# shubhamchandak94/Spring

Hardware: AMD Instinct MI355X
Metric: Mreads/s through reorder stage (higher is better)
Workload: dtype u64; 1 GPU; 100000000 x 150 bp single-end synthetic reads per GPU (uniform genome 600000000 bp, 25x coverage, 1.0% substitutions, 50% reverse-complemented), inputs resident in HBM as .dna records; reads_per_gpu=100000000, read_len=150, chains=65536, num_thr=8, parallelism=single GPU, unmatched=13958636, singletons=12720853, rounds=1984, chain_groups=2

## Files before the change

### include/spring_reorder.h

```cpp
#ifndef SPRING_REORDER_H_
#define SPRING_REORDER_H_

#include <stddef.h>
#include <stdint.h>

#ifdef __cplusplus
extern "C" {
#endif

#define SPRING_REORDER_E_ARG (-1)
#define SPRING_REORDER_E_IO (-2)
#define SPRING_REORDER_E_HIP (-3)
#define SPRING_REORDER_E_STATE (-4)

typedef struct spring_reorder_ctx spring_reorder_ctx;

typedef struct {
  int32_t device;
  uint32_t num_chains;
  int32_t num_thr;
  int32_t collect_stats;
  int32_t time_search;
  int32_t force_literal_update;
  int32_t rounds_per_sync;
  int32_t long_budget;
  int32_t first_shifts;
  int32_t seed_wide;
  int32_t tab_scale;
  int32_t search_wpb;
  int32_t dbg_search_lds;
  int32_t dbg_apply_lds;
  int32_t fused;
  int32_t deep_bins;
  int32_t num_devices;
  int32_t devices[8];
  int32_t mg_host_transport;
  int32_t table_mode;
  int32_t plan0[6];
  int32_t plan1[6];
  int32_t long_min;
  int32_t long_blocks;
  int32_t debug;
  int32_t long_split;
  int32_t entry_flags;
  int32_t out_writers;
  int32_t alternatives;
  int32_t phases;
  int32_t known_absent;
  int32_t sort_prefix_bits;
  int32_t dict_build_mode;
  int32_t strand_filter;
} spring_reorder_opts;

typedef struct {
  uint64_t n_reads, n_matched, n_single, unmatched;
  uint64_t probes, keyok, cands, hits, iterations, rounds, lost;
  uint64_t numkeys[2], dict_numreads[2];
  double ms_unpack, ms_dict, ms_chains, ms_finalize, ms_total;
  double ms_search_kernel;
  uint64_t search_launches;
  uint64_t device_bytes;
  double ms_exchange, ms_resolve_mark;
  uint64_t chains;
  uint64_t deep_pool;
  uint64_t long_searches;
  uint64_t table_minz;
  uint64_t table_marked_lines;
  uint64_t long_splits;
  uint64_t alternatives;
  uint64_t phases;
  double ms_search_busy;
  uint64_t sort_prefix_bits;
  uint64_t sort_repaired_runs;
  uint64_t sort_full_sorts;
  uint64_t sort_long_runs;
  uint64_t sort_list_overflows;
  uint64_t dict_build_path;
  uint64_t strand_filter;
  uint64_t strand_filter_dropped;
  uint64_t strand_filter_build;
} spring_reorder_stats;

void spring_reorder_default_opts(spring_reorder_opts *o);
const char *spring_reorder_last_error(void);
void spring_reorder_trim_pool(void);

int spring_reorder_run(const char *temp_dir, uint32_t max_readlen, int32_t num_thr, int32_t paired_end,
                       uint32_t num_reads_clean_0, uint32_t num_reads_clean_1,
                       const spring_reorder_opts *opts );

int spring_reorder_create(spring_reorder_ctx **ctx, const spring_reorder_opts *opts);
void spring_reorder_destroy(spring_reorder_ctx *ctx);

int spring_reorder_load_dna(spring_reorder_ctx *ctx, const uint8_t *dna, size_t nbytes, uint32_t n,
                            uint32_t max_readlen);

int spring_reorder_load_dna_device(spring_reorder_ctx *ctx, const void *d_dna, size_t nbytes, uint32_t n,
                                   uint32_t max_readlen, int32_t fixed_len);

int spring_reorder_build_dict(spring_reorder_ctx *ctx);

int spring_reorder_run_chains(spring_reorder_ctx *ctx);
int spring_reorder_auto_chains(spring_reorder_ctx *ctx, uint32_t *chains, int32_t *deep);

typedef struct {
  uint32_t num_reads[2], num_reads_clean[2], num_reads_N[2];
  uint32_t max_readlen;
  uint32_t pad;
  double ms_device;
} spring_fastq_info;
int spring_reorder_load_fastq(spring_reorder_ctx *ctx, const uint8_t *fastq_1, size_t nbytes_1, const uint8_t *fastq_2,
                              size_t nbytes_2 , spring_fastq_info *info);
int spring_reorder_fastq_N(spring_reorder_ctx *ctx, int32_t which, uint8_t *n_dna, size_t cap, size_t *nbytes,
                           uint32_t *order_N, uint32_t *count);

int spring_reorder_mg_begin(spring_reorder_ctx *ctx, uint32_t rank, uint32_t world, uint32_t total_chains, void *d_prop);
int spring_reorder_mg_search(spring_reorder_ctx *ctx);
int spring_reorder_mg_slice(spring_reorder_ctx *ctx, void **d_prop, size_t *slice_off, size_t *slice_bytes,
                            size_t *total_bytes);
int spring_reorder_mg_slices(spring_reorder_ctx *ctx, void **d_prop, size_t slice_off[2], size_t slice_bytes[2],
                             size_t *total_bytes, uint32_t *count);
int spring_reorder_mg_apply(spring_reorder_ctx *ctx, int32_t check_alive, uint32_t *alive);
int spring_reorder_mg_end(spring_reorder_ctx *ctx);
int spring_reorder_debug_check_seed_state(spring_reorder_ctx *ctx, int32_t group, uint64_t *violations);
int spring_reorder_mg_exchange_virtual(spring_reorder_ctx **ctxs, uint32_t world);

#define SPRING_RCCL_ID_BYTES 128
typedef struct spring_mg_comm spring_mg_comm;
typedef int (*spring_mg_allgather_fn)(void *host_buf, size_t slice_off, size_t slice_bytes, size_t total_bytes,
                                      void *user);
int spring_mg_rccl_unique_id(void *id128);
int spring_mg_comm_create_rccl(spring_mg_comm **comm, int32_t device, const void *id128, uint32_t rank, uint32_t world);
int spring_mg_comm_create_host(spring_mg_comm **comm, spring_mg_allgather_fn fn, void *user, uint32_t rank,
                               uint32_t world);
void spring_mg_comm_destroy(spring_mg_comm *comm);
int spring_reorder_mg_run(spring_reorder_ctx *ctx, spring_mg_comm *comm, uint32_t total_chains);

int spring_reorder_finalize(spring_reorder_ctx *ctx);

int spring_reorder_get_stats(spring_reorder_ctx *ctx, spring_reorder_stats *st);

int spring_reorder_download(spring_reorder_ctx *ctx, uint32_t *order, char *rc, char *flag, int64_t *pos,
                            uint16_t *rlen, uint32_t *order_s, uint64_t *tid_off, uint64_t *tid_off_s);
int spring_reorder_tid_split(spring_reorder_ctx *ctx, uint64_t *mid, uint64_t *mid_s);

int spring_reorder_emit_dna(spring_reorder_ctx *ctx, int32_t tid, uint8_t *dst, size_t cap, size_t *nbytes);

int spring_reorder_dict_lookup(spring_reorder_ctx *ctx, int32_t which, const uint64_t *keys, uint32_t nkeys,
                               uint32_t *bin_size, uint32_t *bin_ids, size_t ids_cap);

int spring_reorder_presence_table(spring_reorder_ctx *ctx, void *out, size_t cap, int32_t *lgb);

int spring_reorder_download_reads(spring_reorder_ctx *ctx, uint64_t *limbs , uint16_t *len);

int spring_order_invert_se(const uint32_t *order, uint32_t n, uint32_t *order_array, double *kernel_ms);
int spring_order_invert_pe(const uint32_t *order, uint32_t n, uint32_t *order_array, double *kernel_ms);
int spring_order_correct(uint32_t *order, uint64_t m, const uint32_t *order_N, uint32_t nN, uint32_t n_clean,
                         double *kernel_ms);
int spring_order_pe_encode(const uint32_t *order, uint32_t n, uint32_t *new_order, double *kernel_ms);

int spring_fastq_reorder(const uint8_t *fastq, size_t nbytes, const uint32_t *order, uint32_t n, uint8_t *out,
                         size_t out_cap, size_t *out_bytes, double *kernel_ms);

#define SPRING_SYNTH_REPEATS 0x80000000u
#define SPRING_SYNTH_PAIRED 0x40000000u
#define SPRING_SYNTH_GENOMIC 0x20000000u
size_t spring_synth_dna_bytes(uint32_t n, uint32_t L);
int spring_synth_dna_host(uint8_t *dst, uint32_t n, uint32_t L, uint64_t G, uint64_t seed, uint32_t err_ppm);
int spring_synth_genome_host(uint8_t *dst, uint64_t G, uint64_t seed, uint32_t flags);
int spring_synth_dna_device(void *d_dst, uint32_t n, uint32_t L, uint64_t G, uint64_t seed, uint32_t err_ppm);
int spring_reorder_load_synth(spring_reorder_ctx *ctx, uint32_t n, uint32_t L, uint64_t G, uint64_t seed,
                              uint32_t err_ppm);
int spring_reorder_download_dna(spring_reorder_ctx *ctx, uint8_t *dst, size_t cap);

#ifdef __cplusplus
}
#endif
#endif
```

### spring_amd/_lib.py

```python
import ctypes as C
import os

HERE = os.path.dirname(os.path.abspath(__file__))
LIB_PATH = os.environ.get("SPRING_AMD_LIB") or os.path.join(HERE, "lib", "libspring_reorder_hip.so")

EXPORTS = [
    "spring_reorder_default_opts", "spring_reorder_last_error", "spring_reorder_trim_pool", "spring_reorder_run", "spring_reorder_create",
    "spring_reorder_destroy", "spring_reorder_load_dna", "spring_reorder_load_dna_device",
    "spring_reorder_build_dict", "spring_reorder_run_chains", "spring_reorder_auto_chains", "spring_reorder_finalize",
    "spring_reorder_mg_begin", "spring_reorder_mg_search", "spring_reorder_mg_slice", "spring_reorder_mg_slices",
    "spring_reorder_mg_apply",
    "spring_reorder_mg_end", "spring_reorder_mg_exchange_virtual", "spring_reorder_debug_check_seed_state",
    "spring_mg_rccl_unique_id", "spring_mg_comm_create_rccl", "spring_mg_comm_create_host", "spring_mg_comm_destroy",
    "spring_reorder_mg_run",
    "spring_reorder_get_stats", "spring_reorder_download", "spring_reorder_tid_split", "spring_reorder_emit_dna",
    "spring_reorder_dict_lookup", "spring_reorder_presence_table", "spring_reorder_download_reads", "spring_synth_dna_bytes",
    "spring_reorder_load_fastq", "spring_reorder_fastq_N",
    "spring_order_invert_se", "spring_order_invert_pe", "spring_order_correct", "spring_order_pe_encode",
    "spring_fastq_reorder",
    "spring_synth_dna_host", "spring_synth_genome_host", "spring_synth_dna_device", "spring_reorder_load_synth", "spring_reorder_download_dna",
    "spring_encoder_create", "spring_encoder_destroy", "spring_encoder_set_split_tables", "spring_encoder_encode_reorder", "spring_encoder_download",
    "spring_encoder_download_seq_packed", "spring_encoder_get_info", "spring_reorder_encode_run", "spring_encoder_encode_host", "spring_encoder_run",
]

STREAMS_EXPORTS = [
    "spring_streams_create", "spring_streams_destroy", "spring_streams_from_encoder", "spring_streams_from_host",
    "spring_streams_download", "spring_streams_get_info", "spring_streams_run",
]
STREAMS_NUM = 9

DECODE_EXPORTS = [
    "spring_decode_create", "spring_decode_destroy", "spring_decode_seq_from_encoder", "spring_decode_seq_from_host",
    "spring_decode_seq_from_files", "spring_decode_from_streams", "spring_decode_from_host", "spring_decode_from_files",
    "spring_decode_download", "spring_decode_get_info",
]

QUALID_EXPORTS = [
    "spring_qualid_create", "spring_qualid_destroy", "spring_qualid_order_from_host", "spring_qualid_order_from_encoder",
    "spring_qualid_from_fastq", "spring_qualid_from_lines", "spring_qualid_download", "spring_qualid_get_info",
    "spring_quality_table", "spring_id_pattern",
]

FASTQ_OUT_EXPORTS = [
    "spring_fastq_out_create", "spring_fastq_out_destroy", "spring_fastq_out_assemble", "spring_fastq_out_download",
    "spring_fastq_out_write", "spring_fastq_out_get_info",
]

GZIP_EXPORTS = [
    "spring_gzip_create", "spring_gzip_destroy", "spring_gzip_set_chunk_bytes", "spring_gzip_set_token_bytes",
    "spring_gzip_from_fastq_out", "spring_gzip_from_host", "spring_gzip_download", "spring_gzip_write",
    "spring_gzip_get_info",
]

BWT_EXPORTS = [
    "spring_bwt_create", "spring_bwt_destroy", "spring_bwt_set_block_bytes", "spring_bwt_set_workspace_bytes",
    "spring_bwt_workspace_need", "spring_bwt_from_host", "spring_bwt_from_streams", "spring_bwt_download",
    "spring_bwt_segments", "spring_bwt_get_info", "spring_bwt_encode_inplace", "spring_bwt_set_run_keys",
    "spring_bwt_from_qualid", "spring_bwt_round_entries",
]
BWT_MAX_INDEXES = 256
BWT_SRC_QUALITY, BWT_SRC_ID = -2, -3

UNBWT_EXPORTS = [
    "spring_unbwt_create", "spring_unbwt_destroy", "spring_unbwt_set_workspace_bytes", "spring_unbwt_workspace_need",
    "spring_unbwt_set_head_spacing", "spring_unbwt_from_host", "spring_unbwt_from_bwt", "spring_unbwt_download",
    "spring_unbwt_get_info", "spring_unbwt_decode_inplace", "spring_unbwt_from_unqlfc",
]
UNBWT_PASSES = 6

IDCODEC_EXPORTS = [
    "spring_idcodec_create", "spring_idcodec_destroy", "spring_idcodec_set_workspace_bytes",
    "spring_idcodec_workspace_need", "spring_idcodec_from_qualid", "spring_idcodec_from_host", "spring_idcodec_download",
    "spring_idcodec_symbols", "spring_idcodec_get_info",
]
QLFC_EXPORTS = [
    "spring_qlfc_create", "spring_qlfc_destroy", "spring_qlfc_set_state_tables", "spring_qlfc_set_workspace_bytes",
    "spring_qlfc_workspace_need", "spring_qlfc_from_host", "spring_qlfc_from_bwt", "spring_qlfc_download",
    "spring_qlfc_get_info", "spring_qlfc_compress",
]
QLFC_RANK_TABLE, QLFC_RUN_TABLE = 32768, 8192
QLFC_PASSES = 6
QLFC_NOT_COMPRESSIBLE = -16
QLFC_EVENT_BYTES = 160

UNQLFC_EXPORTS = [
    "spring_unqlfc_create", "spring_unqlfc_destroy", "spring_unqlfc_set_state_tables", "spring_unqlfc_set_workspace_bytes",
    "spring_unqlfc_workspace_need", "spring_unqlfc_from_host", "spring_unqlfc_from_qlfc", "spring_unqlfc_download",
    "spring_unqlfc_get_info", "spring_unqlfc_decompress",
]
UNQLFC_PASSES = 3
UNQLFC_MODEL_BYTES = 1619200

BSC_EXPORTS = [
    "spring_bsc_create", "spring_bsc_destroy", "spring_bsc_from_streams", "spring_bsc_from_qualid", "spring_bsc_from_host",
    "spring_bsc_download", "spring_bsc_files", "spring_bsc_get_info", "spring_bsc_adler32", "spring_bsc_compress",
]
BSC_HEADER_BYTES = 28
BSC_PASSES = 3
BSC_BLOCKS, BSC_FILE, BSC_STR_ARRAY = 0, 1, 2
BSC_CODED, BSC_STORED_SMALL, BSC_STORED_CODER, BSC_STORED_NO_GAIN = 0, 1, 2, 3


class Opts(C.Structure):
    _fields_ = [("device", C.c_int32), ("num_chains", C.c_uint32), ("num_thr", C.c_int32),
                ("collect_stats", C.c_int32), ("time_search", C.c_int32), ("force_literal_update", C.c_int32),
                ("rounds_per_sync", C.c_int32), ("long_budget", C.c_int32),
                ("first_shifts", C.c_int32), ("seed_wide", C.c_int32), ("tab_scale", C.c_int32),
                ("search_wpb", C.c_int32), ("dbg_search_lds", C.c_int32), ("dbg_apply_lds", C.c_int32),
                ("fused", C.c_int32), ("deep_bins", C.c_int32),
                ("num_devices", C.c_int32), ("devices", C.c_int32 * 8), ("mg_host_transport", C.c_int32),
                ("table_mode", C.c_int32), ("plan0", C.c_int32 * 6), ("plan1", C.c_int32 * 6), ("long_min", C.c_int32),
                ("long_blocks", C.c_int32), ("debug", C.c_int32), ("long_split", C.c_int32), ("entry_flags", C.c_int32),
                ("out_writers", C.c_int32), ("alternatives", C.c_int32), ("phases", C.c_int32), ("known_absent", C.c_int32),
                ("sort_prefix_bits", C.c_int32), ("dict_build_mode", C.c_int32), ("strand_filter", C.c_int32)]


class Info(C.Structure):

    def asdict(self):
        d = {}
        for k, _ in self._fields_:
            v = getattr(self, k)
            d[k] = list(v) if hasattr(v, "__len__") else v
        return d


class FastqInfo(C.Structure):
    _fields_ = [("num_reads", C.c_uint32 * 2), ("num_reads_clean", C.c_uint32 * 2), ("num_reads_N", C.c_uint32 * 2),
                ("max_readlen", C.c_uint32), ("pad", C.c_uint32), ("ms_device", C.c_double)]


class EncoderInfo(Info):
    _fields_ = ([(k, C.c_uint64) for k in ("n_aligned", "n_total", "seq_len", "noise_bytes", "n_noisepos",
                                           "unaligned_bytes", "len_unaligned", "num_contigs")]
                + [(k, C.c_uint32) for k in ("matched_s", "matched_N", "align_passes", "max_bin")]
                + [("ms_device", C.c_double), ("ms_phase", C.c_double * 8)])


class StreamsInfo(Info):
    _fields_ = ([("num_units", C.c_uint64), ("num_blocks", C.c_uint64), ("bytes", C.c_uint64 * STREAMS_NUM),
                 ("flag_count", C.c_uint64 * 5), ("pos_escapes", C.c_uint64), ("n_aligned", C.c_uint64),
                 ("ms_device", C.c_double), ("ms_file", C.c_double)])


class QualIdInfo(Info):
    _fields_ = [("num_units", C.c_uint64), ("num_blocks", C.c_uint64), ("bytes", C.c_uint64 * 2),
                ("bytes_changed", C.c_uint64), ("max_len", C.c_uint32 * 2), ("ms_device", C.c_double)]


class FastqOutParams(C.Structure):
    _fields_ = ([(k, C.c_uint32) for k in ("first_block", "num_blocks", "num_reads", "num_reads_per_block")]
                + [(k, C.c_int32) for k in ("paired_end", "mate", "preserve_quality", "id_mode", "paired_id_code", "pad")]
                + [("range_start", C.c_uint64), ("range_end", C.c_uint64)])


class FastqOutSources(C.Structure):
    _fields_ = [("decode", C.c_void_p), ("bases", C.c_void_p), ("read_off", C.c_void_p),
                ("quality_ctx", C.c_void_p), ("quality", C.c_void_p), ("quality_bytes", C.c_uint64),
                ("quality_block_off", C.c_void_p),
                ("id_ctx", C.c_void_p), ("ids", C.c_void_p), ("id_bytes", C.c_uint64), ("id_block_off", C.c_void_p)]


class FastqOutInfo(Info):
    _fields_ = [("num_units", C.c_uint64), ("first_slot", C.c_uint64), ("bytes", C.c_uint64),
                ("ms_device", C.c_double), ("ms_file", C.c_double)]


class GzipInfo(Info):
    _fields_ = ([(k, C.c_uint64) for k in ("num_members", "bytes_in", "bytes_out", "chunk_bytes", "num_chunks",
                                           "chunks_stored")]
                + [("ms_device", C.c_double), ("ms_file", C.c_double), ("ms_pass", C.c_double * 6),
                   ("num_batches", C.c_uint64)])


class BwtInfo(Info):
    _fields_ = ([(k, C.c_uint64) for k in ("num_segments", "bytes", "max_segment", "sub_batches", "rounds",
                                           "rounds_total", "workspace_bytes")]
                + [("ms_device", C.c_double), ("ms_pass", C.c_double * 5), ("run_positions", C.c_uint64)])


class UnbwtInfo(Info):
    _fields_ = ([(k, C.c_uint64) for k in ("num_segments", "bytes", "max_segment", "sub_batches", "heads", "head_spacing",
                                           "max_walk", "rank_rounds", "workspace_bytes")]
                + [("ms_device", C.c_double), ("ms_pass", C.c_double * UNBWT_PASSES)])


class IdCodecInfo(Info):
    _fields_ = ([(k, C.c_uint64) for k in ("num_lines", "num_blocks", "num_symbols", "bytes", "max_tokens", "sub_batches")]
                + [("ms_tokens", C.c_double), ("ms_coder", C.c_double)])


class DecodeInfo(Info):
    _fields_ = ([(k, C.c_uint64) for k in ("seq_len", "first_block", "num_blocks", "num_units")]
                + [("bases", C.c_uint64 * 2)]
                + [(k, C.c_uint64) for k in ("n_aligned", "n_unaligned", "pos_escapes")]
                + [("ms_device", C.c_double), ("ms_file", C.c_double)])


class Stats(Info):
    _fields_ = ([(k, C.c_uint64) for k in ("n_reads", "n_matched", "n_single", "unmatched", "probes", "keyok",
                                          "cands", "hits", "iterations", "rounds", "lost")]
                + [("numkeys", C.c_uint64 * 2), ("dict_numreads", C.c_uint64 * 2)]
                + [(k, C.c_double) for k in ("ms_unpack", "ms_dict", "ms_chains", "ms_finalize", "ms_total",
                                             "ms_search_kernel")]
                + [("search_launches", C.c_uint64), ("device_bytes", C.c_uint64),
                   ("ms_exchange", C.c_double), ("ms_resolve_mark", C.c_double), ("chains", C.c_uint64),
                   ("deep_pool", C.c_uint64), ("long_searches", C.c_uint64),
                   ("table_minz", C.c_uint64), ("table_marked_lines", C.c_uint64), ("long_splits", C.c_uint64), ("alternatives", C.c_uint64), ("phases", C.c_uint64),
                   ("ms_search_busy", C.c_double),
                   ("sort_prefix_bits", C.c_uint64), ("sort_repaired_runs", C.c_uint64), ("sort_full_sorts", C.c_uint64),
                   ("sort_long_runs", C.c_uint64), ("sort_list_overflows", C.c_uint64), ("dict_build_path", C.c_uint64),
                   ("strand_filter", C.c_uint64), ("strand_filter_dropped", C.c_uint64),
                   ("strand_filter_build", C.c_uint64)])


NOT_INT = {"spring_reorder_last_error": C.c_char_p, "spring_synth_dna_bytes": C.c_size_t,
           "spring_reorder_default_opts": None, "spring_reorder_trim_pool": None, "spring_mg_comm_destroy": None}
NOT_INT.update({p + "_destroy": None for p in ("spring_reorder", "spring_encoder", "spring_streams", "spring_decode",
                                               "spring_qualid", "spring_fastq_out", "spring_gzip", "spring_bwt",
                                               "spring_unbwt", "spring_idcodec", "spring_qlfc", "spring_bsc",
                                               "spring_unqlfc")})
NOT_INT.update({p + "_workspace_need": C.c_uint64 for p in ("spring_bwt", "spring_unbwt", "spring_idcodec", "spring_qlfc",
                                                             "spring_unqlfc")})

MG_ALLGATHER_FN = C.CFUNCTYPE(C.c_int, C.c_void_p, C.c_size_t, C.c_size_t, C.c_size_t, C.c_void_p)

_lib = None


def lib():
    global _lib
    if _lib is not None:
        return _lib
    if not os.path.exists(LIB_PATH):
        raise RuntimeError(
            "spring_amd: %s is missing. Build it with `python -m spring_amd.build` "
            "(or __graft_entry__.build()); there is no CPU fallback." % LIB_PATH)
    L = C.CDLL(LIB_PATH)
    vp, u8p = C.c_void_p, C.c_void_p
    L.spring_reorder_default_opts.argtypes = [C.POINTER(Opts)]
    L.spring_reorder_run.argtypes = [C.c_char_p, C.c_uint32, C.c_int32, C.c_int32, C.c_uint32, C.c_uint32,
                                     C.POINTER(Opts)]
    L.spring_reorder_create.argtypes = [C.POINTER(vp), C.POINTER(Opts)]
    L.spring_reorder_destroy.argtypes = [vp]
    L.spring_reorder_load_dna.argtypes = [vp, u8p, C.c_size_t, C.c_uint32, C.c_uint32]
    L.spring_reorder_load_dna_device.argtypes = [vp, vp, C.c_size_t, C.c_uint32, C.c_uint32, C.c_int32]
    L.spring_reorder_build_dict.argtypes = [vp]
    L.spring_reorder_run_chains.argtypes = [vp]
    L.spring_reorder_auto_chains.argtypes = [vp, C.POINTER(C.c_uint32), C.POINTER(C.c_int32)]
    L.spring_reorder_finalize.argtypes = [vp]
    L.spring_reorder_mg_begin.argtypes = [vp, C.c_uint32, C.c_uint32, C.c_uint32, vp]
    L.spring_reorder_mg_search.argtypes = [vp]
    L.spring_reorder_mg_slice.argtypes = [vp, C.POINTER(vp), C.POINTER(C.c_size_t), C.POINTER(C.c_size_t), C.POINTER(C.c_size_t)]
    L.spring_reorder_mg_slices.argtypes = [vp, C.POINTER(vp), C.POINTER(C.c_size_t), C.POINTER(C.c_size_t), C.POINTER(C.c_size_t),
                                           C.POINTER(C.c_uint32)]
    L.spring_reorder_debug_check_seed_state.argtypes = [vp, C.c_int32, C.POINTER(C.c_uint64)]
    L.spring_reorder_mg_apply.argtypes = [vp, C.c_int32, C.POINTER(C.c_uint32)]
    L.spring_reorder_mg_end.argtypes = [vp]
    L.spring_reorder_mg_exchange_virtual.argtypes = [C.POINTER(vp), C.c_uint32]
    L.spring_mg_rccl_unique_id.argtypes = [vp]
    L.spring_mg_comm_create_rccl.argtypes = [C.POINTER(vp), C.c_int32, vp, C.c_uint32, C.c_uint32]
    L.spring_mg_comm_create_host.argtypes = [C.POINTER(vp), MG_ALLGATHER_FN, vp, C.c_uint32, C.c_uint32]
    L.spring_mg_comm_destroy.argtypes = [vp]
    L.spring_reorder_mg_run.argtypes = [vp, vp, C.c_uint32]
    L.spring_reorder_get_stats.argtypes = [vp, C.POINTER(Stats)]
    L.spring_reorder_download.argtypes = [vp] + [vp] * 8
    L.spring_reorder_tid_split.argtypes = [vp, vp, vp]
    L.spring_reorder_emit_dna.argtypes = [vp, C.c_int32, u8p, C.c_size_t, C.POINTER(C.c_size_t)]
    L.spring_reorder_dict_lookup.argtypes = [vp, C.c_int32, vp, C.c_uint32, vp, vp, C.c_size_t]
    L.spring_reorder_presence_table.argtypes = [vp, vp, C.c_size_t, C.POINTER(C.c_int32)]
    L.spring_reorder_download_reads.argtypes = [vp, vp, vp]
    L.spring_reorder_load_fastq.argtypes = [vp, vp, C.c_size_t, vp, C.c_size_t, C.POINTER(FastqInfo)]
    L.spring_reorder_fastq_N.argtypes = [vp, C.c_int32, vp, C.c_size_t, C.POINTER(C.c_size_t), vp, C.POINTER(C.c_uint32)]
    L.spring_order_invert_se.argtypes = [vp, C.c_uint32, vp, C.POINTER(C.c_double)]
    L.spring_order_invert_pe.argtypes = [vp, C.c_uint32, vp, C.POINTER(C.c_double)]
    L.spring_fastq_reorder.argtypes = [u8p, C.c_size_t, vp, C.c_uint32, u8p, C.c_size_t, C.POINTER(C.c_size_t),
                                       C.POINTER(C.c_double)]
    L.spring_order_pe_encode.argtypes = [vp, C.c_uint32, vp, C.POINTER(C.c_double)]
    L.spring_order_correct.argtypes = [vp, C.c_uint64, vp, C.c_uint32, C.c_uint32, C.POINTER(C.c_double)]
    L.spring_synth_dna_bytes.argtypes = [C.c_uint32, C.c_uint32]
    L.spring_synth_dna_host.argtypes = [u8p, C.c_uint32, C.c_uint32, C.c_uint64, C.c_uint64, C.c_uint32]
    L.spring_synth_genome_host.argtypes = [u8p, C.c_uint64, C.c_uint64, C.c_uint32]
    L.spring_synth_dna_device.argtypes = [vp, C.c_uint32, C.c_uint32, C.c_uint64, C.c_uint64, C.c_uint32]
    L.spring_reorder_load_synth.argtypes = [vp, C.c_uint32, C.c_uint32, C.c_uint64, C.c_uint64, C.c_uint32]
    L.spring_reorder_download_dna.argtypes = [vp, u8p, C.c_size_t]
    L.spring_encoder_create.argtypes = [C.c_int32, C.POINTER(vp)]
    L.spring_encoder_destroy.argtypes = [vp]
    L.spring_encoder_encode_reorder.argtypes = [vp, vp, u8p, C.c_uint64, vp, C.c_uint32, C.POINTER(EncoderInfo)]
    L.spring_encoder_download.argtypes = [vp] + [vp] * 9
    L.spring_encoder_download_seq_packed.argtypes = [vp, vp, vp]
    L.spring_encoder_encode_host.argtypes = [vp, C.c_uint32, C.c_int32, vp, u8p, C.c_uint64, vp, vp, vp, vp, vp, u8p,
                                             C.c_uint64, vp, C.c_uint32, u8p, C.c_uint64, vp, C.c_uint32,
                                             C.POINTER(EncoderInfo)]
    L.spring_encoder_run.argtypes = [C.c_char_p, C.c_uint32, C.c_int32, C.c_uint32, C.c_uint32, C.c_int32,
                                     C.POINTER(EncoderInfo)]
    L.spring_encoder_get_info.argtypes = [vp, C.POINTER(EncoderInfo)]
    L.spring_reorder_encode_run.argtypes = [C.c_char_p, C.c_uint32, C.c_int32, C.c_int32, C.c_uint32, C.c_uint32,
                                            C.c_uint32, C.POINTER(Opts), C.POINTER(EncoderInfo)]
    L.spring_streams_create.argtypes = [C.c_int32, C.POINTER(vp)]
    L.spring_streams_destroy.argtypes = [vp]
    L.spring_streams_from_encoder.argtypes = [vp, vp, C.c_uint32, C.c_int32, C.c_int32, C.c_uint32, C.c_int32,
                                              C.POINTER(StreamsInfo)]
    L.spring_streams_from_host.argtypes = [vp, vp, vp, C.c_uint64, vp, C.c_uint64, vp, C.c_uint64, vp, vp, C.c_uint64, vp,
                                           C.c_uint64, C.c_uint32, C.c_int32, C.c_int32, C.c_uint32, C.POINTER(StreamsInfo)]
    L.spring_streams_download.argtypes = [vp, C.c_int32, vp, vp]
    L.spring_streams_get_info.argtypes = [vp, C.POINTER(StreamsInfo)]
    L.spring_streams_run.argtypes = [C.c_char_p, C.c_uint32, C.c_int32, C.c_int32, C.c_uint32, C.c_int32,
                                     C.POINTER(StreamsInfo)]
    L.spring_decode_create.argtypes = [C.c_int32, C.POINTER(vp)]
    L.spring_decode_destroy.argtypes = [vp]
    L.spring_decode_seq_from_encoder.argtypes = [vp, vp]
    L.spring_decode_seq_from_host.argtypes = [vp, C.c_int32, vp, vp, vp]
    L.spring_decode_seq_from_files.argtypes = [vp, C.c_char_p, C.c_int32]
    L.spring_decode_from_streams.argtypes = [vp, vp, C.POINTER(DecodeInfo)]
    L.spring_decode_from_host.argtypes = [vp, vp, vp, C.c_uint32, C.c_uint32, C.c_uint32, C.c_int32, C.c_int32,
                                          C.c_uint32, C.POINTER(DecodeInfo)]
    L.spring_decode_from_files.argtypes = [vp, C.c_char_p, C.c_uint32, C.c_uint32, C.c_uint32, C.c_int32, C.c_int32,
                                           C.c_uint32, C.POINTER(DecodeInfo)]
    L.spring_decode_download.argtypes = [vp, C.c_int32, vp, vp]
    L.spring_decode_get_info.argtypes = [vp, C.POINTER(DecodeInfo)]
    L.spring_qualid_create.argtypes = [C.c_int32, C.POINTER(vp)]
    L.spring_qualid_destroy.argtypes = [vp]
    L.spring_qualid_order_from_host.argtypes = [vp, vp, C.c_uint32, C.c_int32]
    L.spring_qualid_order_from_encoder.argtypes = [vp, vp, C.c_uint32, C.c_int32]
    L.spring_qualid_from_fastq.argtypes = [vp, u8p, C.c_size_t, C.c_int32, u8p, C.c_uint32, C.POINTER(QualIdInfo)]
    L.spring_qualid_from_lines.argtypes = [vp, C.c_int32, u8p, C.c_size_t, u8p, C.c_uint32, C.POINTER(QualIdInfo)]
    L.spring_qualid_download.argtypes = [vp, C.c_int32, u8p, vp, vp]
    L.spring_qualid_get_info.argtypes = [vp, C.POINTER(QualIdInfo)]
    L.spring_quality_table.argtypes = [C.c_int32, C.c_uint32, C.c_uint32, C.c_uint32, u8p]
    L.spring_id_pattern.argtypes = [u8p, C.c_size_t, u8p, C.c_size_t, C.c_int32, C.POINTER(C.c_uint8),
                                    C.POINTER(C.c_double)]
    L.spring_fastq_out_create.argtypes = [C.c_int32, C.POINTER(vp)]
    L.spring_fastq_out_destroy.argtypes = [vp]
    L.spring_fastq_out_assemble.argtypes = [vp, C.POINTER(FastqOutParams), C.POINTER(FastqOutSources),
                                            C.POINTER(FastqOutInfo)]
    L.spring_fastq_out_download.argtypes = [vp, u8p, vp]
    L.spring_fastq_out_write.argtypes = [vp, C.c_char_p, C.c_int32, C.POINTER(FastqOutInfo)]
    L.spring_fastq_out_get_info.argtypes = [vp, C.POINTER(FastqOutInfo)]
    L.spring_gzip_create.argtypes = [C.c_int32, C.POINTER(vp)]
    L.spring_gzip_destroy.argtypes = [vp]
    L.spring_gzip_set_chunk_bytes.argtypes = [vp, C.c_uint32]
    L.spring_gzip_set_token_bytes.argtypes = [vp, C.c_uint64]
    L.spring_gzip_from_fastq_out.argtypes = [vp, vp, C.c_uint64, C.c_int32, C.POINTER(GzipInfo)]
    L.spring_gzip_from_host.argtypes = [vp, u8p, C.c_uint64, vp, C.c_uint64, C.c_int32, C.POINTER(GzipInfo)]
    L.spring_gzip_download.argtypes = [vp, u8p, vp]
    L.spring_gzip_write.argtypes = [vp, C.c_char_p, C.c_int32, C.POINTER(GzipInfo)]
    L.spring_gzip_get_info.argtypes = [vp, C.POINTER(GzipInfo)]
    L.spring_bwt_create.argtypes = [C.c_int32, C.POINTER(vp)]
    L.spring_bwt_destroy.argtypes = [vp]
    L.spring_bwt_set_block_bytes.argtypes = [vp, C.c_uint64]
    L.spring_bwt_set_workspace_bytes.argtypes = [vp, C.c_uint64]
    L.spring_bwt_workspace_need.argtypes = [C.c_uint64, C.c_uint64]
    L.spring_bwt_from_host.argtypes = [vp, u8p, C.c_uint64, vp, C.c_uint64, C.POINTER(BwtInfo)]
    L.spring_bwt_from_streams.argtypes = [vp, vp, C.c_uint32, C.POINTER(BwtInfo)]
    L.spring_bwt_download.argtypes = [vp, u8p, vp, vp, vp, vp]
    L.spring_bwt_segments.argtypes = [vp, vp, vp, vp]
    L.spring_bwt_get_info.argtypes = [vp, C.POINTER(BwtInfo)]
    L.spring_bwt_encode_inplace.argtypes = [vp, u8p, C.c_int32, vp, vp]
    L.spring_bwt_set_run_keys.argtypes = [vp, C.c_int32, C.c_uint32]
    L.spring_bwt_round_entries.argtypes = [vp, vp, C.c_uint64]
    L.spring_bwt_from_qualid.argtypes = [vp, vp, C.c_int32, C.c_uint64, C.POINTER(BwtInfo)]
    L.spring_unbwt_create.argtypes = [C.c_int32, C.POINTER(vp)]
    L.spring_unbwt_destroy.argtypes = [vp]
    L.spring_unbwt_set_workspace_bytes.argtypes = [vp, C.c_uint64]
    L.spring_unbwt_workspace_need.argtypes = [C.c_uint64, C.c_uint64]
    L.spring_unbwt_set_head_spacing.argtypes = [vp, C.c_uint32]
# ... 51 lines not shown
```

### spring_amd/csrc/dict_build.h

```cpp
#ifndef SPRING_DICT_BUILD_H_
#define SPRING_DICT_BUILD_H_

#include "reorder_device.h"

namespace sr {

bool launch_unpack_keys(hipStream_t st, const uint8_t *dna, uint32_t n, int L, int W, int S, uint32_t rec_fixed,
                        uint64_t *reads, uint16_t *lens, uint32_t *bad_len, int dstart0, int dend0, int dstart1, int dend1,
                        uint64_t *keys0, uint32_t *vals0, uint64_t *keys1, uint32_t *vals1);

constexpr int TAB_WRITE_LG = 10;
inline int tab_write_lg(int bshift) { return 64 - bshift < TAB_WRITE_LG ? 64 - bshift : TAB_WRITE_LG; }
inline uint32_t tab_write_blocks(int bshift) { return (uint32_t)(1ull << (64 - bshift - tab_write_lg(bshift))); }
void launch_tab_partition(hipStream_t st, const uint64_t *h0, uint32_t nk0, const uint64_t *h1, uint32_t nk1, int bshift,
                          uint32_t *part);
constexpr uint32_t TAB_OVF_SLOTS = 8;
void launch_tab_write(hipStream_t st, const uint64_t *h0, uint32_t nk0, const uint64_t *h1, uint32_t nk1,
                      const uint32_t *part, DictBuild d0, DictBuild d1, uint4 *fpt, int bshift, uint32_t *ovf,
                      uint32_t *ovf_blk, uint32_t *ovf_cnt);
void launch_tab_overflow_blocks(hipStream_t st, const uint64_t *h0, uint32_t nk0, const uint64_t *h1, DictBuild d0,
                                DictBuild d1, uint32_t *fpt, int bshift, const uint32_t *ovf_blk, const uint32_t *ovf_cnt);
void launch_tab_overflow_pairs(hipStream_t st, const uint64_t *h0, uint32_t nk0, const uint64_t *h1, DictBuild d0,
                               DictBuild d1, uint32_t *fpt, int bshift, const uint32_t *ovf, uint32_t novf);

constexpr uint32_t PRES_DROP_CTRS = 1024;
constexpr int PRES_WRITE_LG = 10;
inline int pres_write_lg(int lgb) { return lgb < PRES_WRITE_LG ? lgb : PRES_WRITE_LG; }
inline uint32_t pres_write_blocks(int lgb) { return 1u << (lgb - pres_write_lg(lgb)); }
void launch_pres_insert(hipStream_t st, const uint64_t *h0, uint32_t nk0, const uint64_t *h1, uint32_t nk1, int wl, uint32_t *pres,
                        int lgb, uint32_t *drops, bool skip_self_canonical);
void launch_pres_write(hipStream_t st, const uint64_t *h0, uint32_t nk0, const uint64_t *h1, uint32_t nk1, int wl, uint4 *pres,
                       int lgb, uint32_t *part, uint32_t *drops);

}

#endif
```

### spring_amd/csrc/dict_build.hip

```cpp
#include <hip/hip_runtime.h>

#include "dict_build.h"
#include "strand_filter.h"

namespace sr {

__device__ __forceinline__ uint64_t db_mix64(uint64_t x) {
  x ^= x >> 33; x *= 0xff51afd7ed558ccdull; x ^= x >> 33; x *= 0xc4ceb9fe1a85ec53ull; x ^= x >> 33;
  return x;
}
__device__ __forceinline__ uint64_t db_unmix64(uint64_t x) {
  x ^= x >> 33; x *= 0x9cb4b2f8129337dbull; x ^= x >> 33; x *= 0x4f74430c22a54005ull; x ^= x >> 33;
  return x;
}
__device__ __forceinline__ uint32_t db_fp30_of(uint64_t h) {
  const uint32_t f = (uint32_t)h & 0x3fffffffu;
  return f == 0u ? 1u : f == 0x3fffffffu ? 0x3ffffffeu : f;
}

__global__ __launch_bounds__(256) void k_unpack_fixed_keys(const uint8_t *__restrict__ dna, uint32_t n, int L, int W, int lgS,
                                                           uint32_t rec, uint64_t *__restrict__ reads,
                                                           uint16_t *__restrict__ lens, uint32_t *__restrict__ bad_len,
                                                           int dstart0, int klen0, int dstart1, int klen1,
                                                           uint64_t *__restrict__ keys0, uint32_t *__restrict__ vals0,
                                                           uint64_t *__restrict__ keys1, uint32_t *__restrict__ vals1) {
  extern __shared__ uint4 s_unpack[];
  const uint32_t r0 = blockIdx.x * (uint32_t)UNPACK_READS;
  const uint32_t nr = min((uint32_t)UNPACK_READS, n - r0);
  const uint8_t *g = dna + (uint64_t)r0 * rec;
  const uint32_t sh = (uint32_t)((uintptr_t)g & 15u);
  const uint4 *ga = reinterpret_cast<const uint4 *>(g - sh);
  const uint32_t nchunk = (sh + nr * rec + 15u) >> 4;
  for (uint32_t k = threadIdx.x; k < nchunk; k += 256) s_unpack[k] = ga[k];
  __syncthreads();
  const uint8_t *sb = reinterpret_cast<const uint8_t *>(s_unpack);
  const uint32_t *sw = reinterpret_cast<const uint32_t *>(s_unpack);
  const bool chk = bad_len != nullptr;
  const uint32_t S = 1u << lgS;
  auto len_of = [&](uint32_t r) -> uint32_t {
    const uint32_t p = sh + r * rec;
    return (uint32_t)sb[p] | ((uint32_t)sb[p + 1] << 8);
  };
  auto limb = [&](uint32_t m) -> uint64_t {
    const uint32_t r = m >> lgS, j = m & (S - 1u);
    if ((int)j >= W) return 0;
    uint32_t len = len_of(r);
    if (chk && len != (uint32_t)L) len = (uint32_t)L;
    const uint32_t nb = min((len + 3u) / 4u, rec - 2u), pos = 8u * j;
    if (pos >= nb) return 0;
    const uint32_t p = sh + r * rec + 2u + pos, k = p >> 2, s8 = (p & 3u) * 8u;
    uint64_t v = (uint64_t)sw[k] | ((uint64_t)sw[k + 1] << 32);
    if (s8) v = (v >> s8) | ((uint64_t)sw[k + 2] << (64u - s8));
    if (nb - pos < 8u) v &= (1ull << (8u * (nb - pos))) - 1ull;
    return v;
  };
  for (uint32_t t = threadIdx.x; 2u * t < nr; t += 256) {
    const uint32_t r = 2u * t;
    uint32_t l0 = len_of(r), l1 = r + 1 < nr ? len_of(r + 1) : (uint32_t)L;
    if (chk && (l0 != (uint32_t)L || l1 != (uint32_t)L)) {
      *bad_len = 1u;
      l0 = l1 = (uint32_t)L;
    }
    if (r + 1 < nr) *reinterpret_cast<uint32_t *>(lens + r0 + r) = l0 | (l1 << 16);
    else lens[r0 + r] = (uint16_t)l0;
  }
  const uint32_t nl = nr << lgS;
  uint64_t *out = reads + ((uint64_t)r0 << lgS);
  for (uint32_t q = threadIdx.x; 2u * q < nl; q += 256) {
    const uint32_t m = 2u * q;
    const uint64_t v0 = limb(m);
    if (m + 1 < nl) *reinterpret_cast<ulonglong2 *>(out + m) = make_ulonglong2(v0, limb(m + 1));
    else out[m] = v0;
  }
  auto window = [&](uint32_t r, int dstart, int klen2) -> uint64_t {
    const uint32_t bitpos = 2u * (uint32_t)dstart, li = bitpos >> 6, off = bitpos & 63u;
    uint64_t v = limb((r << lgS) + li) >> off;
    if (off && li + 1u < S) v |= limb((r << lgS) + li + 1u) << (64u - off);
    if (klen2 < 64) v &= (1ull << klen2) - 1ull;
    return v;
  };
  for (uint32_t r = threadIdx.x; r < nr; r += 256) {
    const uint32_t i = r0 + r;
    keys0[i] = db_mix64(window(r, dstart0, 2 * klen0));
    vals0[i] = i;
    keys1[i] = db_mix64(window(r, dstart1, 2 * klen1));
    vals1[i] = i;
  }
}

bool launch_unpack_keys(hipStream_t st, const uint8_t *dna, uint32_t n, int L, int W, int S, uint32_t rec_fixed,
                        uint64_t *reads, uint16_t *lens, uint32_t *bad_len, int dstart0, int dend0, int dstart1, int dend1,
                        uint64_t *keys0, uint32_t *vals0, uint64_t *keys1, uint32_t *vals1) {
  if (!n || ((uintptr_t)reads & 15u) || ((uintptr_t)lens & 3u)) return false;
  if (dstart0 < 0 || dstart1 < 0 || dend0 >= L || dend1 >= L || 2 * dend0 / 64 >= S || 2 * dend1 / 64 >= S) return false;
  int lgS = 0;
  while ((1 << lgS) < S) lgS++;
  const size_t lds = ((size_t)UNPACK_READS * rec_fixed + 15 + 12 + 15) / 16 * 16;
  hipLaunchKernelGGL(k_unpack_fixed_keys, dim3((n + UNPACK_READS - 1) / UNPACK_READS), dim3(256), lds, st, dna, n, L, W, lgS,
                     rec_fixed, reads, lens, bad_len, dstart0, dend0 - dstart0 + 1, dstart1, dend1 - dstart1 + 1, keys0, vals0,
                     keys1, vals1);
  return true;
}

__global__ void k_tab_partition(const uint64_t *__restrict__ h0, uint32_t nk0, const uint64_t *__restrict__ h1, uint32_t nk1,
                                int bshift, int lg, uint32_t nblk, uint32_t *__restrict__ part) {
  const uint64_t t = (uint64_t)blockIdx.x * blockDim.x + threadIdx.x;
  if (t >= 2ull * ((uint64_t)nblk + 1)) return;
  const uint32_t l = t > nblk ? 1u : 0u, j = (uint32_t)(t - (l ? (uint64_t)nblk + 1 : 0));
  const uint64_t *__restrict__ h = l ? h1 : h0;
  const uint32_t nk = l ? nk1 : nk0;
  uint32_t lo = 0, hi = nk;
  if (j == nblk) {
    lo = nk;
  } else if (j != 0u) {
    const uint64_t bound = ((uint64_t)j << lg) << bshift;
    while (lo < hi) {
      const uint32_t mid = lo + (hi - lo) / 2;
      if (h[mid] < bound) lo = mid + 1; else hi = mid;
    }
  }
  part[t] = lo;
}

constexpr uint32_t TAB_WRITE_TILE = 512, TAB_WRITE_THREADS = 512;
__global__ __launch_bounds__(TAB_WRITE_THREADS) void k_tab_write(const uint64_t *__restrict__ h0, uint32_t nk0,
                                                                 const uint64_t *__restrict__ h1, uint32_t nk1,
                                                                 const uint32_t *__restrict__ part, uint32_t nblk,
                                                                 DictBuild d0, DictBuild d1, uint4 *__restrict__ fpt,
                                                                 int bshift, int lg, uint32_t *__restrict__ ovf,
                                                                 uint32_t *__restrict__ ovf_blk, uint32_t *__restrict__ ovf_cnt) {
  __shared__ uint4 img[2u << TAB_WRITE_LG];
  __shared__ uint64_t tile[2][TAB_WRITE_TILE];
  __shared__ uint16_t first[2][1u << TAB_WRITE_LG];
  __shared__ uint32_t s_novf;
  const uint32_t nbk = 1u << lg, bmask = nbk - 1u, blk = blockIdx.x;
  for (uint32_t k = threadIdx.x; k < 2u * nbk; k += TAB_WRITE_THREADS) img[k] = make_uint4(0u, 0u, 0u, 0u);
  for (uint32_t k = threadIdx.x; k < nbk / 2u + 1u; k += TAB_WRITE_THREADS) {
    if (2u * k < nbk) { reinterpret_cast<uint32_t *>(first[0])[k] = 0u; reinterpret_cast<uint32_t *>(first[1])[k] = 0u; }
  }
  if (threadIdx.x == 0) s_novf = 0u;
  const uint32_t a0 = part[blk], a1 = part[(uint64_t)nblk + 1 + blk];
  const uint32_t c0 = part[blk + 1] - a0, c1 = part[(uint64_t)nblk + 2 + blk] - a1;
  const uint32_t ntot = c0 + c1;
  auto bin_of = [&](uint32_t t, uint32_t &st, uint32_t &cn, uint32_t &pay) {
    const bool l = t >= c0;
    const uint32_t i = l ? a1 + (t - c0) : a0 + t;
    st = (l ? d1.ustart : d0.ustart)[i]; cn = (l ? d1.ucount : d0.ucount)[i];
    pay = cn == 1u ? (l ? d1.ids : d0.ids)[st] : i;
  };
  uint32_t st0 = 0, cn0 = 0, pay0 = 0, st1 = 0, cn1 = 0, pay1 = 0;
  if (threadIdx.x < ntot) bin_of(threadIdx.x, st0, cn0, pay0);
  if (threadIdx.x + TAB_WRITE_THREADS < ntot) bin_of(threadIdx.x + TAB_WRITE_THREADS, st1, cn1, pay1);
  __syncthreads();
  for (uint32_t k = threadIdx.x; k < min(c0, TAB_WRITE_TILE); k += TAB_WRITE_THREADS) {
    const uint64_t x = h0[a0 + k];
    tile[0][k] = x;
    if (k == 0u || (h0[a0 + k - 1u] >> bshift) != (x >> bshift)) first[0][(uint32_t)(x >> bshift) & bmask] = (uint16_t)(k + 1u);
  }
  for (uint32_t k = threadIdx.x; k < min(c1, TAB_WRITE_TILE); k += TAB_WRITE_THREADS) {
    const uint64_t x = h1[a1 + k];
    tile[1][k] = x;
    if (k == 0u || (h1[a1 + k - 1u] >> bshift) != (x >> bshift)) first[1][(uint32_t)(x >> bshift) & bmask] = (uint16_t)(k + 1u);
  }
  const bool staged = c0 <= TAB_WRITE_TILE && c1 <= TAB_WRITE_TILE;
  __syncthreads();
  if (ntot) {
    uint32_t *imgw = reinterpret_cast<uint32_t *>(img);
    auto H = [&](bool l, uint32_t k) -> uint64_t {
      if (k < TAB_WRITE_TILE) return l ? tile[1][k] : tile[0][k];
      return l ? h1[a1 + k] : h0[a0 + k];
    };
    auto place = [&](uint32_t t, uint32_t st, uint32_t cn, uint32_t pay) {
      const bool l = t >= c0;
      const uint32_t k = l ? t - c0 : t, i = (l ? a1 : a0) + k;
      const uint64_t hh = H(l, k), b = hh >> bshift;
      uint32_t rank = 0;
      while (rank < 4u && k > rank && (H(l, k - 1u - rank) >> bshift) == b) rank++;
      if (rank < 4u && staged) {
        const uint32_t f = l ? first[0][(uint32_t)b & bmask] : first[1][(uint32_t)b & bmask], co = l ? c0 : c1;
        if (f) {
          for (uint32_t o = f - 1u; rank < 4u && o < co; o++) {
            const uint64_t x = l ? tile[0][o] : tile[1][o];
            if ((x >> bshift) != b || (l ? x > hh : x >= hh)) break;
            rank++;
          }
        }
      } else if (rank < 4u) {
        uint32_t lo = 0, hi = l ? c0 : c1;
        while (lo < hi) {
          const uint32_t mid = (lo + hi) >> 1;
          const uint64_t x = H(!l, mid);
          if (l ? x <= hh : x < hh) lo = mid + 1u; else hi = mid;
        }
        while (rank < 4u && lo > 0u && (H(!l, lo - 1u) >> bshift) == b) { rank++; lo--; }
      }
      uint32_t *nd = l ? d1.ndeep : d0.ndeep;
      if (cn >= DEEP_BIN) (l ? d1.deep : d0.deep)[atomicAdd(nd, 1u)] = i;
      if (cn >= BIG_BIN) atomicAdd(nd + 1, cn);
      if (cn >= MID_BIN) atomicAdd(nd + 2, cn);
      (l ? d1.urec : d0.urec)[i] = make_ulonglong2(db_unmix64(hh), (uint64_t)st | ((uint64_t)cn << 32));
      if (rank >= 4u) {
        const uint32_t g = l ? nk0 + i : i, slot = atomicAdd(&s_novf, 1u);
        if (slot < TAB_OVF_SLOTS) ovf_blk[(uint64_t)blk * TAB_OVF_SLOTS + slot] = g;
        else ovf[1u + atomicAdd(ovf, 1u)] = g;
      } else {
        const uint32_t bl = (uint32_t)b & bmask;
        imgw[bl * 8u + rank] = (db_fp30_of(hh) << 2) | ((uint32_t)l << 1) | (cn == 1u ? 1u : 0u);
        imgw[bl * 8u + 4u + rank] = pay;
      }
    };
    if (threadIdx.x < ntot) place(threadIdx.x, st0, cn0, pay0);
    if (threadIdx.x + TAB_WRITE_THREADS < ntot) place(threadIdx.x + TAB_WRITE_THREADS, st1, cn1, pay1);
    for (uint32_t t = threadIdx.x + 2u * TAB_WRITE_THREADS; t < ntot; t += TAB_WRITE_THREADS) {
      bin_of(t, st0, cn0, pay0);
      place(t, st0, cn0, pay0);
    }
    __syncthreads();
  }
  if (threadIdx.x == 0) ovf_cnt[blk] = min(s_novf, TAB_OVF_SLOTS);
  uint4 *__restrict__ out = fpt + (((uint64_t)blk << lg) << 1);
  for (uint32_t k = threadIdx.x; k < 2u * nbk; k += TAB_WRITE_THREADS) out[k] = img[k];
}

__device__ __forceinline__ void tab_overflow_insert(uint32_t g, const uint64_t *__restrict__ h0, uint32_t nk0,
                                                    const uint64_t *__restrict__ h1, const DictBuild &d0, const DictBuild &d1,
                                                    uint32_t *fpt, int bshift) {
  const uint32_t l = g >= nk0 ? 1u : 0u, u = l ? g - nk0 : g;
  const uint64_t h = (l ? h1 : h0)[u];
  const DictBuild &d = l ? d1 : d0;
  const uint32_t st = d.ustart[u], cn = d.ucount[u];
  const bool single = cn == 1u;
  const uint32_t tag = (db_fp30_of(h) << 2) | (l << 1) | (single ? 1u : 0u);
  const uint32_t pay = single ? d.ids[st] : u;
  const uint64_t bmask = (1ull << (64 - bshift)) - 1;
  uint64_t b = ((h >> bshift) + 1) & bmask;
  for (;;) {
    uint32_t *bk = fpt + b * 8;
    for (int sl = 0; sl < 4; sl++) {
      if (atomicCAS(bk + sl, 0u, tag) == 0u) {
        bk[4 + sl] = pay;
        return;
      }
    }
    b = (b + 1) & bmask;
  }
}
__global__ void k_tab_overflow_blocks(const uint64_t *__restrict__ h0, uint32_t nk0, const uint64_t *__restrict__ h1,
                                      DictBuild d0, DictBuild d1, uint32_t *fpt, int bshift, uint32_t nblk,
                                      const uint32_t *__restrict__ ovf_blk, const uint32_t *__restrict__ ovf_cnt) {
  const uint64_t t = (uint64_t)blockIdx.x * blockDim.x + threadIdx.x;
  const uint64_t blk = t / TAB_OVF_SLOTS;
  if (blk >= nblk || (uint32_t)(t % TAB_OVF_SLOTS) >= ovf_cnt[blk]) return;
  tab_overflow_insert(ovf_blk[t], h0, nk0, h1, d0, d1, fpt, bshift);
}
// ... 124 lines not shown
```

### spring_amd/csrc/reorder_pipeline.cpp

```cpp
#include <hip/hip_runtime.h>
#include <dlfcn.h>

#include <algorithm>
#include <system_error>
#include <thread>
#include <memory>
#include <atomic>
#include <chrono>
#include <cstdarg>
#include <cstdio>
#include <cstdlib>
#include <cstring>
#include <map>
#include <mutex>
#include <new>
#include <stdexcept>
#include <string>
#include <unordered_map>
#include <vector>
#include <zlib.h>

#include "reorder_device.h"
#include "dict_build.h"
#include "reorder_internal.h"
#include "spring_reorder.h"
#include "stage_host.h"
#include "synth_common.h"

namespace sr {
thread_local std::string g_err;
int fail(int code, const char *fmt, ...) {
  char buf[512];
  va_list ap;
  va_start(ap, fmt);
  vsnprintf(buf, sizeof(buf), fmt, ap);
  va_end(ap);
  g_err = buf;
  return code;
}
}

using namespace sr;

namespace {
struct DevPool {
  std::mutex mu;
  std::multimap<size_t, void *> free_blocks;
  std::unordered_map<void *, size_t> sizes;
  size_t cached = 0;
};
DevPool g_pool[16];
constexpr size_t POOL_GRAN = 2u << 20;

hipError_t pool_alloc(int dev, size_t bytes, void **out, size_t *actual) {
  const size_t want = (bytes + POOL_GRAN - 1) / POOL_GRAN * POOL_GRAN;
  DevPool &p = g_pool[dev & 15];
  {
    std::lock_guard<std::mutex> lk(p.mu);
    auto it = p.free_blocks.lower_bound(want);
    if (it != p.free_blocks.end() && it->first <= want + want / 4 + POOL_GRAN) {
      *out = it->second; *actual = it->first;
      p.cached -= it->first;
      p.free_blocks.erase(it);
      return hipSuccess;
    }
  }
  hipError_t e = hipMalloc(out, want);
  if (e != hipSuccess) {
    std::lock_guard<std::mutex> lk(p.mu);
    for (auto &kv : p.free_blocks) { (void)hipFree(kv.second); p.sizes.erase(kv.second); }
    p.free_blocks.clear(); p.cached = 0;
    (void)hipGetLastError();
    e = hipMalloc(out, want);
  }
  if (e == hipSuccess) {
    std::lock_guard<std::mutex> lk(p.mu);
    p.sizes[*out] = want;
    *actual = want;
  }
  return e;
}
void pool_free(int dev, void *ptr) {
  DevPool &p = g_pool[dev & 15];
  std::lock_guard<std::mutex> lk(p.mu);
  auto it = p.sizes.find(ptr);
  if (it == p.sizes.end()) { (void)hipFree(ptr); return; }
  p.free_blocks.emplace(it->second, ptr);
  p.cached += it->second;
}
}

enum { ST_CREATED = 0, ST_LOADED = 1, ST_DICT = 2, ST_CHAINS = 3, ST_FINAL = 4 };

struct DictDev {
  int start = 0, end = 0;
  uint32_t numkeys = 0, numreads = 0;
  ulonglong2 *urec = nullptr;
  uint32_t *ids = nullptr;
  uint32_t *deep = nullptr, *d_ndeep = nullptr;
  uint32_t ndeep = 0;
  uint32_t big_reads = 0;
  uint32_t mid_reads = 0;
};

struct spring_reorder_ctx {
  spring_reorder_opts o;
  int dev = 0;
  hipStream_t st = nullptr;
  int stage = ST_CREATED;
  std::vector<void *> allocs;
  uint64_t dev_bytes = 0, peak_bytes = 0;
  uint8_t *d_dna = nullptr;
  bool dna_borrowed = false;
  size_t dna_bytes = 0;
  uint64_t *d_off = nullptr;
  uint32_t n = 0;
  int L = 0, W = 0, S = 0, Lpad = 0;
  bool uniform = true;
  uint64_t *d_reads = nullptr;
  uint16_t *d_lens = nullptr;
  uint64_t *pre_keys[2] = {nullptr, nullptr};
  uint32_t *pre_vals[2] = {nullptr, nullptr};
  DictDev dict[2];
  uint4 *fpt = nullptr;
  int bshift = 63;
  int minz = 0, lshift = 31;
  uint32_t marked_lines = 0;
  uint4 *pres = nullptr;
  int pres_lgb = 0;
  bool user_plan0 = false;
  DevParams P;
  uint32_t K = 0;
  uint64_t nrec = 0, nsing = 0, cap = 0;
  bool mg = false;
  uint32_t *cnt_buf[2] = {nullptr, nullptr};
  uint64_t round_no = 0;
  hipStream_t st2 = nullptr, st3 = nullptr;
  uint64_t *taken2 = nullptr;
  uint32_t *resv2 = nullptr, *won = nullptr;
  uint32_t Kh = 0, nmid = 0;
  struct GroupGeom { uint32_t g0 = 0, Kg = 0, c0 = 0, gg0 = 0, gKg = 0; } grp[2];
  struct LongBufs { uint32_t *longq = nullptr, *lctl = nullptr, *lparts = nullptr; LongHead *lhead = nullptr; uint2 *lbin = nullptr; uint16_t *lbcode = nullptr; } lb2;
  bool in_source_fallback = false;
  uint8_t *d_N[2] = {nullptr, nullptr};
  uint32_t *d_orderN[2] = {nullptr, nullptr};
  uint64_t *d_offN[2] = {nullptr, nullptr};
  uint64_t N_bytes[2] = {0, 0};
  spring_fastq_info fq;
  double fq_ms = 0;
  std::vector<uint64_t> tid_off, tid_off_s;
  std::vector<uint64_t> tid_mid, tid_mid_s;
  spring_reorder_stats stats;
  hipEvent_t ev[8];
  bool ev_ok = false;

  int dmalloc(void **p, size_t bytes) {
    if (bytes == 0) bytes = 16;
    size_t actual = 0;
    hipError_t e = pool_alloc(dev, bytes, p, &actual);
    if (e != hipSuccess) return fail(SPRING_REORDER_E_HIP, "hipMalloc(%zu) failed: %s", bytes, hipGetErrorString(e));
    allocs.push_back(*p);
    dev_bytes += actual;
    peak_bytes = std::max(peak_bytes, dev_bytes);
    return 0;
  }
  void dfree(void *p) {
    if (!p) return;
    auto it = std::find(allocs.begin(), allocs.end(), p);
    if (it != allocs.end()) allocs.erase(it);
    {
      std::lock_guard<std::mutex> lk(g_pool[dev & 15].mu);
      auto sz = g_pool[dev & 15].sizes.find(p);
      if (sz != g_pool[dev & 15].sizes.end()) dev_bytes -= std::min<uint64_t>(dev_bytes, sz->second);
    }
    (void)hipStreamSynchronize(st);
    pool_free(dev, p);
  }
};

namespace sr {
int reorder_view(spring_reorder_ctx *ctx, ReorderView *v) {
  if (ctx && ctx->mg) return fail(SPRING_REORDER_E_STATE, "single-pool multi-GPU contexts hold partial streams");
  return reorder_view_any(ctx, v);
}
int reorder_view_any(spring_reorder_ctx *ctx, ReorderView *v) {
  if (!ctx || !v) return fail(SPRING_REORDER_E_ARG, "NULL argument");
  if (ctx->stage != ST_FINAL) return fail(SPRING_REORDER_E_STATE, "reorder context is not finalized");
  v->dev = ctx->dev; v->st = ctx->st; v->n = ctx->n; v->L = ctx->L; v->W = ctx->W; v->S = ctx->S;
  v->reads = ctx->d_reads; v->lens = ctx->d_lens; v->nrec = ctx->nrec; v->nsing = ctx->nsing;
  v->f_order = ctx->P.f_order; v->f_order_s = ctx->P.f_order_s; v->f_rc = ctx->P.f_rc; v->f_flag = ctx->P.f_flag;
  v->f_pos = ctx->P.f_pos; v->f_len = ctx->P.f_len; v->tid_off = ctx->tid_off.data(); v->num_thr = ctx->o.num_thr;
  v->tid_off_s = ctx->tid_off_s.data();
  v->tid_mid = ctx->tid_mid.data(); v->tid_mid_s = ctx->tid_mid_s.data();
  for (int j = 0; j < 2; j++) {
    v->N_dna[j] = ctx->d_N[j]; v->N_off[j] = ctx->d_offN[j]; v->N_order[j] = ctx->d_orderN[j];
    v->N_count[j] = ctx->fq.num_reads_N[j]; v->N_bytes[j] = ctx->N_bytes[j];
  }
  v->fq_num_reads_0 = ctx->fq.num_reads[0];
  return 0;
}
hipError_t dev_alloc(int dev, size_t bytes, void **out) {
  size_t actual = 0;
  return pool_alloc(dev, bytes ? bytes : 16, out, &actual);
}
void dev_free(int dev, void *p) { if (p) pool_free(dev, p); }
}

namespace {
struct RcclId128 { char b[128]; };
struct Rccl {
  void *h = nullptr;
  int (*GetUniqueId)(void *) = nullptr;
  int (*CommInitRank)(void **, int, RcclId128, int) = nullptr;
  int (*CommDestroy)(void *) = nullptr;
  int (*CommAbort)(void *) = nullptr;
  int (*AllGather)(const void *, void *, size_t, int, void *, hipStream_t) = nullptr;
  const char *(*GetErrorString)(int) = nullptr;
};
Rccl g_rccl;
std::mutex g_rccl_mu;
int rccl_load() {
  std::lock_guard<std::mutex> lk(g_rccl_mu);
  if (g_rccl.h) return 0;
  void *h = dlopen("librccl.so.1", RTLD_NOW | RTLD_GLOBAL);
  if (!h) h = dlopen("librccl.so", RTLD_NOW | RTLD_GLOBAL);
  if (!h) return fail(SPRING_REORDER_E_HIP, "cannot load librccl.so.1: %s", dlerror());
  g_rccl.GetUniqueId = (decltype(g_rccl.GetUniqueId))dlsym(h, "ncclGetUniqueId");
  g_rccl.CommInitRank = (decltype(g_rccl.CommInitRank))dlsym(h, "ncclCommInitRank");
  g_rccl.CommDestroy = (decltype(g_rccl.CommDestroy))dlsym(h, "ncclCommDestroy");
  g_rccl.CommAbort = (decltype(g_rccl.CommAbort))dlsym(h, "ncclCommAbort");
  g_rccl.AllGather = (decltype(g_rccl.AllGather))dlsym(h, "ncclAllGather");
  g_rccl.GetErrorString = (decltype(g_rccl.GetErrorString))dlsym(h, "ncclGetErrorString");
  if (!g_rccl.GetUniqueId || !g_rccl.CommInitRank || !g_rccl.CommDestroy || !g_rccl.AllGather)
    return fail(SPRING_REORDER_E_HIP, "librccl lacks an expected entry point");
  g_rccl.h = h;
  return 0;
}
const char *rccl_err(int e) { return g_rccl.GetErrorString ? g_rccl.GetErrorString(e) : "rccl error"; }
constexpr int RCCL_UINT64 = 5;
}
#if defined(__has_include)
#if __has_include(<rccl/rccl.h>)
#include <rccl/rccl.h>
#include <type_traits>
static_assert(sizeof(ncclUniqueId) == sizeof(RcclId128) && NCCL_UNIQUE_ID_BYTES == 128, "ncclUniqueId is not 128 bytes");
static_assert((int)ncclUint64 == RCCL_UINT64, "ncclUint64 has another code");
static_assert(sizeof(ncclResult_t) == sizeof(int) && sizeof(ncclDataType_t) == sizeof(int) && sizeof(ncclComm_t) == sizeof(void *),
              "enum / handle sizes differ from the hand-written prototypes");
static_assert(std::is_same<decltype(&ncclGetUniqueId), ncclResult_t (*)(ncclUniqueId *)>::value, "ncclGetUniqueId");
static_assert(std::is_same<decltype(&ncclCommInitRank), ncclResult_t (*)(ncclComm_t *, int, ncclUniqueId, int)>::value, "ncclCommInitRank");
static_assert(std::is_same<decltype(&ncclCommDestroy), ncclResult_t (*)(ncclComm_t)>::value, "ncclCommDestroy");
static_assert(std::is_same<decltype(&ncclCommAbort), ncclResult_t (*)(ncclComm_t)>::value, "ncclCommAbort");
static_assert(std::is_same<decltype(&ncclAllGather),
                           ncclResult_t (*)(const void *, void *, size_t, ncclDataType_t, ncclComm_t, hipStream_t)>::value, "ncclAllGather");
static_assert(std::is_same<decltype(&ncclGetErrorString), const char *(*)(ncclResult_t)>::value, "ncclGetErrorString");
#endif
#endif
namespace {
}

struct spring_mg_comm {
  uint32_t rank = 0, world = 1;
  int dev = 0;
  void *rccl = nullptr;
  std::mutex mu;
  bool aborted = false;
  spring_mg_allgather_fn host_fn = nullptr;
  void *host_user = nullptr;
};

#define DMALLOC(ptr, bytes)                                   \
  do {                                                        \
    int r_ = ctx->dmalloc((void **)&(ptr), (bytes));          \
    if (r_) return r_;                                        \
  } while (0)

extern "C" {

void spring_reorder_default_opts(spring_reorder_opts *o) {
  memset(o, 0, sizeof(*o));
  o->device = -1;
  o->num_chains = 0;
  o->num_thr = 1;
}

const char *spring_reorder_last_error(void) { return g_err.c_str(); }

extern "C++" {
namespace {
struct PinCache {
  std::mutex mu;
  std::vector<void *> free_chunks;
};
PinCache g_pin;
}
namespace sr {
void *pinned_get() {
  {
    std::lock_guard<std::mutex> lk(g_pin.mu);
    if (!g_pin.free_chunks.empty()) {
      void *p = g_pin.free_chunks.back();
      g_pin.free_chunks.pop_back();
      return p;
    }
  }
  void *p = nullptr;
  if (hipHostMalloc(&p, PIN_CHUNK, hipHostMallocDefault) != hipSuccess) { (void)hipGetLastError(); return nullptr; }
  return p;
}
void pinned_put(void *p) {
  if (!p) return;
  std::lock_guard<std::mutex> lk(g_pin.mu);
  g_pin.free_chunks.push_back(p);
}
}
}

void spring_reorder_trim_pool(void) {
  {
    std::lock_guard<std::mutex> lk(g_pin.mu);
    for (void *p : g_pin.free_chunks) (void)hipHostFree(p);
    g_pin.free_chunks.clear();
  }
  for (int d = 0; d < 16; d++) {
    DevPool &p = g_pool[d];
    std::lock_guard<std::mutex> lk(p.mu);
    if (p.free_blocks.empty()) continue;
    (void)hipSetDevice(d);
    for (auto &kv : p.free_blocks) { (void)hipFree(kv.second); p.sizes.erase(kv.second); }
    p.free_blocks.clear();
    p.cached = 0;
  }
}

int spring_reorder_create(spring_reorder_ctx **out, const spring_reorder_opts *opts) {
  if (!out) return fail(SPRING_REORDER_E_ARG, "ctx is NULL");
  spring_reorder_opts o;
  if (opts) o = *opts; else spring_reorder_default_opts(&o);
  if (o.num_thr <= 0) return fail(SPRING_REORDER_E_ARG, "num_thr must be >= 1");
  if (o.sort_prefix_bits < 0 || o.sort_prefix_bits > 64)
    return fail(SPRING_REORDER_E_ARG, "sort_prefix_bits: 0 (library's choice) or 1 .. 64 bits of the key hash (64 = the full sort)");
  if (o.dict_build_mode < 0 || o.dict_build_mode > 1)
    return fail(SPRING_REORDER_E_ARG, "dict_build_mode: 0 (library's choice) or 1 (key pass, memset, merge and insert passes)");
  if (o.strand_filter < -1 || o.strand_filter > 32)
    return fail(SPRING_REORDER_E_ARG, "strand_filter: 0 (library's choice), -1 (off) or 1 .. 32 (on, at most 2^n buckets)");
  int ndev = 0;
  HIPCHK(hipGetDeviceCount(&ndev));
  if (ndev <= 0) return fail(SPRING_REORDER_E_HIP, "no HIP device");
  int dev = o.device;
  if (dev < 0) HIPCHK(hipGetDevice(&dev));
  if (dev >= ndev) return fail(SPRING_REORDER_E_ARG, "device %d out of range (%d devices)", dev, ndev);
  HIPCHK(hipSetDevice(dev));
  spring_reorder_ctx *ctx = new spring_reorder_ctx();
  ctx->o = o;
  ctx->dev = dev;
  memset(&ctx->P, 0, sizeof(ctx->P));
  memset(&ctx->stats, 0, sizeof(ctx->stats));
  HIPCHK(hipStreamCreateWithFlags(&ctx->st, hipStreamNonBlocking));
  for (auto &e : ctx->ev) HIPCHK(hipEventCreate(&e));
  ctx->ev_ok = true;
  *out = ctx;
  return 0;
}

void spring_reorder_destroy(spring_reorder_ctx *ctx) {
  if (!ctx) return;
  (void)hipSetDevice(ctx->dev);
  if (ctx->st) (void)hipStreamSynchronize(ctx->st);
  if (ctx->st2) (void)hipStreamSynchronize(ctx->st2);
  if (ctx->st3) (void)hipStreamSynchronize(ctx->st3);
  for (void *p : ctx->allocs) pool_free(ctx->dev, p);
  if (ctx->ev_ok) for (auto &e : ctx->ev) (void)hipEventDestroy(e);
  if (ctx->st) (void)hipStreamDestroy(ctx->st);
  if (ctx->st2) (void)hipStreamDestroy(ctx->st2);
  if (ctx->st3) (void)hipStreamDestroy(ctx->st3);
  delete ctx;
}

static int setup_geometry(spring_reorder_ctx *ctx, uint32_t n, uint32_t max_readlen) {
  if (max_readlen == 0 || max_readlen > (uint32_t)MAX_READ_LEN)
    return fail(SPRING_REORDER_E_ARG, "Wrong bitset size. (max_readlen=%u, supported 1..511)", max_readlen);
  ctx->n = n;
  ctx->L = (int)max_readlen;
  ctx->W = (2 * ctx->L - 1) / 64 + 1;
  int S = 1;
  while (S < ctx->W) S <<= 1;
  ctx->S = S;
  ctx->Lpad = (ctx->L + 63) / 64 * 64;
  const int L = ctx->L;
  ctx->dict[0].start = L > 100 ? L / 2 - 32 : L / 2 - L * 32 / 100;
  ctx->dict[0].end = L / 2 - 1;
  ctx->dict[1].start = L / 2;
  ctx->dict[1].end = L > 100 ? L / 2 - 1 + 32 : L / 2 - 1 + L * 32 / 100;
  return 0;
}

static void drop_pre_keys(spring_reorder_ctx *ctx) {
  for (int l = 0; l < 2; l++) {
    ctx->dfree(ctx->pre_keys[l]); ctx->pre_keys[l] = nullptr;
    ctx->dfree(ctx->pre_vals[l]); ctx->pre_vals[l] = nullptr;
  }
}

static int unpack_on_device(spring_reorder_ctx *ctx, uint32_t *d_bad_len = nullptr, bool with_keys = false) {
  if (!ctx->d_reads) DMALLOC(ctx->d_reads, (size_t)std::max<uint32_t>(ctx->n, 1) * ctx->S * sizeof(uint64_t));
  if (!ctx->d_lens) DMALLOC(ctx->d_lens, (size_t)std::max<uint32_t>(ctx->n, 1) * sizeof(uint16_t));
  drop_pre_keys(ctx);
  const uint32_t rec = 2u + ((uint32_t)ctx->L + 3u) / 4u;
  with_keys = with_keys && ctx->n && !ctx->d_off && ctx->uniform && ctx->o.dict_build_mode != 1 &&
              ctx->L > ctx->dict[0].end && ctx->L > ctx->dict[1].end && ctx->dict[0].start >= 0;
  if (with_keys) {
    for (int l = 0; l < 2; l++) {
      DMALLOC(ctx->pre_keys[l], (size_t)ctx->n * 8);
      DMALLOC(ctx->pre_vals[l], (size_t)ctx->n * 4);
    }
  }
  HIPCHK(hipEventRecord(ctx->ev[0], ctx->st));
  if (with_keys && !launch_unpack_keys(ctx->st, ctx->d_dna, ctx->n, ctx->L, ctx->W, ctx->S, rec, ctx->d_reads, ctx->d_lens, d_bad_len,
                                       ctx->dict[0].start, ctx->dict[0].end, ctx->dict[1].start, ctx->dict[1].end,
                                       ctx->pre_keys[0], ctx->pre_vals[0], ctx->pre_keys[1], ctx->pre_vals[1])) {
    with_keys = false;
    drop_pre_keys(ctx);
  }
  if (!with_keys)
    launch_unpack(ctx->st, ctx->d_dna, ctx->d_off, ctx->n, ctx->L, ctx->W, ctx->S, rec, ctx->d_reads, ctx->d_lens, d_bad_len);
  HIPCHK(hipGetLastError());
  HIPCHK(hipEventRecord(ctx->ev[1], ctx->st));
  ctx->stage = ST_LOADED;
  return 0;
}

static int upload_chunked(spring_reorder_ctx *ctx, uint8_t *d_dst, size_t nbytes,
                          int (*fill)(void *, size_t, void *, size_t), void *self) {
  if (!nbytes) return 0;
  const size_t nchunks = (nbytes + PIN_CHUNK - 1) / PIN_CHUNK;
  const unsigned hw = std::max(1u, std::thread::hardware_concurrency());
  const int nthr = (int)std::min<size_t>(std::min<size_t>(8, hw), nchunks);
  std::atomic<size_t> next{0};
  std::atomic<int> rc{0};
  std::vector<std::string> errs((size_t)nthr);
  auto worker = [&](int ti) {
    void *pin[2] = {nullptr, nullptr};
    hipEvent_t ev[2] = {nullptr, nullptr};
    hipStream_t st = nullptr;
    bool used[2] = {false, false};
    auto bail = [&](int code, const char *what) {
      int zero = 0;
      if (rc.compare_exchange_strong(zero, code)) errs[(size_t)ti] = what;
    };
    if (hipSetDevice(ctx->dev) != hipSuccess || hipStreamCreateWithFlags(&st, hipStreamNonBlocking) != hipSuccess) {
      bail(SPRING_REORDER_E_HIP, "upload: cannot create a copy stream");
    } else {
      for (int k = 0; k < 2 && !rc.load(); k++) {
        pin[k] = pinned_get();
        if (!pin[k] || hipEventCreateWithFlags(&ev[k], hipEventDisableTiming) != hipSuccess) bail(SPRING_REORDER_E_HIP, "upload: cannot pin a staging chunk");
      }
      for (int k = 0; !rc.load(); k ^= 1) {
        const size_t i = next.fetch_add(1);
        if (i >= nchunks) break;
        const size_t off = i * PIN_CHUNK, len = std::min(PIN_CHUNK, nbytes - off);
        if (used[k] && hipEventSynchronize(ev[k]) != hipSuccess) { bail(SPRING_REORDER_E_HIP, "upload: event wait failed"); break; }
        if (fill(self, off, pin[k], len)) { bail(SPRING_REORDER_E_IO, g_err.c_str()); break; }
        if (hipMemcpyAsync(d_dst + off, pin[k], len, hipMemcpyHostToDevice, st) != hipSuccess ||
            hipEventRecord(ev[k], st) != hipSuccess) { bail(SPRING_REORDER_E_HIP, "upload: hipMemcpyAsync failed"); break; }
        used[k] = true;
      }
      (void)hipStreamSynchronize(st);
    }
    for (int k = 0; k < 2; k++) { if (ev[k]) (void)hipEventDestroy(ev[k]); pinned_put(pin[k]); }
    if (st) (void)hipStreamDestroy(st);
  };
  std::vector<std::thread> th;
  try {
    for (int t = 1; t < nthr; t++) th.emplace_back(worker, t);
  } catch (const std::system_error &) {
  }
  worker(0);
  for (auto &x : th) x.join();
  (void)hipGetLastError();
  if (rc.load()) {
    for (auto &e : errs) if (!e.empty()) return fail(rc.load(), "%s", e.c_str());
    return fail(rc.load(), "upload failed");
  }
  return 0;
}

struct D2HJob { void *dst; const void *src; size_t nbytes; };
static int download_chunked(spring_reorder_ctx *ctx, const std::vector<D2HJob> &jobs) {
  struct Piece { uint8_t *dst; const uint8_t *src; size_t len; };
  std::vector<Piece> pieces;
  for (const D2HJob &j : jobs)
    for (size_t off = 0; off < j.nbytes; off += PIN_CHUNK)
      pieces.push_back({(uint8_t *)j.dst + off, (const uint8_t *)j.src + off, std::min(PIN_CHUNK, j.nbytes - off)});
  if (pieces.empty()) return 0;
  HIPCHK(hipStreamSynchronize(ctx->st));
  const unsigned hw = std::max(1u, std::thread::hardware_concurrency());
  const int nthr = (int)std::min<size_t>(std::min<size_t>(8, hw), pieces.size());
  std::atomic<size_t> next{0};
  std::atomic<int> rc{0};
  auto worker = [&]() {
    void *pin[2] = {nullptr, nullptr};
    hipStream_t st = nullptr;
    const Piece *pending[2] = {nullptr, nullptr};
    if (hipSetDevice(ctx->dev) != hipSuccess || hipStreamCreateWithFlags(&st, hipStreamNonBlocking) != hipSuccess) rc = SPRING_REORDER_E_HIP;
    for (int k = 0; k < 2 && !rc.load(); k++) if (!(pin[k] = pinned_get())) rc = SPRING_REORDER_E_HIP;
    hipEvent_t ev[2] = {nullptr, nullptr};
    for (int k = 0; k < 2 && !rc.load(); k++) if (hipEventCreateWithFlags(&ev[k], hipEventDisableTiming) != hipSuccess) rc = SPRING_REORDER_E_HIP;
    auto drain = [&](int k) {
      if (!pending[k]) return;
      if (hipEventSynchronize(ev[k]) != hipSuccess) rc = SPRING_REORDER_E_HIP;
      else memcpy(pending[k]->dst, pin[k], pending[k]->len);
      pending[k] = nullptr;
    };
    for (int k = 0; !rc.load(); k ^= 1) {
      const size_t i = next.fetch_add(1);
      if (i >= pieces.size()) break;
      drain(k);
      if (hipMemcpyAsync(pin[k], pieces[i].src, pieces[i].len, hipMemcpyDeviceToHost, st) != hipSuccess ||
          hipEventRecord(ev[k], st) != hipSuccess) { rc = SPRING_REORDER_E_HIP; break; }
      pending[k] = &pieces[i];
// ... 341 lines not shown
  HIPCHK(hipEventRecord(ctx->ev[6], st));
  for (int j = 0; j < 2; j++) {
    if (!f[j].nreads) continue;
    DMALLOC(ctx->d_N[j], f[j].N_bytes + 16);
    DMALLOC(ctx->d_orderN[j], (size_t)std::max<uint32_t>(f[j].n_N, 1) * 4);
    DMALLOC(ctx->d_offN[j], (size_t)std::max<uint32_t>(f[j].n_N, 1) * 8);
    ctx->N_bytes[j] = f[j].N_bytes;
    launch_pack_reads(st, f[j].d_txt, f[j].line_end, f[j].nreads, f[j].len, f[j].fclean, f[j].cidx, f[j].coff, f[j].nidx,
                      f[j].noff, cbase, obase, 0u, ctx->d_dna, ctx->d_off, ctx->d_N[j], ctx->d_orderN[j], ctx->d_offN[j]);
    HIPCHK(hipGetLastError());
    cbase += f[j].n_clean; obase += f[j].clean_bytes; rbase += (uint32_t)f[j].nreads;
  }
  (void)rbase;
  ctx->uniform = n_clean > 0 && std::min(f[0].min_clean, f[1].min_clean) == maxlen;
  if (ctx->uniform) { ctx->dfree(ctx->d_off); ctx->d_off = nullptr; }
  r = unpack_on_device(ctx);
  if (r) return r;
  HIPCHK(hipEventRecord(ctx->ev[7], st));
  HIPCHK(hipStreamSynchronize(st));
  { float ms = 0; if (hipEventElapsedTime(&ms, ctx->ev[6], ctx->ev[7]) == hipSuccess) ctx->fq_ms += ms; }
  ms_dev = ctx->fq_ms;
  ctx->fq.ms_device = ms_dev;
  if (info) info->ms_device = ms_dev;
  for (int j = 0; j < 2; j++) {
    ctx->dfree(f[j].d_txt); ctx->dfree(f[j].line_end); ctx->dfree(f[j].len); ctx->dfree(f[j].fclean); ctx->dfree(f[j].szc);
    ctx->dfree(f[j].fN); ctx->dfree(f[j].szN); ctx->dfree(f[j].cidx); ctx->dfree(f[j].nidx); ctx->dfree(f[j].coff);
    ctx->dfree(f[j].noff);
  }
  ctx->dfree(d_err);
  return 0;
}

int spring_reorder_fastq_N(spring_reorder_ctx *ctx, int32_t which, uint8_t *n_dna, size_t cap, size_t *nbytes,
                           uint32_t *order_N, uint32_t *count) {
  if (!ctx || ctx->stage < ST_LOADED) return fail(SPRING_REORDER_E_STATE, "fastq_N: load_fastq first");
  if (which < 0 || which > 1) return fail(SPRING_REORDER_E_ARG, "which must be 0 or 1");
  HIPCHK(hipSetDevice(ctx->dev));
  const uint32_t nN = ctx->fq.num_reads_N[which];
  if (nbytes) *nbytes = ctx->N_bytes[which];
  if (count) *count = nN;
  if (n_dna && ctx->N_bytes[which]) {
    if (cap < ctx->N_bytes[which]) return fail(SPRING_REORDER_E_ARG, "fastq_N: buffer too small");
    HIPCHK(hipMemcpy(n_dna, ctx->d_N[which], ctx->N_bytes[which], hipMemcpyDeviceToHost));
  }
  if (order_N && nN) HIPCHK(hipMemcpy(order_N, ctx->d_orderN[which], (size_t)nN * 4, hipMemcpyDeviceToHost));
  return 0;
}

size_t spring_synth_dna_bytes(uint32_t n, uint32_t L) { return (size_t)n * (2u + (L + 3u) / 4u); }

int spring_synth_dna_host(uint8_t *dst, uint32_t n, uint32_t L, uint64_t G, uint64_t seed, uint32_t err_ppm) {
  if (L == 0 || L > (uint32_t)MAX_READ_LEN || G < L) return fail(SPRING_REORDER_E_ARG, "bad synth geometry");
  if ((err_ppm & SYN_PAIRED_FLAG) && (n & 1)) return fail(SPRING_REORDER_E_ARG, "a paired pool holds an even number of reads");
  const uint32_t rec = 2u + (L + 3u) / 4u, thr = syn_err_thr24(err_ppm);
  for (uint64_t i = 0; i < n; i++) {
    uint8_t *o = dst + i * rec;
    uint64_t pos; uint32_t rc;
    syn_read_params(seed, G, L, i, (err_ppm & SYN_PAIRED_FLAG) ? n / 2 : 0, &pos, &rc);
    o[0] = (uint8_t)(L & 0xff); o[1] = (uint8_t)(L >> 8);
    for (uint32_t b = 0; b < (L + 3) / 4; b++) {
      uint32_t v = 0;
      for (uint32_t q = 0; q < 4; q++) {
        uint32_t j = 4 * b + q;
        if (j < L) v |= syn_nat_to_spring(syn_read_base(seed, G, L, thr, i, j, pos, rc)) << (2 * q);
      }
      o[2 + b] = (uint8_t)v;
    }
  }
  return 0;
}

int spring_synth_genome_host(uint8_t *dst, uint64_t G, uint64_t seed, uint32_t flags) {
  if (!dst) return fail(SPRING_REORDER_E_ARG, "dst is NULL");
  for (uint64_t p = 0; p < G; p++) {
    uint64_t gp = p;
    if (flags & SYN_REPEAT_FLAG) {
      const uint64_t seg = G / 8, k = seg ? gp / seg : 0;
      if (seg && k < 8 && (k & 1) == 0) gp %= seg;
    }
    dst[p] = (uint8_t)"ACGT"[(flags & SYN_GENOMIC_FLAG) ? syn_genomic_base(seed, gp) : syn_genome_base(seed, gp)];
  }
  return 0;
}

int spring_synth_dna_device(void *d_dst, uint32_t n, uint32_t L, uint64_t G, uint64_t seed, uint32_t err_ppm) {
  if (!d_dst || L == 0 || L > (uint32_t)MAX_READ_LEN || G < L) return fail(SPRING_REORDER_E_ARG, "bad synth arguments");
  if ((err_ppm & SYN_PAIRED_FLAG) && (n & 1)) return fail(SPRING_REORDER_E_ARG, "a paired pool holds an even number of reads");
  launch_synth(nullptr, (uint8_t *)d_dst, n, L, G, seed, syn_err_thr24(err_ppm));
  HIPCHK(hipGetLastError());
  HIPCHK(hipStreamSynchronize(nullptr));
  return 0;
}

int spring_reorder_load_synth(spring_reorder_ctx *ctx, uint32_t n, uint32_t L, uint64_t G, uint64_t seed,
                              uint32_t err_ppm) {
  if (!ctx) return fail(SPRING_REORDER_E_ARG, "ctx is NULL");
  if (ctx->stage != ST_CREATED) return fail(SPRING_REORDER_E_STATE, "load_synth: context already loaded");
  if (L == 0 || L > (uint32_t)MAX_READ_LEN || G < L) return fail(SPRING_REORDER_E_ARG, "bad synth geometry");
  if ((err_ppm & SYN_PAIRED_FLAG) && (n & 1)) return fail(SPRING_REORDER_E_ARG, "a paired pool holds an even number of reads");
  HIPCHK(hipSetDevice(ctx->dev));
  int r = setup_geometry(ctx, n, L);
  if (r) return r;
  ctx->uniform = true;
  ctx->dna_bytes = spring_synth_dna_bytes(n, L);
  DMALLOC(ctx->d_dna, ctx->dna_bytes + 16);
  launch_synth(ctx->st, ctx->d_dna, n, L, G, seed, syn_err_thr24(err_ppm));
  HIPCHK(hipGetLastError());
  return unpack_on_device(ctx, nullptr, true);
}

int spring_reorder_download_dna(spring_reorder_ctx *ctx, uint8_t *dst, size_t cap) {
  if (!ctx || ctx->stage < ST_LOADED) return fail(SPRING_REORDER_E_STATE, "download_dna: nothing loaded");
  if (cap < ctx->dna_bytes) return fail(SPRING_REORDER_E_ARG, "buffer too small");
  HIPCHK(hipSetDevice(ctx->dev));
  HIPCHK(hipStreamSynchronize(ctx->st));
  if (ctx->dna_bytes) HIPCHK(hipMemcpy(dst, ctx->d_dna, ctx->dna_bytes, hipMemcpyDeviceToHost));
  return 0;
}

int spring_reorder_download_reads(spring_reorder_ctx *ctx, uint64_t *limbs, uint16_t *len) {
  if (!ctx || ctx->stage < ST_LOADED) return fail(SPRING_REORDER_E_STATE, "download_reads: nothing loaded");
  HIPCHK(hipSetDevice(ctx->dev));
  HIPCHK(hipStreamSynchronize(ctx->st));
  if (!ctx->n) return 0;
  if (limbs)
    HIPCHK(hipMemcpy2D(limbs, (size_t)ctx->W * 8, ctx->d_reads, (size_t)ctx->S * 8, (size_t)ctx->W * 8, ctx->n,
                       hipMemcpyDeviceToHost));
  if (len) HIPCHK(hipMemcpy(len, ctx->d_lens, (size_t)ctx->n * 2, hipMemcpyDeviceToHost));
  return 0;
}

static uint64_t pow2ceil(uint64_t x) {
  uint64_t p = 1;
  while (p < x) p <<= 1;
  return p;
}

static double now_ms() {
  return std::chrono::duration<double, std::milli>(std::chrono::steady_clock::now().time_since_epoch()).count();
}
#define DBG_T(label)                                                                         \
  do {                                                                                       \
    if (dbg) { (void)hipStreamSynchronize(st); double t_ = now_ms(); fprintf(stderr, "[dict] %-14s %8.2f ms\n", label, t_ - t_last); t_last = t_; } \
  } while (0)

static TabView tab_view(const spring_reorder_ctx *ctx) {
  TabView t;
  t.buck = ctx->fpt;
  t.bshift = ctx->bshift; t.minz = ctx->minz; t.lshift = ctx->lshift;
  return t;
}

static unsigned sort_prefix_auto(uint64_t m) { return m <= (1ull << 29) ? 40u : 48u; }

static bool strand_filter_wanted(const spring_reorder_ctx *ctx);

static bool presence_wanted(const spring_reorder_ctx *ctx, uint64_t nm) { return nm && nm < 0xffffffffull && strand_filter_wanted(ctx); }
static int presence_alloc(spring_reorder_ctx *ctx, uint64_t nm, bool dbg) {
  int lgb = 0;
  while (lgb < 32 && (1ull << lgb) < nm) lgb++;
  if (ctx->o.strand_filter > 0) lgb = std::min(lgb, ctx->o.strand_filter);
  if (ctx->dmalloc((void **)&ctx->pres, (size_t)16 << lgb)) {
    (void)hipGetLastError();
    ctx->pres = nullptr;
    if (dbg) fprintf(stderr, "[dict] presence table: no room for 2^%d buckets, running without\n", lgb);
  }
  return lgb;
}
int spring_reorder_build_dict(spring_reorder_ctx *ctx) {
  double t_last = now_ms();
  if (!ctx) return fail(SPRING_REORDER_E_ARG, "ctx is NULL");
  const bool dbg = ctx->o.debug != 0;
  if (ctx->stage != ST_LOADED) return fail(SPRING_REORDER_E_STATE, "build_dict: load reads first");
  HIPCHK(hipSetDevice(ctx->dev));
  hipStream_t st = ctx->st;
  const uint32_t n = ctx->n;
  HIPCHK(hipEventRecord(ctx->ev[2], st));
  ctx->pres = nullptr; ctx->pres_lgb = 0;
  ctx->stats.strand_filter = 0; ctx->stats.strand_filter_dropped = 0; ctx->stats.strand_filter_build = 0;
  uint64_t *uhash[2] = {nullptr, nullptr};
  uint32_t *ustart[2] = {nullptr, nullptr}, *ucount[2] = {nullptr, nullptr};
  const bool both_dense = n && ctx->uniform && ctx->L > ctx->dict[0].end && ctx->L > ctx->dict[1].end;
  uint64_t *keys_both[2] = {nullptr, nullptr};
  uint32_t *vals_both[2] = {nullptr, nullptr};
  ctx->stats.dict_build_path = 0;
  if (both_dense && ctx->pre_keys[0] && ctx->o.dict_build_mode != 1) {
    for (int l = 0; l < 2; l++) {
      keys_both[l] = ctx->pre_keys[l]; vals_both[l] = ctx->pre_vals[l];
      ctx->pre_keys[l] = nullptr; ctx->pre_vals[l] = nullptr;
    }
    ctx->stats.dict_build_path |= 1;
  } else {
    drop_pre_keys(ctx);
  }
  ctx->stats.sort_repaired_runs = 0; ctx->stats.sort_full_sorts = 0; ctx->stats.sort_prefix_bits = 0;
  ctx->stats.sort_long_runs = 0; ctx->stats.sort_list_overflows = 0;
  for (int l = 0; l < 2; l++) {
    DictDev &d = ctx->dict[l];
    uint32_t m = 0;
    uint32_t *d_slot = nullptr, *d_flag = nullptr;
    void *d_tmp = nullptr;
    size_t tmp_bytes = 0;
    if (n) {
      if (ctx->uniform) {
        m = ctx->L > d.end ? n : 0;
      } else {
        DMALLOC(d_flag, (size_t)n * 4);
        DMALLOC(d_slot, (size_t)n * 4);
        launch_flag_in_dict(st, ctx->d_lens, n, d.end, d_flag);
        HIPCHK(excl_scan_u32(st, nullptr, tmp_bytes, d_flag, d_slot, n));
        DMALLOC(d_tmp, tmp_bytes);
        HIPCHK(excl_scan_u32(st, d_tmp, tmp_bytes, d_flag, d_slot, n));
        uint32_t last_slot = 0, last_flag = 0;
        HIPCHK(hipMemcpyAsync(&last_slot, d_slot + (n - 1), 4, hipMemcpyDeviceToHost, st));
        HIPCHK(hipMemcpyAsync(&last_flag, d_flag + (n - 1), 4, hipMemcpyDeviceToHost, st));
        HIPCHK(hipStreamSynchronize(st));
        m = last_slot + last_flag;
        ctx->dfree(d_tmp); d_tmp = nullptr;
      }
    }
    d.numreads = m;
    d.numkeys = 0;
    d.ndeep = 0; d.big_reads = 0; d.mid_reads = 0;
    if (m == 0) {
      DMALLOC(d.urec, 16);
      DMALLOC(d.ids, 16);
      DMALLOC(d.deep, 16);
      DMALLOC(d.d_ndeep, 16);
      HIPCHK(hipMemsetAsync(d.d_ndeep, 0, 12, st));
      if (d_flag) { ctx->dfree(d_flag); ctx->dfree(d_slot); }
      continue;
    }
    uint64_t *k_in = keys_both[l], *k_out = nullptr;
    uint32_t *v_in = vals_both[l], *cnt = nullptr, *d_nruns = nullptr;
    if (!k_in) {
      DMALLOC(k_in, (size_t)m * 8);
      DMALLOC(v_in, (size_t)m * 4);
    }
    DMALLOC(k_out, (size_t)m * 8);
    DMALLOC(d.ids, (size_t)m * 4);
    DBG_T("alloc keys");
    if (l == 0 && both_dense && !keys_both[0]) {
      DMALLOC(keys_both[1], (size_t)n * 8);
      DMALLOC(vals_both[1], (size_t)n * 4);
      launch_keys2(st, ctx->d_reads, n, ctx->S, d.start, d.end, ctx->dict[1].start, ctx->dict[1].end, k_in, v_in,
                   keys_both[1], vals_both[1]);
    } else if (!keys_both[l]) {
      launch_keys(st, ctx->d_reads, ctx->d_lens, ctx->uniform ? nullptr : d_slot, n, ctx->S, d.start, d.end, k_in, v_in);
    }
    HIPCHK(hipGetLastError());
    DBG_T("k_keys");
    const unsigned T = ctx->o.sort_prefix_bits > 0 ? (unsigned)ctx->o.sort_prefix_bits : sort_prefix_auto(m);
    ctx->stats.sort_prefix_bits = T;
    bool full = T >= 64;
    if (!full) {
      uint32_t *d_ctr = nullptr, *d_list = nullptr;
      uint2 *d_runs = nullptr;
      const uint32_t cap = m / 4 + 1024;
      DMALLOC(d_ctr, 16);
      DMALLOC(d_list, (size_t)cap * 4);
      DMALLOC(d_runs, (size_t)cap * 8);
      HIPCHK(hipMemsetAsync(d_ctr, 0, 16, st));
      tmp_bytes = 0;
      HIPCHK(sort_pairs(st, nullptr, tmp_bytes, k_in, k_out, v_in, d.ids, m, 64, 64 - T));
      DMALLOC(d_tmp, tmp_bytes);
      HIPCHK(sort_pairs(st, d_tmp, tmp_bytes, k_in, k_out, v_in, d.ids, m, 64, 64 - T));
      DBG_T("prefix sort");
      launch_sort_repair(st, k_out, d.ids, m, T, d_list, cap, d_ctr, d_runs);
      HIPCHK(hipGetLastError());
      uint32_t ctr[4] = {0, 0, 0, 0};
      HIPCHK(hipMemcpyAsync(ctr, d_ctr, 16, hipMemcpyDeviceToHost, st));
      HIPCHK(hipStreamSynchronize(st));
      full = ctr[0] > cap || ctr[2] != 0;
      if (ctr[0] > cap) ctx->stats.sort_list_overflows++;
      else if (ctr[2]) ctx->stats.sort_long_runs++;
      if (!full) ctx->stats.sort_repaired_runs += ctr[1];
      if (dbg) fprintf(stderr, "[dict] prefix bits %u: %u hash changes inside runs, %u runs re-ordered%s\n", T, ctr[0], ctr[1],
                       full ? " -- not repairable in place: full sort" : "");
      ctx->dfree(d_tmp); d_tmp = nullptr;
      ctx->dfree(d_ctr); ctx->dfree(d_list); ctx->dfree(d_runs);
      DBG_T("sort repair");
    }
    if (full) {
      if (T < 64) ctx->stats.sort_full_sorts++;
      tmp_bytes = 0;
      HIPCHK(sort_pairs(st, nullptr, tmp_bytes, k_in, k_out, v_in, d.ids, m, 64));
      DMALLOC(d_tmp, tmp_bytes);
      HIPCHK(sort_pairs(st, d_tmp, tmp_bytes, k_in, k_out, v_in, d.ids, m, 64));
      DBG_T("sort");
    }
    ctx->dfree(d_tmp); d_tmp = nullptr;
    ctx->dfree(v_in);
    DMALLOC(cnt, (size_t)m * 4);
    DMALLOC(d_nruns, 16);
    tmp_bytes = 0;
    HIPCHK(rle(st, nullptr, tmp_bytes, k_out, m, k_in, cnt, d_nruns));
    DMALLOC(d_tmp, tmp_bytes);
    HIPCHK(rle(st, d_tmp, tmp_bytes, k_out, m, k_in, cnt, d_nruns));
    uint32_t numkeys = 0;
    HIPCHK(hipMemcpyAsync(&numkeys, d_nruns, 4, hipMemcpyDeviceToHost, st));
    HIPCHK(hipStreamSynchronize(st));
    ctx->dfree(d_tmp); d_tmp = nullptr;
    ctx->dfree(k_out); ctx->dfree(d_nruns);
    d.numkeys = numkeys;
    DBG_T("rle");
    DMALLOC(ustart[l], (size_t)numkeys * 4);
    tmp_bytes = 0;
    HIPCHK(excl_scan_u32(st, nullptr, tmp_bytes, cnt, ustart[l], numkeys));
    DMALLOC(d_tmp, tmp_bytes);
    HIPCHK(excl_scan_u32(st, d_tmp, tmp_bytes, cnt, ustart[l], numkeys));
    DBG_T("scan");
    uhash[l] = k_in;
    ucount[l] = cnt;
    DMALLOC(d.urec, (size_t)numkeys * 16);
    DMALLOC(d.deep, ((size_t)m / DEEP_BIN + 1) * 4);
    DMALLOC(d.d_ndeep, 16);
    HIPCHK(hipMemsetAsync(d.d_ndeep, 0, 12, st));
    HIPCHK(hipStreamSynchronize(st));
    ctx->dfree(d_tmp);
    if (d_flag) { ctx->dfree(d_flag); ctx->dfree(d_slot); }
  }
  const uint64_t nk0 = ctx->dict[0].numkeys, nk1 = ctx->dict[1].numkeys, nm = nk0 + nk1;
  const int tab_scale = ctx->o.tab_scale > 0 ? ctx->o.tab_scale : 2;
  const uint64_t nb = std::max<uint64_t>(8, pow2ceil(std::max<uint64_t>(2, (nm * 10 + 15) / 16)) * (uint64_t)pow2ceil(tab_scale));
  ctx->bshift = 64;
  for (uint64_t v = nb; v > 1; v >>= 1) ctx->bshift--;
  ctx->minz = (ctx->dict[0].end - ctx->dict[0].start + 1 == MINZ_WL && ctx->L <= 192 && ctx->o.table_mode == 2) ? 1 : 0;
  ctx->lshift = 32 - (64 - ctx->bshift - 2);
  if (ctx->lshift < 1) return fail(SPRING_REORDER_E_ARG, "build_dict: table too large for minimizer addressing");
  ctx->stats.table_minz = ctx->minz; ctx->stats.table_marked_lines = 0;
  DMALLOC(ctx->fpt, nb * 32);
  const bool one_pass = nm && !ctx->minz && ctx->o.dict_build_mode != 1;
  if (!one_pass) HIPCHK(hipMemsetAsync(ctx->fpt, 0, nb * 32, st));
  uint32_t *const tab_words = reinterpret_cast<uint32_t *>(ctx->fpt);
  DBG_T("alloc+memset tab");
  if (one_pass) {
    if (nm >= 0xffffffffull) return fail(SPRING_REORDER_E_ARG, "build_dict: %llu keys exceed the 32-bit index space of the table build", (unsigned long long)nm);
    ctx->stats.dict_build_path |= 2;
    ctx->marked_lines = 0;
    DictBuild db[2];
    for (int l = 0; l < 2; l++) {
      DictDev &d = ctx->dict[l];
      db[l].ustart = ustart[l]; db[l].ucount = ucount[l]; db[l].ids = d.ids; db[l].urec = d.urec;
      db[l].deep = d.deep; db[l].ndeep = d.d_ndeep;
    }
    uint32_t *d_part = nullptr, *d_ovf = nullptr, *d_ovf_blk = nullptr, *d_ovf_cnt = nullptr, novf = 0;
    const size_t nblk = tab_write_blocks(ctx->bshift);
    DMALLOC(d_part, 2 * (nblk + 1) * 4);
    DMALLOC(d_ovf_blk, nblk * TAB_OVF_SLOTS * 4);
    DMALLOC(d_ovf_cnt, nblk * 4);
    DMALLOC(d_ovf, ((size_t)nm + 1) * 4);
    HIPCHK(hipMemsetAsync(d_ovf, 0, 4, st));
    launch_tab_partition(st, uhash[0], (uint32_t)nk0, uhash[1], (uint32_t)nk1, ctx->bshift, d_part);
    launch_tab_write(st, uhash[0], (uint32_t)nk0, uhash[1], (uint32_t)nk1, d_part, db[0], db[1], ctx->fpt, ctx->bshift, d_ovf,
                     d_ovf_blk, d_ovf_cnt);
    launch_tab_overflow_blocks(st, uhash[0], (uint32_t)nk0, uhash[1], db[0], db[1], tab_words, ctx->bshift, d_ovf_blk, d_ovf_cnt);
    HIPCHK(hipGetLastError());
    HIPCHK(hipMemcpyAsync(&novf, d_ovf, 4, hipMemcpyDeviceToHost, st));
    uint32_t nd[2][3] = {{0, 0, 0}, {0, 0, 0}};
    for (int l = 0; l < 2; l++)
      HIPCHK(hipMemcpyAsync(nd[l], ctx->dict[l].d_ndeep, 12, hipMemcpyDeviceToHost, st));
    HIPCHK(hipStreamSynchronize(st));
    DBG_T("table write");
    launch_tab_overflow_pairs(st, uhash[0], (uint32_t)nk0, uhash[1], db[0], db[1], tab_words, ctx->bshift, d_ovf, novf);
    HIPCHK(hipGetLastError());
    for (int l = 0; l < 2; l++) { ctx->dict[l].ndeep = nd[l][0]; ctx->dict[l].big_reads = nd[l][1]; ctx->dict[l].mid_reads = nd[l][2]; }
    if (dbg) {
      fprintf(stderr, "[dict] %u of %llu pairs past the %u overflow slots of their workgroup\n", novf, (unsigned long long)nm, TAB_OVF_SLOTS);
      fprintf(stderr, "[dict] reads %u + %u, keys %u + %u, bins >= %u: %u + %u, reads in bins >= %u: %u + %u, >= %u: %u + %u\n",
              ctx->dict[0].numreads, ctx->dict[1].numreads, ctx->dict[0].numkeys, ctx->dict[1].numkeys, DEEP_BIN, nd[0][0], nd[1][0],
              MID_BIN, nd[0][2], nd[1][2], BIG_BIN, nd[0][1], nd[1][1]);
    }
    ctx->stats.table_marked_lines = 0;
    ctx->dfree(d_part); ctx->dfree(d_ovf); ctx->dfree(d_ovf_blk); ctx->dfree(d_ovf_cnt);
    DBG_T("overflow");
  } else if (nm) {
    uint64_t *mv0 = nullptr, *mh = nullptr, *mv = nullptr;
    void *d_tmp = nullptr;
    const uint64_t *h_in = nullptr, *v_in = nullptr;
    if (nk0 && nk1) {
      DMALLOC(mh, nm * 8);
      DMALLOC(mv, nm * 8);
      size_t tb = 0;
      HIPCHK(merge_by_hash(st, nullptr, tb, uhash[0], uhash[1], 1ull << 63, mh, mv, nk0, nk1));
      DMALLOC(d_tmp, tb);
      HIPCHK(merge_by_hash(st, d_tmp, tb, uhash[0], uhash[1], 1ull << 63, mh, mv, nk0, nk1));
      h_in = mh; v_in = mv;
    } else {
      DMALLOC(mv0, nm * 8);
      launch_iota_tag(st, mv0, nm, nk0 ? 0ull : 1ull << 63);
      h_in = nk0 ? uhash[0] : uhash[1];
      v_in = mv0;
    }
    DBG_T("merge");
    DictBuild db[2];
    for (int l = 0; l < 2; l++) {
      DictDev &d = ctx->dict[l];
      db[l].ustart = ustart[l]; db[l].ucount = ucount[l]; db[l].ids = d.ids; db[l].urec = d.urec;
      db[l].deep = d.deep; db[l].ndeep = d.d_ndeep;
    }
    uint32_t *bk_in = nullptr, *bk_out = nullptr, *d_marked = nullptr, *d_ovf = nullptr;
    uint64_t *tp_in = nullptr, *tp_out = nullptr;
    ctx->marked_lines = 0;
    void *d_tmp2 = nullptr;
    if (!ctx->minz) {
      ctx->dfree(d_tmp); d_tmp = nullptr;
      if (nm >= 0xffffffffull) return fail(SPRING_REORDER_E_ARG, "build_dict: %llu keys exceed the 32-bit index space of the table build", (unsigned long long)nm);
      uint32_t novf = 0;
      DMALLOC(d_ovf, ((size_t)nm + 1) * 4);
      HIPCHK(hipMemsetAsync(d_ovf, 0, 4, st));
      launch_tab_insert(st, h_in, v_in, nm, db[0], db[1], tab_words, ctx->bshift, d_ovf);
      HIPCHK(hipMemcpyAsync(&novf, d_ovf, 4, hipMemcpyDeviceToHost, st));
      HIPCHK(hipStreamSynchronize(st));
      DBG_T("insert pass 0");
      launch_tab_overflow(st, h_in, v_in, nm, db[0], db[1], tab_words, ctx->bshift, d_ovf, novf);
      if (dbg) fprintf(stderr, "[dict] %u of %llu pairs overflow their bucket\n", novf, (unsigned long long)nm);
    } else {
      DMALLOC(bk_in, nm * 4); DMALLOC(bk_out, nm * 4);
      DMALLOC(tp_in, nm * 8); DMALLOC(tp_out, nm * 8);
      launch_minz_prepare(st, h_in, v_in, nm, db[0], db[1], ctx->lshift, bk_in, tp_in);
      DBG_T("minz prepare");
      const unsigned end_bit = (unsigned)(64 - ctx->bshift);
      size_t tb = 0;
      HIPCHK(sort_pairs_u32_u64(st, nullptr, tb, bk_in, bk_out, tp_in, tp_out, nm, end_bit));
      DMALLOC(d_tmp2, tb);
      HIPCHK(sort_pairs_u32_u64(st, d_tmp2, tb, bk_in, bk_out, tp_in, tp_out, nm, end_bit));
      DBG_T("minz sort");
      DMALLOC(d_marked, 16);
      HIPCHK(hipMemsetAsync(d_marked, 0, 4, st));
      launch_tab_insert_minz(st, bk_out, tp_out, nm, tab_words, ctx->bshift, d_marked);
      HIPCHK(hipMemcpyAsync(&ctx->marked_lines, d_marked, 4, hipMemcpyDeviceToHost, st));
    }
    HIPCHK(hipGetLastError());
    uint32_t nd[2][3] = {{0, 0, 0}, {0, 0, 0}};
    for (int l = 0; l < 2; l++)
      HIPCHK(hipMemcpyAsync(nd[l], ctx->dict[l].d_ndeep, 12, hipMemcpyDeviceToHost, st));
    HIPCHK(hipStreamSynchronize(st));
    for (int l = 0; l < 2; l++) { ctx->dict[l].ndeep = nd[l][0]; ctx->dict[l].big_reads = nd[l][1]; ctx->dict[l].mid_reads = nd[l][2]; }
    if (dbg) fprintf(stderr, "[dict] reads %u + %u, keys %u + %u, bins >= %u: %u + %u, reads in bins >= %u: %u + %u, >= %u: %u + %u\n",
                     ctx->dict[0].numreads, ctx->dict[1].numreads, ctx->dict[0].numkeys, ctx->dict[1].numkeys, DEEP_BIN, nd[0][0], nd[1][0],
                     MID_BIN, nd[0][2], nd[1][2], BIG_BIN, nd[0][1], nd[1][1]);
    ctx->stats.table_marked_lines = ctx->marked_lines;
    DBG_T("insert");
    ctx->dfree(mv0); ctx->dfree(mh); ctx->dfree(mv); ctx->dfree(d_tmp);
    ctx->dfree(bk_in); ctx->dfree(bk_out); ctx->dfree(tp_in); ctx->dfree(tp_out); ctx->dfree(d_tmp2); ctx->dfree(d_marked); ctx->dfree(d_ovf);
  }
  int lgb = 0;
  if (presence_wanted(ctx, nm)) lgb = presence_alloc(ctx, nm, dbg);
  if (ctx->pres) {
    const int wl = ctx->dict[0].end - ctx->dict[0].start + 1;
    uint32_t *d_drops = nullptr, *d_part = nullptr;
    std::vector<uint32_t> h_drops(PRES_DROP_CTRS);
    DMALLOC(d_drops, PRES_DROP_CTRS * 4);
    HIPCHK(hipMemsetAsync(d_drops, 0, PRES_DROP_CTRS * 4, st));
    if (one_pass) {
      DMALLOC(d_part, 2 * ((size_t)pres_write_blocks(lgb) + 1) * 4);
      launch_pres_write(st, uhash[0], (uint32_t)nk0, uhash[1], (uint32_t)nk1, wl, ctx->pres, lgb, d_part, d_drops);
    } else {
      HIPCHK(hipMemsetAsync(ctx->pres, 0, (size_t)16 << lgb, st));
    }
    launch_pres_insert(st, uhash[0], (uint32_t)nk0, uhash[1], (uint32_t)nk1, wl, reinterpret_cast<uint32_t *>(ctx->pres), lgb, d_drops,
                       one_pass);
    HIPCHK(hipGetLastError());
    HIPCHK(hipMemcpyAsync(h_drops.data(), d_drops, PRES_DROP_CTRS * 4, hipMemcpyDeviceToHost, st));
    HIPCHK(hipStreamSynchronize(st));
    for (uint32_t v : h_drops) ctx->stats.strand_filter_dropped += v;
    ctx->pres_lgb = lgb;
    ctx->stats.strand_filter_build = one_pass ? 2 : 1;
    ctx->dfree(d_drops); ctx->dfree(d_part);
    if (dbg) fprintf(stderr, "[dict] presence table: 2^%d buckets%s, %llu of %llu keys dropped\n", lgb, one_pass ? " written once" : "",
                     (unsigned long long)ctx->stats.strand_filter_dropped, (unsigned long long)nm);
    DBG_T("presence table");
  }
  for (int l = 0; l < 2; l++) { ctx->dfree(uhash[l]); ctx->dfree(ustart[l]); ctx->dfree(ucount[l]); }
  DBG_T("free temps");
  HIPCHK(hipEventRecord(ctx->ev[3], st));
  ctx->stage = ST_DICT;
  return 0;
}

int spring_reorder_dict_lookup(spring_reorder_ctx *ctx, int32_t which, const uint64_t *keys, uint32_t nkeys,
                               uint32_t *bin_size, uint32_t *bin_ids, size_t ids_cap) {
  if (!ctx || ctx->stage < ST_DICT) return fail(SPRING_REORDER_E_STATE, "dict_lookup: build_dict first");
  if (which < 0 || which > 1) return fail(SPRING_REORDER_E_ARG, "which must be 0 or 1");
  HIPCHK(hipSetDevice(ctx->dev));
  DictDev &d = ctx->dict[which];
  uint64_t *dk = nullptr;
  uint32_t *ds = nullptr, *dc = nullptr;
  DMALLOC(dk, (size_t)nkeys * 8);
  DMALLOC(ds, (size_t)nkeys * 4);
  DMALLOC(dc, (size_t)nkeys * 4);
  std::vector<uint32_t> hs(nkeys), hc(nkeys), hids(d.numreads);
  if (nkeys) {
    HIPCHK(hipMemcpyAsync(dk, keys, (size_t)nkeys * 8, hipMemcpyHostToDevice, ctx->st));
    launch_dict_lookup(ctx->st, tab_view(ctx), d.urec, which, ctx->d_reads, ctx->S, d.start, d.end, dk, nkeys, ds, dc);
    HIPCHK(hipMemcpyAsync(hs.data(), ds, (size_t)nkeys * 4, hipMemcpyDeviceToHost, ctx->st));
    HIPCHK(hipMemcpyAsync(hc.data(), dc, (size_t)nkeys * 4, hipMemcpyDeviceToHost, ctx->st));
  }
  if (d.numreads) HIPCHK(hipMemcpyAsync(hids.data(), d.ids, (size_t)d.numreads * 4, hipMemcpyDeviceToHost, ctx->st));
  HIPCHK(hipStreamSynchronize(ctx->st));
  ctx->dfree(dk); ctx->dfree(ds); ctx->dfree(dc);
  size_t o = 0;
  for (uint32_t i = 0; i < nkeys; i++) {
    if (hc[i] != 0xffffffffu && (hc[i] & 0x80000000u)) {
      bin_size[i] = 1;
      if (o + 1 > ids_cap) return fail(SPRING_REORDER_E_ARG, "bin_ids too small");
      bin_ids[o++] = hs[i];
      continue;
    }
    bin_size[i] = hc[i];
    if (hc[i] == 0xffffffffu) continue;
    if (o + hc[i] > ids_cap) return fail(SPRING_REORDER_E_ARG, "bin_ids too small");
    memcpy(bin_ids + o, hids.data() + hs[i], (size_t)hc[i] * 4);
    o += hc[i];
  }
  return 0;
}

int spring_reorder_presence_table(spring_reorder_ctx *ctx, void *out, size_t cap, int32_t *lgb) {
  if (!ctx || ctx->stage < ST_DICT) return fail(SPRING_REORDER_E_STATE, "presence_table: build_dict first");
  if (!ctx->pres) return fail(SPRING_REORDER_E_STATE, "presence_table: this build made no presence table");
  const size_t nb = (size_t)16 << ctx->pres_lgb;
  if (lgb) *lgb = ctx->pres_lgb;
  if (!out) return 0;
  if (cap < nb) return fail(SPRING_REORDER_E_ARG, "presence_table: the table has %zu bytes, the buffer %zu", nb, cap);
  HIPCHK(hipSetDevice(ctx->dev));
  HIPCHK(hipMemcpyAsync(out, ctx->pres, nb, hipMemcpyDeviceToHost, ctx->st));
  HIPCHK(hipStreamSynchronize(ctx->st));
  return 0;
}

static bool dict_is_deep(const spring_reorder_ctx *ctx) {
  const uint64_t nd = (uint64_t)ctx->dict[0].numreads + ctx->dict[1].numreads, nk = (uint64_t)ctx->dict[0].numkeys + ctx->dict[1].numkeys;
  return nd * 10 >= nk * 13;
}
static bool dict_has_heavy_tail(const spring_reorder_ctx *ctx) {
  const uint64_t mid = (uint64_t)ctx->dict[0].mid_reads + ctx->dict[1].mid_reads, nd = (uint64_t)ctx->dict[0].numreads + ctx->dict[1].numreads;
  return nd > 0 && mid * 1000 >= nd;
}
static bool dict_is_contended(const spring_reorder_ctx *ctx) {
  const uint64_t mid = (uint64_t)ctx->dict[0].mid_reads + ctx->dict[1].mid_reads, nd = (uint64_t)ctx->dict[0].numreads + ctx->dict[1].numreads;
  return nd > 0 && mid * 4 >= nd;
}
static bool dict_wants_deep_kernel(const spring_reorder_ctx *ctx) {
  const uint64_t nd = (uint64_t)ctx->dict[0].numreads + ctx->dict[1].numreads, nk = (uint64_t)ctx->dict[0].numkeys + ctx->dict[1].numkeys;
  return nd * 100 >= nk * 115 || dict_has_heavy_tail(ctx);
}
static bool dict_is_very_deep(const spring_reorder_ctx *ctx) {
  const uint64_t big = (uint64_t)ctx->dict[0].big_reads + ctx->dict[1].big_reads, nd = (uint64_t)ctx->dict[0].numreads + ctx->dict[1].numreads;
  return dict_is_deep(ctx) && nd > 0 && big * 4 >= nd;
}
static bool ka_layout_ok(const spring_reorder_ctx *ctx, int *ka_lo) {
  if (ctx->Lpad > 192 || ctx->o.known_absent < 0 || ctx->minz) return false;
  const int wlen = ctx->dict[0].end - ctx->dict[0].start + 1, lo = ctx->dict[0].start >> 5;
  if (wlen <= 32 && ctx->dict[1].start == ctx->dict[0].end + 1 && ctx->dict[1].end - ctx->dict[1].start + 1 == wlen &&
      2 * (ctx->L - wlen) + 2 <= 64 * (lo + 4) && 2 * ctx->dict[1].start + 2 <= 256 && lo + 4 <= 6) {
    if (ka_lo) *ka_lo = lo;
    return true;
  }
  return false;
}
static uint32_t auto_chains(uint32_t n, bool deep, bool very_deep, bool heavy_tail);
static bool deep_kernel_chosen(const spring_reorder_ctx *ctx) {
  const spring_reorder_opts &o = ctx->o;
  return (o.deep_bins ? o.deep_bins > 0 : dict_wants_deep_kernel(ctx)) || o.alternatives == 2;
}
static uint32_t group_half(uint32_t Ktot) {
  return (uint32_t)std::max<uint64_t>((((uint64_t)Ktot / 2 + 1024) / 2048) * 2048, 2048);
}
static uint32_t group_nmid(uint32_t n) { return (uint32_t)(((uint64_t)n / 2) >> UBLK_SHIFT << UBLK_SHIFT); }
static bool two_groups_fit(uint32_t n, uint32_t Ktot) {
  const uint32_t half = group_half(Ktot), nmid = group_nmid(n);
  return Ktot >= 4096 && half < Ktot && n < 0x80000000u && nmid > 0 && n >= Ktot;
}
static bool two_groups_pay_shallow(uint32_t Ktot) { return Ktot >= 16384; }
static int groups_wanted(const spring_reorder_opts &o, uint32_t Ktot, bool pays) {
  return o.phases > 0 ? o.phases : (pays && Ktot % 2048 == 0 ? 2 : 1);
}
static bool mc_kernel_chosen(const spring_reorder_ctx *ctx, uint32_t K, int phases, bool ka_ok) {
  if (ctx->o.fused == 2 || 64 - ctx->bshift > 32) return false;
  const uint64_t nd = (uint64_t)ctx->dict[0].numreads + ctx->dict[1].numreads, nk = (uint64_t)ctx->dict[0].numkeys + ctx->dict[1].numkeys;
  const uint32_t mc_min = phases == 2 ? ((ka_ok && nd * 100 < nk * 105) ? 20480u : 32768u) : 49152u;
  return K >= mc_min || ctx->o.fused == 3;
}
static bool strand_filter_wanted(const spring_reorder_ctx *ctx) {
  const spring_reorder_opts &o = ctx->o;
  if (o.strand_filter < 0 || !ka_layout_ok(ctx, nullptr)) return false;
  const bool fused = !o.force_literal_update && o.fused >= 0;
  if (!fused || o.collect_stats || deep_kernel_chosen(ctx)) return false;
  const uint32_t K = o.num_chains ? o.num_chains : auto_chains(ctx->n, dict_is_deep(ctx), dict_is_very_deep(ctx), dict_has_heavy_tail(ctx));
  const int phases = (groups_wanted(o, K, two_groups_pay_shallow(K)) == 2 && two_groups_fit(ctx->n, K)) ? 2 : 1;
  return mc_kernel_chosen(ctx, K, phases, true);
}
static void fill_params(spring_reorder_ctx *ctx, DevParams &P) {
  const spring_reorder_opts &o = ctx->o;
  P.reads = ctx->d_reads; P.lens = ctx->d_lens; P.n = ctx->n;
  P.L = ctx->L; P.W = ctx->W; P.S = ctx->S; P.Lpad = ctx->Lpad;
  P.maxshift = ctx->L / 2;
  memset(P.plan, 0, sizeof(P.plan));
  if (o.first_shifts < 0) { P.plan[0][0] = 4; P.plan[0][1] = 4; P.plan[0][2] = 8; P.plan[0][3] = 8; }
  else if (o.first_shifts > 0) { P.plan[0][0] = std::min(16, o.first_shifts); P.plan[0][1] = 16; }
  else if (o.fused >= 0 && o.fused != 2 && !o.collect_stats && !o.force_literal_update) {
    P.plan[0][0] = 4; P.plan[0][1] = 8; P.plan[0][2] = 16;
  } else { P.plan[0][0] = 8; P.plan[0][1] = 16; }
  P.plan[1][0] = 16; P.plan[1][1] = 16;
  bool user_plan[2] = {false, false};
  for (int w = 0; w < 2; w++) {
    const int32_t *up = w ? o.plan1 : o.plan0;
    if (up[0] <= 0) continue;
    int k = 0, sum = 0;
    int tmp[6] = {0, 0, 0, 0, 0, 0};
    for (; k < 6 && up[k] > 0; k++) {
      if (up[k] > 16 || sum + up[k] > 32) break;
      tmp[k] = up[k]; sum += up[k];
    }
    if (k == 0) continue;
    memcpy(P.plan[w], tmp, sizeof(tmp));
    user_plan[w] = true;
  }
  ctx->user_plan0 = user_plan[0];
  P.seed_wide = o.seed_wide < 0 ? 0 : 1;
  P.search_wpb = (o.search_wpb == 1 || o.search_wpb == 2 || o.search_wpb == 4) ? o.search_wpb : 1;
  P.dbg_search_lds = std::max(0, o.dbg_search_lds);
  P.dbg_apply_lds = std::max(0, o.dbg_apply_lds);
  P.uniform_len = ctx->uniform ? 1 : 0;
  P.wl = ctx->dict[0].end - ctx->dict[0].start + 1;
  for (int l = 0; l < 2; l++) {
    P.dstart[l] = ctx->dict[l].start; P.dend[l] = ctx->dict[l].end; P.numkeys[l] = ctx->dict[l].numkeys;
    P.urec[l] = ctx->dict[l].urec; P.ids[l] = ctx->dict[l].ids;
    P.epos[l] = nullptr;
  }
  P.idmask = 0xffffffffu;
  P.tab = tab_view(ctx);
  P.deep_bins = deep_kernel_chosen(ctx) ? 1 : 0;
  if (P.deep_bins && !dict_is_deep(ctx) && o.first_shifts == 0 && !user_plan[0]) {
    memset(P.plan[0], 0, sizeof(P.plan[0]));
    P.plan[0][0] = 8; P.plan[0][1] = 16;
  }
  if (P.deep_bins && dict_is_deep(ctx) && o.first_shifts == 0 && o.fused >= 0 && !o.collect_stats && !o.force_literal_update &&
      !user_plan[0]) {
    memset(P.plan[0], 0, sizeof(P.plan[0]));
    P.plan[0][0] = 2; P.plan[0][1] = 6; P.plan[0][2] = 8; P.plan[0][3] = 16;
    if (!user_plan[1]) {
      memset(P.plan[1], 0, sizeof(P.plan[1]));
      P.plan[1][0] = 4; P.plan[1][1] = 12; P.plan[1][2] = 16;
    }
  }
  const bool very_deep = P.deep_bins && (dict_is_very_deep(ctx) || (dict_has_heavy_tail(ctx) && !dict_is_deep(ctx)));
  P.long_budget = o.long_budget < 0 ? 0 : (o.long_budget ? o.long_budget : (very_deep ? 8 : 0));
  P.long_blocks = 256;
  P.long_min = P.long_budget < 8 ? 0 : 512;
  if (o.long_min > 0) P.long_min = o.long_min;
  if (o.long_blocks > 0) P.long_blocks = o.long_blocks;
  P.long_part = o.long_split > 0 ? o.long_split : (o.long_split < 0 ? 0 : 192);
  P.longq = nullptr;
  P.lctl = nullptr; P.lparts = nullptr; P.lhead = nullptr; P.lbin = nullptr; P.lbcode = nullptr; P.lbin_stride = 0;
  P.sig[0] = P.sig[1] = nullptr;
}
static uint32_t auto_chains(uint32_t n, bool deep, bool very_deep, bool heavy_tail) {
  uint64_t k = (deep || heavy_tail) ? n >> 7 : n >> 10;
  const uint64_t cap = ((deep && !very_deep) || (heavy_tail && !deep)) ? 131072 : 65536;
  if (k < 1) k = 1;
  if (k > cap) k = cap;
  if (k >= 16384) k &= ~2047ull;
  return (uint32_t)k;
}

static int setup_chains(spring_reorder_ctx *ctx, uint32_t K, uint32_t c0, uint32_t Ktot, bool fused, void *d_prop,
                        bool allow_phases = false) {
  hipStream_t st = ctx->st;
  const uint32_t n = ctx->n;
  ctx->K = K;
  DevParams &P = ctx->P;
  fill_params(ctx, P);
  const uint64_t nublk = std::max<uint64_t>(((uint64_t)n + (1u << UBLK_SHIFT) - 1) >> UBLK_SHIFT, 1);
  const uint64_t nwords = nublk << (UBLK_SHIFT - 6);
  const size_t nn = std::max<uint32_t>(n, 1);
  if (ctx->o.alternatives > 2) return fail(SPRING_REORDER_E_ARG, "alternatives: <= 0 (library's choice), 1 or 2");
  if (ctx->o.phases > 2) return fail(SPRING_REORDER_E_ARG, "phases: <= 0 (library's choice), 1 or 2");
  P.K = K; P.c0 = c0; P.Ktot = Ktot;
  P.fused = fused ? 1 : 0;
  {
    const bool can = fused && P.deep_bins && n < ALT_MAX_READS && Ktot < ALT_KEY;
    const int want = ctx->o.alternatives > 0 ? ctx->o.alternatives : (dict_is_contended(ctx) ? 2 : 1);
    if (ctx->o.alternatives == 2 && !can)
      return fail(SPRING_REORDER_E_ARG, "alternatives = 2 needs the fused round (no literal consensus path, fused >= 0) and a pool of fewer than %u reads", ALT_MAX_READS);
    P.alts = (want == 2 && can) ? 2 : 1;
    ctx->stats.alternatives = (uint64_t)P.alts;
  }
  {
    const uint32_t world = K ? Ktot / K : 1, rank = K ? c0 / K : 0;
    const uint32_t half = group_half(Ktot);
    const uint32_t nmid = group_nmid(n);
    const bool pool_ok = world == 1 ? c0 == 0
                                    : ((uint64_t)K * world == Ktot && half % (MARK_BLOCK * world) == 0 && (Ktot - half) % (MARK_BLOCK * world) == 0);
    const bool can = allow_phases && fused && K > 0 && pool_ok && two_groups_fit(n, Ktot);
    const bool long_kernels = P.deep_bins && P.long_budget > 0;
    const bool pays = P.deep_bins ? (Ktot >= 131072 && P.alts == 1 && !long_kernels) : two_groups_pay_shallow(Ktot);
    const int want = groups_wanted(ctx->o, Ktot, pays);
    if (ctx->o.phases > 2) return fail(SPRING_REORDER_E_ARG, "phases: 0 (library's choice), 1 or 2");
    if (ctx->o.phases == 2 && !can)
      return fail(SPRING_REORDER_E_ARG, "phases = 2 needs the fused round (fused >= 0, no literal consensus path), at least 4096 "
                  "chains and 8192 .. 2^31 - 1 reads, at least as many reads as chains; in a pool over G GPUs both groups' chain "
                  "counts must be multiples of %u x G", MARK_BLOCK);
    P.phases = (want == 2 && can) ? 2 : 1;
    ctx->nmid = nmid;
    if (P.phases == 2) {
      const uint32_t sA = half / world, sB = (Ktot - half) / world;
      ctx->grp[0].g0 = 0; ctx->grp[0].Kg = sA; ctx->grp[0].c0 = rank * sA; ctx->grp[0].gg0 = 0; ctx->grp[0].gKg = half;
      ctx->grp[1].g0 = sA; ctx->grp[1].Kg = sB; ctx->grp[1].c0 = half + rank * sB - sA; ctx->grp[1].gg0 = half; ctx->grp[1].gKg = Ktot - half;
      ctx->Kh = sA;
    } else {
      ctx->grp[0].g0 = 0; ctx->grp[0].Kg = K; ctx->grp[0].c0 = c0; ctx->grp[0].gg0 = 0; ctx->grp[0].gKg = Ktot;
      ctx->grp[1] = spring_reorder_ctx::GroupGeom();
      ctx->grp[1].g0 = K; ctx->grp[1].gg0 = Ktot;
      ctx->Kh = K;
    }
    ctx->stats.phases = (uint64_t)P.phases;
  }
  DMALLOC(P.taken, nwords * 8);
  DMALLOC(P.ublk, nublk * 4);
  DMALLOC(P.resv, nn * 4);
  const size_t needy_bytes = (((size_t)Ktot + 31) / 32 + 255) / 256 * 256 * 4;
  DMALLOC(P.needy, needy_bytes);
  DMALLOC(P.glob, sizeof(Globals));
  P.cursor = &P.glob->cursor;
  DMALLOC(P.chains, (size_t)K * sizeof(Chain));
  DMALLOC(P.cnt, (size_t)K * 2 * ctx->Lpad * sizeof(int4));
  DMALLOC(P.cnt8, (size_t)K * 2 * ctx->Lpad * sizeof(uint32_t) + 64);
  const size_t cap = (size_t)n + (size_t)K * CHUNK;
  if (cap > 0xfffffff0ull) return fail(SPRING_REORDER_E_ARG, "n + K*%u exceeds the 32-bit slot space", CHUNK);
  ctx->cap = cap;
  const size_t nchunk = cap / CHUNK + 2;
  DMALLOC(P.e_rec, cap * sizeof(uint4)); DMALLOC(P.e_chunk, nchunk * sizeof(uint2));
  DMALLOC(P.s_rec, cap * 4); DMALLOC(P.s_chunk, nchunk * sizeof(uint2));
  int ka_lo = 0;
  const bool ka_ok = ka_layout_ok(ctx, &ka_lo);
  P.mc = mc_kernel_chosen(ctx, K, P.phases, ka_ok) ? 1 : 0;
  P.ka = (P.mc && ka_ok) ? 1 : 0;
  P.ka_lo = P.ka ? ka_lo : 0;
  P.sf = (P.ka && ctx->pres && fused && !ctx->o.collect_stats && !P.deep_bins) ? 1 : 0;
  P.pres = P.sf ? ctx->pres : nullptr;
  P.pres_lgb = P.sf ? ctx->pres_lgb : 0;
  ctx->stats.strand_filter = (uint64_t)P.sf;
  if (ctx->minz && !(fused && P.mc && !ctx->o.collect_stats && !P.deep_bins))
// ... 59 lines not shown
        DMALLOC(ctx->lb2.lbin, K1 * P.lbin_stride * sizeof(uint2));
        DMALLOC(ctx->lb2.lbcode, K1 * P.lbin_stride * sizeof(uint16_t));
      }
      for (int l = 0; l < 2; l++) {
        ulonglong2 *sg = nullptr;
        const uint64_t m = ctx->dict[l].numreads;
        DMALLOC(sg, std::max<uint64_t>(m, 1) * sizeof(ulonglong2));
        launch_build_sig(st, ctx->dict[l].ids, m, ctx->d_reads, ctx->S, ctx->W, sg);
        P.sig[l] = sg;
      }
    }
  } else {
    P.ord = nullptr; P.ord_cnt = nullptr;
  }
#ifdef SR_PHASE_TIMING
  DMALLOC(P.dbg, 65 * sizeof(unsigned long long));
  HIPCHK(hipMemsetAsync(P.dbg, 0, 65 * sizeof(unsigned long long), ctx->st));
#endif
  HIPCHK(hipEventRecord(ctx->ev[4], st));
  launch_init_taken(st, P.taken, nwords, n, P.ublk);
  launch_fill_u32(st, P.resv, n, 0xffffffffu);
  HIPCHK(hipMemsetAsync(P.needy, 0, needy_bytes, st));
  HIPCHK(hipMemsetAsync(P.chains, 0, (size_t)K * sizeof(Chain), st));
  Globals g;
  memset(&g, 0, sizeof(g));
  g.cursor = (long long)n - 1;
  g.cursor_b = (long long)ctx->nmid - 1;
  g.e_alloc = g.s_alloc = K * CHUNK;
  g.alive = n == 0 ? 0 : (n / Ktot > 0 ? K : (c0 == 0 ? 1 : 0));
  HIPCHK(hipMemsetAsync(P.e_chunk, 0xff, nchunk * sizeof(uint2), st));
  HIPCHK(hipMemsetAsync(P.s_chunk, 0xff, nchunk * sizeof(uint2), st));
  HIPCHK(hipMemcpyAsync(P.glob, &g, sizeof(g), hipMemcpyHostToDevice, st));
  if (P.phases == 2) {
    for (int g = 0; g < 2; g++) {
      DevParams Q = P;
      const auto &a = ctx->grp[g];
      Q.g0 = a.g0; Q.Kg = a.Kg; Q.c0 = a.c0; Q.gg0 = a.gg0; Q.gKg = a.gKg;
      launch_init_chains(st, Q, g == 0);
    }
    HIPCHK(hipMemcpyAsync(ctx->taken2, P.taken, nwords * 8, hipMemcpyDeviceToDevice, st));
    launch_fill_u32(st, ctx->resv2, n, 0xffffffffu);
    HIPCHK(hipMemsetAsync(ctx->won, 0xff, (size_t)Ktot * 4, st));
  } else launch_init_chains(st, P);
  HIPCHK(hipGetLastError());
  ctx->round_no = 0;
  return 0;
}

static void set_round_buffers(const spring_reorder_ctx *ctx, uint64_t round_no, DevParams &Q) {
  const int w = (int)(round_no & 1);
  Q.needy_cnt = ctx->cnt_buf[w ^ 1];
  Q.needy_cnt_next = ctx->cnt_buf[w];
}

static void trim_deep_bins(const spring_reorder_ctx *ctx, hipStream_t st, const uint64_t *taken) {
  const DevParams &P = ctx->P;
  for (int l = 0; l < 2; l++)
    launch_trim_bins(st, ctx->dict[l].deep, ctx->dict[l].d_ndeep, ctx->dict[l].ndeep, ctx->dict[l].urec, ctx->dict[l].ids, taken, const_cast<ulonglong2 *>(P.sig[l]), P.epos[l]);
}

static int running_chains(spring_reorder_ctx *ctx, std::vector<uint32_t> &buf, uint32_t *alive) {
  const size_t nw = ((size_t)ctx->P.Ktot + 63) / 64;
  buf.resize(nw);
  HIPCHK(hipMemcpyAsync(buf.data(), ctx->P.alive_wave, nw * 4, hipMemcpyDeviceToHost, ctx->st));
  HIPCHK(hipStreamSynchronize(ctx->st));
  uint64_t a = 0;
  for (uint32_t v : buf) a += v;
  *alive = (uint32_t)std::min<uint64_t>(a, 0xffffffffull);
  return 0;
}

static DevParams group_params(spring_reorder_ctx *ctx, int g, uint64_t round_no) {
  DevParams Q = ctx->P;
  const auto &a = ctx->grp[g], &b = ctx->grp[g ^ 1];
  Q.g0 = a.g0; Q.Kg = a.Kg; Q.c0 = a.c0; Q.gg0 = a.gg0; Q.gKg = a.gKg;
  Q.g0_other = b.g0; Q.Kg_other = b.Kg; Q.gKg_other = b.gKg;
  Q.seed_lo = g ? 0u : ctx->nmid; Q.seed_hi = g ? ctx->nmid : ctx->n;
  Q.nb_lo = a.gg0 / 2048; Q.nb_hi = (a.gg0 + a.gKg + 2047) / 2048;
  Q.taken = g ? ctx->taken2 : ctx->P.taken; Q.taken_other = g ? ctx->P.taken : ctx->taken2;
  Q.resv = g ? ctx->resv2 : ctx->P.resv;
  Q.cursor = g ? &ctx->P.glob->cursor_b : &ctx->P.glob->cursor;
  Q.won = ctx->won + a.gg0; Q.won_other = ctx->won + b.gg0;
  if (g == 1 && ctx->P.longq) {
    Q.longq = ctx->lb2.longq; Q.lctl = ctx->lb2.lctl; Q.lparts = ctx->lb2.lparts; Q.lhead = ctx->lb2.lhead;
    Q.lbin = ctx->lb2.lbin; Q.lbcode = ctx->lb2.lbcode;
  }
  set_round_buffers(ctx, round_no, Q);
  return Q;
}

struct AliveLook {
  uint32_t *h_aw = nullptr;
  size_t nw = 0;
  hipEvent_t bev[2] = {nullptr, nullptr};
  int init(RunOwned &own, const DevParams &P) {
    nw = ((size_t)P.Ktot + 63) / 64;
    HIPCHK(own.pin(&h_aw, 2 * nw * sizeof(uint32_t)));
    for (auto &e : bev) HIPCHK(own.event(&e, hipEventDisableTiming));
    return 0;
  }
  int queue(hipStream_t st, const DevParams &P, int slot) const {
    HIPCHK(hipMemcpyAsync(h_aw + (size_t)slot * nw, P.alive_wave, nw * 4, hipMemcpyDeviceToHost, st));
    HIPCHK(hipEventRecord(bev[slot], st));
    return 0;
  }
};

static uint64_t alive_in(const uint32_t *h_aw, size_t nw, int slot) {
  uint64_t a = 0;
  for (size_t i = 0; i < nw; i++) a += h_aw[(size_t)slot * nw + i];
  return a;
}

static double union_ms(std::vector<std::pair<float, float>> &iv) {
  if (iv.empty()) return 0;
  std::sort(iv.begin(), iv.end());
  double busy = 0;
  float cs = iv[0].first, ce = iv[0].second;
  for (size_t i = 1; i < iv.size(); i++) {
    if (iv[i].first > ce) { busy += ce - cs; cs = iv[i].first; ce = iv[i].second; }
    else ce = std::max(ce, iv[i].second);
  }
  return busy + (ce - cs);
}

extern "C++" {
template <class Enqueue, class Count, class After>
static int run_round_loop(const spring_reorder_ctx *ctx, const AliveLook &look, const uint64_t &rounds, bool late, const char *suffix,
                          Enqueue enqueue_batch, Count count_batch, After after_batch) {
  uint64_t a = 0;
  auto running = [&](int slot, uint64_t at) -> int {
    HIPCHK(hipEventSynchronize(look.bev[slot]));
    a = alive_in(look.h_aw, look.nw, slot);
    HIPCHK(hipGetLastError());
    if (ctx->o.debug) fprintf(stderr, "[chains] rounds %llu running %llu%s\n", (unsigned long long)at, (unsigned long long)a, suffix);
    return 0;
  };
  int rr;
  if (!late) {
    do {
      if ((rr = enqueue_batch()) || (rr = count_batch(0)) || (rr = running(0, rounds)) || (rr = after_batch())) return rr;
    } while (a);
    return 0;
  }
  if ((rr = enqueue_batch()) || (rr = count_batch(0))) return rr;
  for (int b = 0;; b ^= 1) {
    const uint64_t at = rounds;
    if ((rr = enqueue_batch()) || (rr = count_batch(b ^ 1)) || (rr = running(b, at))) return rr;
    if (!a) return 0;
  }
}
}

static int run_chains_phased(spring_reorder_ctx *ctx, int R, bool timed) {
  DevParams &P = ctx->P;
  const bool stats = ctx->o.collect_stats != 0;
  if (!ctx->st2) HIPCHK(hipStreamCreateWithFlags(&ctx->st2, hipStreamNonBlocking));
  if (!ctx->st3) HIPCHK(hipStreamCreateWithFlags(&ctx->st3, hipStreamNonBlocking));
  hipStream_t sg[2] = {ctx->st, ctx->st2}, sc = ctx->st3;
  uint64_t round_no[2] = {0, 0};
  RunOwned own;
  SyncOnError sync_guard{{ctx->st2, ctx->st3, ctx->st}};
  constexpr unsigned ORDER_ONLY = hipEventDisableTiming | hipEventDisableSystemFence;
  hipEvent_t ev[2], cev[2], ev0, evt;
  for (int i = 0; i < 2; i++) {
    HIPCHK(own.event(&ev[i], ORDER_ONLY));
    HIPCHK(own.event(&cev[i], hipEventDisableTiming));
  }
  HIPCHK(own.event(&ev0, ORDER_ONLY));
  HIPCHK(own.event(&evt, ORDER_ONLY));
  std::vector<hipEvent_t> tev(timed ? 4 * (size_t)R : 0);
  for (auto &e : tev) HIPCHK(own.event(&e));
  AliveLook look;
  int rr = look.init(own, P);
  if (rr) return rr;
  HIPCHK(hipEventRecord(ev0, sg[0]));
  HIPCHK(hipStreamWaitEvent(sg[1], ev0, 0));
  launch_delay(sg[1], 80);
  bool have_b = false;
  uint64_t rounds = 0, launches = 0;
  double ms_search = 0;
  auto enqueue_batch = [&]() -> int {
    for (int r = 0; r < R; r++) {
      for (int g = 0; g < 2; g++) {
        const DevParams Q = group_params(ctx, g, round_no[g]);
        if (timed) HIPCHK(hipEventRecord(tev[4 * r + 2 * g], sg[g]));
        launch_round(sg[g], Q, stats, false);
        if (timed) HIPCHK(hipEventRecord(tev[4 * r + 2 * g + 1], sg[g]));
        if (g == 1 || have_b) HIPCHK(hipStreamWaitEvent(sg[g], ev[g ^ 1], 0));
        launch_ph_mark(sg[g], Q);
        HIPCHK(hipEventRecord(ev[g], sg[g]));
        round_no[g]++;
      }
      have_b = true;
    }
    for (int g = 0; g < 2; g++) HIPCHK(hipEventRecord(cev[g], sg[g]));
    rounds += R;
    if (P.deep_bins && (ctx->dict[0].ndeep || ctx->dict[1].ndeep)) {
      HIPCHK(hipStreamWaitEvent(sg[0], ev[1], 0));
      trim_deep_bins(ctx, sg[0], P.taken);
      HIPCHK(hipEventRecord(evt, sg[0]));
      HIPCHK(hipStreamWaitEvent(sg[1], evt, 0));
    }
    return 0;
  };
  auto count_batch = [&](int slot) -> int {
    HIPCHK(hipStreamWaitEvent(sc, cev[0], 0));
    HIPCHK(hipStreamWaitEvent(sc, cev[1], 0));
    return look.queue(sc, P, slot);
  };
  double ms_busy = 0;
  auto collect_times = [&]() -> int {
    HIPCHK(hipStreamSynchronize(sg[0]));
    HIPCHK(hipStreamSynchronize(sg[1]));
    std::vector<std::pair<float, float>> iv(2 * (size_t)R);
    for (int i = 0; i < 2 * R; i++) {
      float ms = 0, s0 = 0;
      HIPCHK(hipEventElapsedTime(&ms, tev[2 * i], tev[2 * i + 1]));
      HIPCHK(hipEventElapsedTime(&s0, tev[0], tev[2 * i]));
      ms_search += ms;
      iv[i] = {s0, s0 + ms};
    }
    ms_busy += union_ms(iv);
    launches += 2 * (uint64_t)R;
    return 0;
  };
  if ((rr = run_round_loop(ctx, look, rounds, !timed, " (two groups)", enqueue_batch, count_batch, collect_times))) return rr;
  HIPCHK(hipStreamWaitEvent(sg[0], ev[1], 0));
  HIPCHK(hipEventRecord(ctx->ev[5], sg[0]));
  HIPCHK(hipStreamSynchronize(sg[1]));
  HIPCHK(hipStreamSynchronize(sc));
  HIPCHK(hipStreamSynchronize(sg[0]));
  ctx->round_no = round_no[0];
  ctx->stats.rounds = rounds;
  ctx->stats.ms_search_kernel = ms_search;
  ctx->stats.ms_search_busy = ms_busy;
  ctx->stats.search_launches = launches;
  sync_guard.ok = true;
  return 0;
}

int spring_reorder_auto_chains(spring_reorder_ctx *ctx, uint32_t *chains, int32_t *deep) {
  if (!ctx) return fail(SPRING_REORDER_E_ARG, "ctx is NULL");
  if (ctx->stage < ST_DICT) return fail(SPRING_REORDER_E_STATE, "auto_chains: build_dict first");
  const bool d = dict_is_deep(ctx);
  if (chains) *chains = auto_chains(ctx->n, d, dict_is_very_deep(ctx), dict_has_heavy_tail(ctx));
  if (deep) *deep = d ? 1 : 0;
  return 0;
}

int spring_reorder_run_chains(spring_reorder_ctx *ctx) {
  if (!ctx) return fail(SPRING_REORDER_E_ARG, "ctx is NULL");
  if (ctx->stage != ST_DICT) return fail(SPRING_REORDER_E_STATE, "run_chains: build_dict first");
  HIPCHK(hipSetDevice(ctx->dev));
  hipStream_t st = ctx->st;
  const uint32_t n = ctx->n;
  const uint32_t K = ctx->o.num_chains ? ctx->o.num_chains : auto_chains(n, dict_is_deep(ctx), dict_is_very_deep(ctx), dict_has_heavy_tail(ctx));
  const bool stats = ctx->o.collect_stats != 0;
  const bool timed = ctx->o.time_search != 0;
  const bool literal = ctx->o.force_literal_update != 0;
  const bool fused = !literal && ctx->o.fused >= 0;
  ctx->stats.chains = K;
  ctx->stats.deep_pool = (dict_is_deep(ctx) ? 1 : 0) | (dict_has_heavy_tail(ctx) ? 2 : 0);
  int r0 = setup_chains(ctx, K, 0, K, fused, nullptr, true);
  if (r0) return r0;
  DevParams &P = ctx->P;
  int R = ctx->o.rounds_per_sync > 0 ? ctx->o.rounds_per_sync : (K >= 256 ? 16 : 256);
  if (P.phases == 2) {
    int rp = run_chains_phased(ctx, R, timed);
    if (rp) return rp;
    ctx->stage = ST_CHAINS;
    return 0;
  }
  RunOwned own;
  SyncOnError sync_guard{{st}};
  std::vector<hipEvent_t> tev(timed ? 2 * (size_t)R : 0);
  for (auto &e : tev) HIPCHK(own.event(&e));
  uint32_t *h_alive = nullptr;
  std::vector<uint32_t> alive_tmp;
  HIPCHK(own.pin(&h_alive, sizeof(uint32_t)));
  uint64_t rounds = 0;
  double ms_search = 0;
  uint64_t launches = 0;
  HIPCHK(hipMemcpyAsync(h_alive, &P.glob->alive, 4, hipMemcpyDeviceToHost, st));
  HIPCHK(hipStreamSynchronize(st));
  auto enqueue_batch = [&]() -> int {
    for (int r = 0; r < R; r++) {
      if (timed) HIPCHK(hipEventRecord(tev[2 * r], st));
      if (fused) {
        set_round_buffers(ctx, ctx->round_no, P);
        launch_round(st, P, stats, false);
        if (timed) HIPCHK(hipEventRecord(tev[2 * r + 1], st));
        launch_mg_mark(st, P);
        ctx->round_no++;
      } else {
        launch_search(st, P, stats);
        if (timed) HIPCHK(hipEventRecord(tev[2 * r + 1], st));
        launch_apply(st, P, literal);
      }
    }
    rounds += R;
    trim_deep_bins(ctx, st, P.taken);
    return 0;
  };
  if (fused && !timed && *h_alive) {
    AliveLook look;
    int rr = look.init(own, P);
    if (rr) return rr;
    rr = run_round_loop(ctx, look, rounds, true, "", enqueue_batch, [&](int slot) { return look.queue(st, P, slot); }, [] { return 0; });
    if (rr) return rr;
    *h_alive = 0;
  }
  while (*h_alive) {
    int rr = enqueue_batch();
    if (rr) return rr;
    if (fused) {
      int ra = running_chains(ctx, alive_tmp, h_alive);
      if (ra) return ra;
    } else {
      HIPCHK(hipMemcpyAsync(h_alive, &P.glob->alive, 4, hipMemcpyDeviceToHost, st));
      HIPCHK(hipStreamSynchronize(st));
    }
    HIPCHK(hipGetLastError());
    if (ctx->o.debug) fprintf(stderr, "[chains] rounds %llu running %u\n", (unsigned long long)rounds, *h_alive);
    if (timed) {
      for (int r = 0; r < R; r++) {
        float ms = 0;
        HIPCHK(hipEventElapsedTime(&ms, tev[2 * r], tev[2 * r + 1]));
        ms_search += ms;
      }
      launches += R;
    }
  }
  HIPCHK(hipEventRecord(ctx->ev[5], st));
  HIPCHK(hipStreamSynchronize(st));
  sync_guard.ok = true;
  ctx->stats.rounds = rounds;
  ctx->stats.ms_search_kernel = ms_search;
  ctx->stats.ms_search_busy = ms_search;
  ctx->stats.search_launches = launches;
  ctx->stage = ST_CHAINS;
  return 0;
}

int spring_reorder_mg_begin(spring_reorder_ctx *ctx, uint32_t rank, uint32_t world, uint32_t total_chains,
                            void *d_prop) {
  if (!ctx) return fail(SPRING_REORDER_E_ARG, "ctx is NULL");
  if (ctx->stage != ST_DICT) return fail(SPRING_REORDER_E_STATE, "mg_begin: build_dict first");
  if (world == 0 || rank >= world || total_chains == 0 || total_chains % world)
    return fail(SPRING_REORDER_E_ARG, "mg_begin: total_chains (%u) must be a positive multiple of world (%u)", total_chains, world);
  if (ctx->o.force_literal_update) return fail(SPRING_REORDER_E_ARG, "mg_begin: the literal consensus path only exists in the two-kernel round");
  HIPCHK(hipSetDevice(ctx->dev));
  const uint32_t K = total_chains / world;
  ctx->stats.chains = total_chains;
  ctx->stats.deep_pool = (dict_is_deep(ctx) ? 1 : 0) | (dict_has_heavy_tail(ctx) ? 2 : 0);
  int r = setup_chains(ctx, K, rank * K, total_chains, true, d_prop, true);
  if (r) return r;
  HIPCHK(hipStreamSynchronize(ctx->st));
  ctx->mg = true;
  ctx->stats.rounds = 0;
  return 0;
}

int spring_reorder_mg_search(spring_reorder_ctx *ctx) {
  if (!ctx || !ctx->mg || ctx->stage != ST_DICT) return fail(SPRING_REORDER_E_STATE, "mg_search: mg_begin first");
  HIPCHK(hipSetDevice(ctx->dev));
  if (ctx->P.phases == 2) {
    for (int g = 0; g < 2; g++) launch_round(ctx->st, group_params(ctx, g, ctx->round_no), ctx->o.collect_stats != 0, true);
  } else {
    set_round_buffers(ctx, ctx->round_no, ctx->P);
    launch_round(ctx->st, ctx->P, ctx->o.collect_stats != 0, true);
  }
  HIPCHK(hipGetLastError());
  HIPCHK(hipStreamSynchronize(ctx->st));
  return 0;
}

int spring_reorder_mg_slice(spring_reorder_ctx *ctx, void **d_prop, size_t *slice_off, size_t *slice_bytes,
                            size_t *total_bytes) {
  if (!ctx || !ctx->mg) return fail(SPRING_REORDER_E_STATE, "mg_slice: mg_begin first");
  if (ctx->P.phases == 2) return fail(SPRING_REORDER_E_STATE, "mg_slice: with two chain groups a rank owns two slices of the proposal words: ask mg_slices");
  if (d_prop) *d_prop = ctx->P.prop;
  if (slice_off) *slice_off = (size_t)ctx->P.c0 * 8;
  if (slice_bytes) *slice_bytes = (size_t)ctx->P.K * 8;
  if (total_bytes) *total_bytes = (size_t)ctx->P.Ktot * 8;
  return 0;
}

int spring_reorder_mg_slices(spring_reorder_ctx *ctx, void **d_prop, size_t *slice_off, size_t *slice_bytes,
                             size_t *total_bytes, uint32_t *count) {
  if (!ctx || !ctx->mg) return fail(SPRING_REORDER_E_STATE, "mg_slices: mg_begin first");
  const uint32_t ns = ctx->P.phases == 2 ? 2u : 1u;
  if (d_prop) *d_prop = ctx->P.prop;
  for (uint32_t g = 0; g < 2; g++) {
    const auto &a = ctx->grp[g];
    if (slice_off) slice_off[g] = g < ns ? ((size_t)a.c0 + a.g0) * 8 : 0;
    if (slice_bytes) slice_bytes[g] = g < ns ? (size_t)a.Kg * 8 : 0;
  }
  if (total_bytes) *total_bytes = (size_t)ctx->P.Ktot * 8;
  if (count) *count = ns;
  return 0;
}

int spring_reorder_mg_apply(spring_reorder_ctx *ctx, int32_t check_alive, uint32_t *alive) {
  if (!ctx || !ctx->mg || ctx->stage != ST_DICT) return fail(SPRING_REORDER_E_STATE, "mg_apply: mg_begin first");
  HIPCHK(hipSetDevice(ctx->dev));
  hipStream_t st = ctx->st;
  if (ctx->P.phases == 2) {
    for (int g = 0; g < 2; g++) {
      const DevParams Q = group_params(ctx, g, ctx->round_no);
      launch_mg_resolve(st, Q);
      launch_ph_mark(st, Q);
    }
  } else {
    launch_mg_resolve(st, ctx->P);
    launch_mg_mark(st, ctx->P);
  }
  HIPCHK(hipGetLastError());
  ctx->round_no++;
  ctx->stats.rounds++;
  if (ctx->stats.rounds % 16 == 0) trim_deep_bins(ctx, st, ctx->P.taken);
  if (check_alive) {
    uint32_t a = 0;
    std::vector<uint32_t> tmp;
    int ra = running_chains(ctx, tmp, &a);
    if (ra) return ra;
    if (alive) *alive = a;
  }
  return 0;
}

int spring_reorder_mg_end(spring_reorder_ctx *ctx) {
  if (!ctx || !ctx->mg || ctx->stage != ST_DICT) return fail(SPRING_REORDER_E_STATE, "mg_end: mg_begin first");
  HIPCHK(hipSetDevice(ctx->dev));
  HIPCHK(hipEventRecord(ctx->ev[5], ctx->st));
  HIPCHK(hipStreamSynchronize(ctx->st));
  ctx->stage = ST_CHAINS;
  return 0;
}

int spring_reorder_debug_check_seed_state(spring_reorder_ctx *ctx, int32_t group, uint64_t *violations ) {
  if (!ctx || !ctx->mg || ctx->stage != ST_DICT || !violations) return fail(SPRING_REORDER_E_STATE, "debug_check_seed_state: between mg_begin and mg_end");
  const int ng = ctx->P.phases == 2 ? 2 : 1;
  if (group < 0 || group >= ng) return fail(SPRING_REORDER_E_ARG, "debug_check_seed_state: group %d, the chains run as %d group(s)", group, ng);
  HIPCHK(hipSetDevice(ctx->dev));
  const DevParams Q = ng == 2 ? group_params(ctx, group, ctx->round_no) : ctx->P;
  unsigned long long *d_bad = nullptr;
  DMALLOC(d_bad, 16);
  HIPCHK(hipMemsetAsync(d_bad, 0, 16, ctx->st));
  const uint64_t nwords = (((uint64_t)ctx->n + (1ull << UBLK_SHIFT) - 1) >> UBLK_SHIFT) << (UBLK_SHIFT - 6);
  const uint64_t hi = Q.seed_hi >= ctx->n ? nwords * 64 : Q.seed_hi;
  launch_check_seed_state(ctx->st, Q, nwords, hi, d_bad);
  unsigned long long h[2] = {0, 0};
  HIPCHK(hipMemcpyAsync(h, d_bad, 16, hipMemcpyDeviceToHost, ctx->st));
  HIPCHK(hipStreamSynchronize(ctx->st));
  ctx->dfree(d_bad);
  violations[0] = h[0]; violations[1] = h[1];
  return 0;
}

int spring_reorder_mg_exchange_virtual(spring_reorder_ctx **ctxs, uint32_t world) {
  if (!ctxs || !world) return fail(SPRING_REORDER_E_ARG, "bad arguments");
  for (uint32_t d = 0; d < world; d++) {
    spring_reorder_ctx *dc = ctxs[d];
    if (!dc || !dc->mg) return fail(SPRING_REORDER_E_STATE, "exchange_virtual: mg_begin first");
    HIPCHK(hipSetDevice(dc->dev));
    for (uint32_t s2 = 0; s2 < world; s2++) {
      if (s2 == d) continue;
      spring_reorder_ctx *sc = ctxs[s2];
      if (sc->P.prop == dc->P.prop) continue;
      for (int g = 0; g < 2; g++) {
        const auto &a = sc->grp[g];
        if (!a.Kg) continue;
        const size_t o = (size_t)a.c0 + a.g0;
        HIPCHK(hipMemcpyAsync(dc->P.prop + o, sc->P.prop + o, (size_t)a.Kg * 8, hipMemcpyDeviceToDevice, dc->st));
      }
    }
  }
  for (uint32_t d = 0; d < world; d++) HIPCHK(hipStreamSynchronize(ctxs[d]->st));
  return 0;
}

int spring_mg_rccl_unique_id(void *id128) {
  if (!id128) return fail(SPRING_REORDER_E_ARG, "id buffer is NULL");
  int r = rccl_load();
  if (r) return r;
  const int e = g_rccl.GetUniqueId(id128);
  if (e) return fail(SPRING_REORDER_E_HIP, "ncclGetUniqueId: %s", rccl_err(e));
  return 0;
}

int spring_mg_comm_create_rccl(spring_mg_comm **out, int32_t device, const void *id128, uint32_t rank, uint32_t world) {
  if (!out || !id128 || !world || rank >= world) return fail(SPRING_REORDER_E_ARG, "comm_create_rccl: bad arguments");
  int r = rccl_load();
  if (r) return r;
  int dev = device;
  if (dev < 0) HIPCHK(hipGetDevice(&dev));
  HIPCHK(hipSetDevice(dev));
  RcclId128 id;
  memcpy(id.b, id128, sizeof(id.b));
  void *comm = nullptr;
  const int e = g_rccl.CommInitRank(&comm, (int)world, id, (int)rank);
  if (e) return fail(SPRING_REORDER_E_HIP, "ncclCommInitRank: %s", rccl_err(e));
  spring_mg_comm *c = new spring_mg_comm();
  c->rank = rank; c->world = world; c->dev = dev; c->rccl = comm;
// ... 84 lines not shown
          const int e = g_rccl.AllGather(mine, grange, a.Kg, RCCL_UINT64, comm->rccl, sx);
          if (e) return fail(SPRING_REORDER_E_HIP, "ncclAllGather: %s", rccl_err(e));
          if (timed) HIPCHK(hipEventRecord(tev[8 * r + 4 * g + 2], sx));
          HIPCHK(hipEventRecord(ex[g], sx));
          HIPCHK(hipStreamWaitEvent(sg[g], ex[g], 0));
        } else {
          const size_t off = (size_t)(a.c0 + a.g0 - a.gg0) * 8, slice = (size_t)a.Kg * 8;
          HIPCHK(hipMemcpyAsync(h_stage + off, mine, slice, hipMemcpyDeviceToHost, sg[g]));
          HIPCHK(hipStreamSynchronize(sg[g]));
          if (comm->host_fn(h_stage, off, slice, gbytes[g], comm->host_user))
            return fail(SPRING_REORDER_E_IO, "mg_run: the caller's all-gather reported an error");
          HIPCHK(hipMemcpyAsync(grange, h_stage, gbytes[g], hipMemcpyHostToDevice, sg[g]));
          HIPCHK(hipStreamSynchronize(sg[g]));
          if (timed) HIPCHK(hipEventRecord(tev[8 * r + 4 * g + 2], sg[g]));
        }
        launch_mg_resolve(sg[g], Q);
        if (g == 1 || have_b) HIPCHK(hipStreamWaitEvent(sg[g], ev[g ^ 1], 0));
        launch_ph_mark(sg[g], Q);
        if (timed) HIPCHK(hipEventRecord(tev[8 * r + 4 * g + 3], sg[g]));
        HIPCHK(hipEventRecord(ev[g], sg[g]));
        round_no[g]++;
      }
      have_b = true;
    }
    rounds += R;
    if (P.deep_bins && (ctx->dict[0].ndeep || ctx->dict[1].ndeep)) {
      HIPCHK(hipStreamWaitEvent(sg[0], ev[1], 0));
      trim_deep_bins(ctx, sg[0], P.taken);
      HIPCHK(hipEventRecord(ev0, sg[0]));
      HIPCHK(hipStreamWaitEvent(sg[1], ev0, 0));
    }
    return 0;
  };
  auto count_batch = [&](int slot) -> int {
    HIPCHK(hipStreamWaitEvent(sx, ev[0], 0));
    HIPCHK(hipStreamWaitEvent(sx, ev[1], 0));
    return look.queue(sx, P, slot);
  };
  auto after_batch = [&]() -> int {
    HIPCHK(hipStreamSynchronize(sg[0]));
    HIPCHK(hipStreamSynchronize(sg[1]));
    if (!timed) return 0;
    std::vector<std::pair<float, float>> iv(2 * (size_t)R);
    for (int i = 0; i < 2 * R; i++) {
      float a = 0, b = 0, c = 0, s0 = 0;
      HIPCHK(hipEventElapsedTime(&a, tev[4 * i], tev[4 * i + 1]));
      HIPCHK(hipEventElapsedTime(&b, tev[4 * i + 1], tev[4 * i + 2]));
      HIPCHK(hipEventElapsedTime(&c, tev[4 * i + 2], tev[4 * i + 3]));
      HIPCHK(hipEventElapsedTime(&s0, tev[0], tev[4 * i]));
      ms_round += a; ms_xchg += b; ms_mark += c;
      iv[(size_t)i] = {s0, s0 + a};
    }
    ms_busy += union_ms(iv);
    timed_rounds += (uint64_t)R;
    return 0;
  };
  const bool late = !(timed || comm->host_fn);
  if ((rr = run_round_loop(ctx, look, rounds, late, " (pool, two groups)", enqueue_batch, count_batch, after_batch))) return rr;
  HIPCHK(hipStreamWaitEvent(sg[0], ev[1], 0));
  HIPCHK(hipStreamSynchronize(sg[1]));
  HIPCHK(hipStreamSynchronize(sx));
  HIPCHK(hipStreamSynchronize(sg[0]));
  ctx->round_no = round_no[0];
  ctx->stats.rounds = rounds;
  if (timed) {
    ctx->stats.ms_search_kernel = ms_round; ctx->stats.ms_search_busy = ms_busy; ctx->stats.search_launches = 2 * timed_rounds;
    ctx->stats.ms_exchange = ms_xchg; ctx->stats.ms_resolve_mark = ms_mark;
  }
  sync_guard.ok = true;
  return 0;
}

static int mg_run_one_group(spring_reorder_ctx *ctx, spring_mg_comm *comm) {
  hipStream_t st = ctx->st;
  DevParams &P = ctx->P;
  const bool stats = ctx->o.collect_stats != 0;
  const int R = ctx->o.rounds_per_sync > 0 ? ctx->o.rounds_per_sync : 8;
  const size_t slice = (size_t)P.K * 8, total = (size_t)P.Ktot * 8;
  RunOwned own;
  SyncOnError sync_guard{{st}};
  char *h_stage = nullptr;
  if (comm->host_fn) HIPCHK(own.pin(&h_stage, total));
  const bool timed = ctx->o.time_search != 0;
  std::vector<hipEvent_t> tev(timed ? 4 * (size_t)R : 0);
  for (auto &e : tev) HIPCHK(own.event(&e));
  double ms_round = 0, ms_xchg = 0, ms_mark = 0;
  uint64_t timed_rounds = 0;
  uint32_t alive = 1;
  std::vector<uint32_t> alive_tmp;
  while (alive) {
    for (int i = 0; i < R; i++) {
      set_round_buffers(ctx, ctx->round_no, P);
      if (timed) HIPCHK(hipEventRecord(tev[4 * i], st));
      launch_round(st, P, stats, true);
      if (timed) HIPCHK(hipEventRecord(tev[4 * i + 1], st));
      if (comm->rccl) {
        const int e = g_rccl.AllGather(P.prop + P.c0, P.prop, P.K, RCCL_UINT64, comm->rccl, st);
        if (e) return fail(SPRING_REORDER_E_HIP, "ncclAllGather: %s", rccl_err(e));
      } else {
        HIPCHK(hipMemcpyAsync(h_stage + (size_t)P.c0 * 8, P.prop + P.c0, slice, hipMemcpyDeviceToHost, st));
        HIPCHK(hipStreamSynchronize(st));
        if (comm->host_fn(h_stage, (size_t)P.c0 * 8, slice, total, comm->host_user))
          return fail(SPRING_REORDER_E_IO, "mg_run: the caller's all-gather reported an error");
        HIPCHK(hipMemcpyAsync(P.prop, h_stage, total, hipMemcpyHostToDevice, st));
      }
      if (timed) HIPCHK(hipEventRecord(tev[4 * i + 2], st));
      launch_mg_resolve(st, P);
      launch_mg_mark(st, P);
      if (timed) HIPCHK(hipEventRecord(tev[4 * i + 3], st));
      ctx->round_no++;
      ctx->stats.rounds++;
      if (ctx->stats.rounds % 16 == 0) trim_deep_bins(ctx, st, P.taken);
    }
    if (timed) {
      HIPCHK(hipStreamSynchronize(st));
      for (int i = 0; i < R; i++) {
        float a = 0, b = 0, c = 0;
        HIPCHK(hipEventElapsedTime(&a, tev[4 * i], tev[4 * i + 1]));
        HIPCHK(hipEventElapsedTime(&b, tev[4 * i + 1], tev[4 * i + 2]));
        HIPCHK(hipEventElapsedTime(&c, tev[4 * i + 2], tev[4 * i + 3]));
        ms_round += a; ms_xchg += b; ms_mark += c;
      }
      timed_rounds += (uint64_t)R;
    }
    const int ra = running_chains(ctx, alive_tmp, &alive);
    if (ra) return ra;
    HIPCHK(hipGetLastError());
  }
  if (timed) {
    ctx->stats.ms_search_kernel = ms_round; ctx->stats.ms_search_busy = ms_round; ctx->stats.search_launches = timed_rounds;
    ctx->stats.ms_exchange = ms_xchg; ctx->stats.ms_resolve_mark = ms_mark;
  }
  sync_guard.ok = true;
  return 0;
}

int spring_reorder_mg_run(spring_reorder_ctx *ctx, spring_mg_comm *comm, uint32_t total_chains) {
  if (!ctx || !comm) return fail(SPRING_REORDER_E_ARG, "mg_run: NULL argument");
  if (comm->rccl && comm->dev != ctx->dev)
    return fail(SPRING_REORDER_E_ARG, "mg_run: the communicator lives on device %d, the context on %d", comm->dev, ctx->dev);
  int r = spring_reorder_mg_begin(ctx, comm->rank, comm->world, total_chains, nullptr);
  if (r) return r;
  const int rr = ctx->P.phases == 2 ? mg_run_phased(ctx, comm) : mg_run_one_group(ctx, comm);
  const std::string keep = g_err;
  const int re = spring_reorder_mg_end(ctx);
  if (rr) { g_err = keep; return rr; }
  return re;
}

int spring_reorder_finalize(spring_reorder_ctx *ctx) {
  if (!ctx) return fail(SPRING_REORDER_E_ARG, "ctx is NULL");
  if (ctx->stage != ST_CHAINS) return fail(SPRING_REORDER_E_STATE, "finalize: run_chains first");
  HIPCHK(hipSetDevice(ctx->dev));
  hipStream_t st = ctx->st;
  DevParams &P = ctx->P;
  const uint32_t K = ctx->K;
  const int T = ctx->o.num_thr;
  HIPCHK(hipEventRecord(ctx->ev[6], st));
  std::vector<uint2> hs(std::max<uint32_t>(K, 1));
  unsigned long long htot[8] = {0, 0, 0, 0, 0, 0, 0, 0};
  Globals g;
  {
    uint2 *d_sum = nullptr;
    unsigned long long *d_tot = nullptr;
    DMALLOC(d_sum, (size_t)std::max<uint32_t>(K, 1) * sizeof(uint2));
    DMALLOC(d_tot, 64);
    HIPCHK(hipMemsetAsync(d_tot, 0, 64, st));
    launch_chain_summary(st, P, d_sum, d_tot);
    HIPCHK(hipGetLastError());
    if (K) HIPCHK(hipMemcpyAsync(hs.data(), d_sum, (size_t)K * sizeof(uint2), hipMemcpyDeviceToHost, st));
    HIPCHK(hipMemcpyAsync(htot, d_tot, 64, hipMemcpyDeviceToHost, st));
    HIPCHK(hipMemcpyAsync(&g, P.glob, sizeof(g), hipMemcpyDeviceToHost, st));
    HIPCHK(hipStreamSynchronize(st));
    ctx->dfree(d_sum); ctx->dfree(d_tot);
  }
#ifdef SR_PHASE_TIMING
  std::vector<Chain> hc(K);
  if (K) HIPCHK(hipMemcpy(hc.data(), P.chains, (size_t)K * sizeof(Chain), hipMemcpyDeviceToHost));
#endif
  std::vector<uint64_t> off_m(K), off_s(K);
  ctx->tid_off.assign(T + 1, 0);
  ctx->tid_off_s.assign(T + 1, 0);
  uint64_t am = 0, as = 0;
  spring_reorder_stats &s = ctx->stats;
  s.unmatched = s.probes = s.keyok = s.cands = s.iterations = s.lost = s.hits = 0;
  ctx->tid_mid.assign(T, 0);
  ctx->tid_mid_s.assign(T, 0);
  for (int t = 0; t < T; t++) {
    ctx->tid_off[t] = am;
    ctx->tid_off_s[t] = as;
    for (int g = 0; g < 2; g++) {
      const auto &a = ctx->grp[g];
      if (g == 1) { ctx->tid_mid[t] = am; ctx->tid_mid_s[t] = as; }
      if (!a.Kg) continue;
      const uint32_t first = (uint32_t)(((uint32_t)t + (uint32_t)T - (a.c0 + a.g0) % (uint32_t)T) % (uint32_t)T);
      for (uint32_t i = a.g0 + first; i < a.g0 + a.Kg; i += (uint32_t)T) {
        off_m[i] = am; off_s[i] = as;
        am += hs[i].x; as += hs[i].y;
      }
    }
  }
  ctx->tid_off[T] = am;
  ctx->tid_off_s[T] = as;
  s.unmatched = htot[0]; s.probes = htot[1]; s.keyok = htot[2]; s.cands = htot[3]; s.iterations = htot[4];
  s.lost = htot[5]; s.hits = htot[6]; s.long_searches = htot[7];
  s.table_minz = ctx->minz; s.table_marked_lines = ctx->marked_lines;
#ifdef SR_PHASE_TIMING
  {
    unsigned long long pt[64] = {0};
    for (uint32_t i = 0; i < K; i++)
      for (int k = 0; k < 64; k++) pt[k] += hc[i].pt[k];
    unsigned long long tot = 0;
    for (int k = 0; k < 32; k++) tot += pt[k];
    fprintf(stderr, "[phase] bucket: total clocks (share of buckets 0-11), visits, clocks per visit\n");
    for (int k = 0; k < 32; k++)
      if (pt[32 + k])
        fprintf(stderr, "[phase] %2d: %16llu (%5.1f %%) %12llu %9.0f\n", k, pt[k], 100.0 * (double)pt[k] / (double)std::max(tot, 1ull),
                pt[32 + k], (double)pt[k] / (double)pt[32 + k]);
    unsigned long long dbg[65];
    HIPCHK(hipMemcpy(dbg, P.dbg, sizeof(dbg), hipMemcpyDeviceToHost));
    fprintf(stderr, "[phase] %llu wavefronts ran > 1M clocks; their buckets (clocks/visits):", dbg[64]);
    for (int k = 0; k < 32; k++)
      if (dbg[32 + k]) fprintf(stderr, " %d:%llu/%llu", k, dbg[k], dbg[32 + k]);
    fprintf(stderr, "\n");
    std::vector<std::pair<unsigned long long, uint32_t>> top;
    for (uint32_t i = 0; i < K; i++) {
      unsigned long long t = 0;
      for (int k = 0; k < 32; k++) t += hc[i].pt[k];
      top.push_back({t, i});
    }
    std::partial_sort(top.begin(), top.begin() + std::min<size_t>(3, top.size()), top.end(), std::greater<>());
    for (size_t j = 0; j < std::min<size_t>(3, top.size()); j++) {
      fprintf(stderr, "[phase] chain %u: %llu clocks:", top[j].second, top[j].first);
      for (int k = 0; k < 32; k++)
        if (hc[top[j].second].pt[32 + k]) fprintf(stderr, " %d:%u/%u", k, hc[top[j].second].pt[k], hc[top[j].second].pt[32 + k]);
      fprintf(stderr, "\n");
    }
  }
#endif
  if ((!ctx->mg && am + as != ctx->n) || am + as > ctx->n || g.e_alloc > ctx->cap + CHUNK || g.s_alloc > ctx->cap + CHUNK)
    return fail(SPRING_REORDER_E_STATE, "internal: emission counts do not add up (%llu+%llu vs n=%u, alloc %u/%u cap %llu)",
                (unsigned long long)am, (unsigned long long)as, ctx->n, g.e_alloc, g.s_alloc,
                (unsigned long long)ctx->cap);
  ctx->nrec = am;
  ctx->nsing = as;
  s.n_reads = ctx->n; s.n_matched = am; s.n_single = as;
  const size_t nm = std::max<uint64_t>(am, 1), ns = std::max<uint64_t>(as, 1);
  DMALLOC(P.f_order, nm * 4); DMALLOC(P.f_rc, nm); DMALLOC(P.f_flag, nm); DMALLOC(P.f_pos, nm * 8);
  DMALLOC(P.f_len, nm * 2); DMALLOC(P.f_order_s, ns * 4);
  uint64_t *d_off_m = nullptr, *d_off_s = nullptr;
  DMALLOC(d_off_m, (size_t)K * 8);
  DMALLOC(d_off_s, (size_t)K * 8);
  HIPCHK(hipMemcpyAsync(d_off_m, off_m.data(), (size_t)K * 8, hipMemcpyHostToDevice, st));
  HIPCHK(hipMemcpyAsync(d_off_s, off_s.data(), (size_t)K * 8, hipMemcpyHostToDevice, st));
  launch_scatter(st, P, am ? ctx->cap : 0, as ? ctx->cap : 0, d_off_m, d_off_s);
  HIPCHK(hipGetLastError());
  HIPCHK(hipEventRecord(ctx->ev[7], st));
  HIPCHK(hipStreamSynchronize(st));
  s.long_splits = 0;
  if (P.lctl) {
    uint32_t ns = 0;
    HIPCHK(hipMemcpy(&ns, P.lctl + 3, 4, hipMemcpyDeviceToHost));
    s.long_splits = ns;
    if (P.phases == 2 && ctx->lb2.lctl) {
      HIPCHK(hipMemcpy(&ns, ctx->lb2.lctl + 3, 4, hipMemcpyDeviceToHost));
      s.long_splits += ns;
    }
  }
  ctx->dfree(d_off_m); ctx->dfree(d_off_s);
  ctx->dfree(P.e_rec); ctx->dfree(P.e_chunk); ctx->dfree(P.s_rec); ctx->dfree(P.s_chunk);
  P.e_rec = nullptr;
  ctx->stage = ST_FINAL;
  return 0;
}

int spring_reorder_tid_split(spring_reorder_ctx *ctx, uint64_t *mid, uint64_t *mid_s) {
  if (!ctx || ctx->stage != ST_FINAL) return fail(SPRING_REORDER_E_STATE, "tid_split: finalize first");
  const int T = (int)ctx->tid_mid.size();
  for (int t = 0; t < T; t++) {
    if (mid) mid[t] = ctx->tid_mid[t];
    if (mid_s) mid_s[t] = ctx->tid_mid_s[t];
  }
  return 0;
}

int spring_reorder_get_stats(spring_reorder_ctx *ctx, spring_reorder_stats *out) {
  if (!ctx || !out) return fail(SPRING_REORDER_E_ARG, "NULL argument");
  HIPCHK(hipSetDevice(ctx->dev));
  HIPCHK(hipStreamSynchronize(ctx->st));
  spring_reorder_stats &s = ctx->stats;
  auto el = [&](int a, int b) {
    float ms = 0;
    if (hipEventElapsedTime(&ms, ctx->ev[a], ctx->ev[b]) != hipSuccess) ms = 0;
    return (double)ms;
  };
  if (ctx->stage >= ST_LOADED) s.ms_unpack = el(0, 1);
  if (ctx->stage >= ST_DICT) s.ms_dict = el(2, 3);
  if (ctx->stage >= ST_CHAINS) s.ms_chains = el(4, 5);
  if (ctx->stage >= ST_FINAL) s.ms_finalize = el(6, 7);
  s.ms_total = s.ms_unpack + s.ms_dict + s.ms_chains + s.ms_finalize;
  for (int l = 0; l < 2; l++) { s.numkeys[l] = ctx->dict[l].numkeys; s.dict_numreads[l] = ctx->dict[l].numreads; }
  s.n_reads = ctx->n;
  s.device_bytes = ctx->peak_bytes;
  *out = s;
  return 0;
}

int spring_reorder_download(spring_reorder_ctx *ctx, uint32_t *order, char *rc, char *flag, int64_t *pos,
                            uint16_t *rlen, uint32_t *order_s, uint64_t *tid_off, uint64_t *tid_off_s) {
  if (!ctx || ctx->stage != ST_FINAL) return fail(SPRING_REORDER_E_STATE, "download: finalize first");
  HIPCHK(hipSetDevice(ctx->dev));
  DevParams &P = ctx->P;
  const size_t nm = ctx->nrec, ns = ctx->nsing;
  std::vector<D2HJob> jobs;
  if (nm) {
    if (order) jobs.push_back({order, P.f_order, nm * 4});
    if (rc) jobs.push_back({rc, P.f_rc, nm});
    if (flag) jobs.push_back({flag, P.f_flag, nm});
    if (pos) jobs.push_back({pos, P.f_pos, nm * 8});
    if (rlen) jobs.push_back({rlen, P.f_len, nm * 2});
  }
  if (ns && order_s) jobs.push_back({order_s, P.f_order_s, ns * 4});
  const int rd = download_chunked(ctx, jobs);
  if (rd) return rd;
  if (tid_off) memcpy(tid_off, ctx->tid_off.data(), ctx->tid_off.size() * 8);
  if (tid_off_s) memcpy(tid_off_s, ctx->tid_off_s.data(), ctx->tid_off_s.size() * 8);
  return 0;
}

extern "C++" {
namespace sr {
int emit_dna_device(spring_reorder_ctx *ctx, int32_t tid, uint8_t **d_out, size_t *nbytes, uint64_t s_first, uint64_t s_cnt, size_t *mid_bytes) {
  if (!ctx || ctx->stage != ST_FINAL) return fail(SPRING_REORDER_E_STATE, "emit_dna: finalize first");
  if (tid < -1 || tid >= ctx->o.num_thr) return fail(SPRING_REORDER_E_ARG, "tid out of range");
  HIPCHK(hipSetDevice(ctx->dev));
  hipStream_t st = ctx->st;
  DevParams &P = ctx->P;
  const uint32_t *order;
  const char *rc;
  uint64_t cnt;
  if (tid < 0) {
    order = P.f_order_s; rc = nullptr; cnt = ctx->nsing;
    if (s_cnt != ~0ull) {
      if (s_first > cnt || s_cnt > cnt - s_first) return fail(SPRING_REORDER_E_ARG, "emit_dna: singleton range out of bounds");
      order += s_first; cnt = s_cnt;
    }
  } else {
    const uint64_t a = ctx->tid_off[tid], b = ctx->tid_off[tid + 1];
    order = P.f_order + a; rc = P.f_rc + a; cnt = b - a;
  }
  const uint32_t rec = 2u + ((uint32_t)ctx->L + 3u) / 4u;
  uint64_t total = 0;
  uint64_t *d_off = nullptr;
  uint32_t *d_sz = nullptr;
  void *d_tmp = nullptr;
  if (ctx->uniform) total = cnt * rec;
  else if (cnt) {
    DMALLOC(d_sz, cnt * 4);
    DMALLOC(d_off, cnt * 8);
    launch_rec_size(st, order, ctx->d_lens, cnt, d_sz);
    size_t tb = 0;
    HIPCHK(excl_scan_u32_to_u64(st, nullptr, tb, d_sz, d_off, cnt));
    DMALLOC(d_tmp, tb);
    HIPCHK(excl_scan_u32_to_u64(st, d_tmp, tb, d_sz, d_off, cnt));
    uint64_t last_off = 0;
    uint32_t last_sz = 0;
    HIPCHK(hipMemcpyAsync(&last_off, d_off + (cnt - 1), 8, hipMemcpyDeviceToHost, st));
    HIPCHK(hipMemcpyAsync(&last_sz, d_sz + (cnt - 1), 4, hipMemcpyDeviceToHost, st));
    HIPCHK(hipStreamSynchronize(st));
    total = last_off + last_sz;
  }
  if (mid_bytes) {
    const uint64_t idx = tid >= 0 ? ctx->tid_mid[tid] - ctx->tid_off[tid] : 0;
    if (ctx->uniform || idx == 0) *mid_bytes = idx * rec;
    else if (idx >= cnt) *mid_bytes = total;
    else {
      uint64_t o = 0;
      HIPCHK(hipMemcpyAsync(&o, d_off + idx, 8, hipMemcpyDeviceToHost, st));
      HIPCHK(hipStreamSynchronize(st));
      *mid_bytes = o;
    }
  }
  if (nbytes) *nbytes = total;
  if (d_out) {
    *d_out = nullptr;
    if (total) {
      uint8_t *d_dst = nullptr;
      DMALLOC(d_dst, total);
      launch_emit_dna(st, ctx->d_reads, ctx->d_lens, ctx->S, order, rc, cnt, d_off, rec, d_dst);
      HIPCHK(hipGetLastError());
      *d_out = d_dst;
    }
  }
  ctx->dfree(d_sz); ctx->dfree(d_off); ctx->dfree(d_tmp);
  return 0;
}
void emit_dna_free(spring_reorder_ctx *ctx, uint8_t *d) { if (ctx && d) ctx->dfree(d); }
}
}

int spring_reorder_emit_dna(spring_reorder_ctx *ctx, int32_t tid, uint8_t *dst, size_t cap, size_t *nbytes) {
  size_t total = 0;
  uint8_t *d = nullptr;
  int r = emit_dna_device(ctx, tid, dst ? &d : nullptr, &total);
  if (r) return r;
  if (nbytes) *nbytes = total;
  if (dst && total) {
    if (cap < total) r = fail(SPRING_REORDER_E_ARG, "emit_dna: buffer too small (%zu < %llu)", cap, (unsigned long long)total);
    else if (hipStreamSynchronize(ctx->st) != hipSuccess || hipMemcpy(dst, d, total, hipMemcpyDeviceToHost) != hipSuccess)
      r = fail(SPRING_REORDER_E_HIP, "emit_dna: device to host copy failed");
  }
  emit_dna_free(ctx, d);
  return r;
}

}
```

### spring_amd/reorder.py

```python
import ctypes as C
from dataclasses import dataclass

import numpy as np

from . import _lib
from ._stage import ReorderError, chk as _chk


@dataclass
class ReorderOpts:
    device: int = -1
    num_chains: int = 0
    num_thr: int = 1
    collect_stats: bool = False
    time_search: bool = False
    force_literal_update: bool = False
    rounds_per_sync: int = 0
    first_shifts: int = 0
    seed_wide: int = 0
    tab_scale: int = 0
    search_wpb: int = 0
    dbg_search_lds: int = 0
    dbg_apply_lds: int = 0
    fused: int = 0
    deep_bins: int = 0
    long_budget: int = 0
    devices: tuple = ()
    mg_host_transport: bool = False
    plan0: tuple = ()
    plan1: tuple = ()
    long_min: int = 0
    long_blocks: int = 0
    entry_flags: int = 0
    long_split: int = 0
    debug: bool = False
    out_writers: int = 0
    alternatives: int = 0
    table_mode: int = 0
    phases: int = 0
    known_absent: int = 0
    sort_prefix_bits: int = 0
    dict_build_mode: int = 0
    strand_filter: int = 0

    def to_c(self):
        o = _lib.Opts()
        _lib.lib().spring_reorder_default_opts(C.byref(o))
        o.device, o.num_chains, o.num_thr = self.device, self.num_chains, self.num_thr
        o.collect_stats, o.time_search = int(self.collect_stats), int(self.time_search)
        o.force_literal_update, o.rounds_per_sync = int(self.force_literal_update), self.rounds_per_sync
        o.first_shifts, o.seed_wide, o.tab_scale = self.first_shifts, self.seed_wide, self.tab_scale
        o.search_wpb, o.dbg_search_lds, o.dbg_apply_lds = self.search_wpb, self.dbg_search_lds, self.dbg_apply_lds
        o.fused, o.deep_bins = self.fused, self.deep_bins
        o.long_budget = self.long_budget
        if len(self.devices) > 8:
            raise ValueError("at most 8 devices")
        o.table_mode = self.table_mode
        for i, v in enumerate(tuple(self.plan0)[:6]):
            o.plan0[i] = int(v)
        for i, v in enumerate(tuple(self.plan1)[:6]):
            o.plan1[i] = int(v)
        o.long_min, o.long_blocks, o.debug = self.long_min, self.long_blocks, int(self.debug)
        o.long_split, o.entry_flags = self.long_split, self.entry_flags
        o.out_writers = self.out_writers
        o.alternatives = self.alternatives
        o.phases = self.phases
        o.known_absent = self.known_absent
        o.sort_prefix_bits = self.sort_prefix_bits
        o.dict_build_mode = self.dict_build_mode
        o.strand_filter = self.strand_filter
        o.num_devices = len(self.devices)
        for i, d in enumerate(self.devices):
            o.devices[i] = d
        o.mg_host_transport = int(self.mg_host_transport)
        return o


class ReorderStage:

    def __init__(self, opts: ReorderOpts = None):
        self.opts = opts or ReorderOpts()
        self._L = _lib.lib()
        self._h = C.c_void_p()
        _chk(self._L.spring_reorder_create(C.byref(self._h), C.byref(self.opts.to_c())))
        self.n = 0
        self.max_readlen = 0

    def close(self):
        if self._h:
            self._L.spring_reorder_destroy(self._h)
            self._h = C.c_void_p()

    def __enter__(self):
        return self

    def __exit__(self, *a):
        self.close()

    def __del__(self):
        try:
            self.close()
        except Exception:
            pass

    def load_dna(self, dna: bytes, n: int, max_readlen: int):
        buf = np.frombuffer(dna, dtype=np.uint8)
        _chk(self._L.spring_reorder_load_dna(self._h, buf.ctypes.data if len(buf) else None, len(buf), n,
                                             max_readlen))
        self.n, self.max_readlen = n, max_readlen

    def load_dna_device(self, dptr: int, nbytes: int, n: int, max_readlen: int, fixed_len: bool):
        _chk(self._L.spring_reorder_load_dna_device(self._h, C.c_void_p(dptr), nbytes, n, max_readlen,
                                                    int(fixed_len)))
        self.n, self.max_readlen = n, max_readlen

    def load_synth(self, n, L, G, seed, err_ppm=10000):
        _chk(self._L.spring_reorder_load_synth(self._h, n, L, G, seed, err_ppm))
        self.n, self.max_readlen = n, L

    def load_fastq(self, fastq_1: bytes, fastq_2: bytes = None):
        a = np.frombuffer(fastq_1, dtype=np.uint8)
        b = np.frombuffer(fastq_2, dtype=np.uint8) if fastq_2 is not None else None
        info = _lib.FastqInfo()
        _chk(self._L.spring_reorder_load_fastq(
            self._h, a.ctypes.data if len(a) else None, len(a),
            (b.ctypes.data if len(b) else C.c_void_p(1)) if b is not None else None, len(b) if b is not None else 0,
            C.byref(info)))
        self.n = info.num_reads_clean[0] + info.num_reads_clean[1]
        self.max_readlen = max(int(info.max_readlen), 1)
        return dict(num_reads=list(info.num_reads), num_reads_clean=list(info.num_reads_clean),
                    num_reads_N=list(info.num_reads_N), max_readlen=int(info.max_readlen),
                    ms_device=float(info.ms_device))

    def fastq_N(self, which=0):
        nb, cnt = C.c_size_t(), C.c_uint32()
        _chk(self._L.spring_reorder_fastq_N(self._h, which, None, 0, C.byref(nb), None, C.byref(cnt)))
        buf = np.zeros(max(nb.value, 1), np.uint8)
        order = np.zeros(max(cnt.value, 1), np.uint32)
        _chk(self._L.spring_reorder_fastq_N(self._h, which, buf.ctypes.data, nb.value, C.byref(nb), order.ctypes.data,
                                            C.byref(cnt)))
        return buf[:nb.value].tobytes(), order[:cnt.value]

    def build_dict(self):
        _chk(self._L.spring_reorder_build_dict(self._h))

    def run_chains(self):
        _chk(self._L.spring_reorder_run_chains(self._h))

    def auto_chains(self):
        k, d = C.c_uint32(0), C.c_int32(0)
        _chk(self._L.spring_reorder_auto_chains(self._h, C.byref(k), C.byref(d)))
        return k.value, bool(d.value)

    def finalize(self):
        _chk(self._L.spring_reorder_finalize(self._h))

    def run(self):
        self.build_dict()
        self.run_chains()
        self.finalize()
        return self

    def stats(self):
        s = _lib.Stats()
        _chk(self._L.spring_reorder_get_stats(self._h, C.byref(s)))
        return s.asdict()

    def streams(self):
        st = self.stats()
        nm, ns, T = st["n_matched"], st["n_single"], self.opts.num_thr
        out = dict(order=np.zeros(max(nm, 1), np.uint32), rc=np.zeros(max(nm, 1), np.uint8),
                   flag=np.zeros(max(nm, 1), np.uint8), pos=np.zeros(max(nm, 1), np.int64),
                   rlen=np.zeros(max(nm, 1), np.uint16), order_s=np.zeros(max(ns, 1), np.uint32),
                   tid_off=np.zeros(T + 1, np.uint64), tid_off_s=np.zeros(T + 1, np.uint64))
        _chk(self._L.spring_reorder_download(self._h, *[out[k].ctypes.data for k in (
            "order", "rc", "flag", "pos", "rlen", "order_s", "tid_off", "tid_off_s")]))
        for k in ("order", "rc", "flag", "pos", "rlen"):
            out[k] = out[k][:nm]
        out["order_s"] = out["order_s"][:ns]
        out["tid_mid"], out["tid_mid_s"] = np.zeros(T, np.uint64), np.zeros(T, np.uint64)
        _chk(self._L.spring_reorder_tid_split(self._h, out["tid_mid"].ctypes.data, out["tid_mid_s"].ctypes.data))
        out["stats"] = st
        return out

    def emit_dna(self, tid: int) -> bytes:
        nb = C.c_size_t()
        _chk(self._L.spring_reorder_emit_dna(self._h, tid, None, 0, C.byref(nb)))
        buf = np.zeros(max(nb.value, 1), np.uint8)
        _chk(self._L.spring_reorder_emit_dna(self._h, tid, buf.ctypes.data, nb.value, C.byref(nb)))
        return buf[:nb.value].tobytes()

    def dict_lookup(self, which, keys):
        keys = np.ascontiguousarray(keys, dtype=np.uint64)
        sizes = np.zeros(max(len(keys), 1), np.uint32)
        ids = np.zeros(max(self.n, 1) * 2, np.uint32)
        _chk(self._L.spring_reorder_dict_lookup(self._h, which, keys.ctypes.data, len(keys), sizes.ctypes.data,
                                                ids.ctypes.data, len(ids)))
        return sizes[:len(keys)], ids

    def presence_table(self):
        lgb = C.c_int32(0)
        _chk(self._L.spring_reorder_presence_table(self._h, None, 0, C.byref(lgb)))
        slots = np.zeros((1 << lgb.value, 4), np.uint32)
        _chk(self._L.spring_reorder_presence_table(self._h, slots.ctypes.data, slots.nbytes, C.byref(lgb)))
        return lgb.value, slots

    def download_reads(self):
        W = (2 * self.max_readlen - 1) // 64 + 1
        limbs = np.zeros((max(self.n, 1), W), np.uint64)
        ln = np.zeros(max(self.n, 1), np.uint16)
        _chk(self._L.spring_reorder_download_reads(self._h, limbs.ctypes.data, ln.ctypes.data))
        return limbs[:self.n], ln[:self.n]

    def download_dna(self) -> bytes:
        nb = self._L.spring_synth_dna_bytes(self.n, self.max_readlen)
        buf = np.zeros(max(nb, 1), np.uint8)
        _chk(self._L.spring_reorder_download_dna(self._h, buf.ctypes.data, nb))
        p = 0
        for _ in range(self.n):
            p += 2 + ((int(buf[p]) | (int(buf[p + 1]) << 8)) + 3) // 4
        return buf[:p].tobytes()


# ... 43 lines not shown
```

Measured before the change: 377.7 Mreads/s.

## Overlap presence-table build with early rounds, widen sort digits, custom unique pass

Three changes to the dictionary build and the rounds that follow it. The presence table is now built on a side stream, and the first chain rounds run without the strand filter sweep until the build finishes. The prefix radix sort moves to a 10-bit-digit onesweep config. The rocprim run-length encode is replaced by custom tile-count, scan and write kernels that emit unique hashes, starts and counts directly. The costs are more sync complexity, filter-less early rounds that may do extra work, and a host sync to read numkeys.

```diff
diff --git a/include/spring_reorder.h b/include/spring_reorder.h
--- a/include/spring_reorder.h
+++ b/include/spring_reorder.h
@@ -50,6 +50,8 @@
   int32_t sort_prefix_bits;
   int32_t dict_build_mode;
   int32_t strand_filter;
+  int32_t sort_digit_bits;
+  int32_t presence_overlap;
 } spring_reorder_opts;
 
 typedef struct {
@@ -79,6 +81,9 @@
   uint64_t strand_filter;
   uint64_t strand_filter_dropped;
   uint64_t strand_filter_build;
+  uint64_t presence_overlap;
+  uint64_t presence_plain_rounds;
+  uint64_t sort_digit_bits;
 } spring_reorder_stats;
 
 void spring_reorder_default_opts(spring_reorder_opts *o);
diff --git a/spring_amd/_lib.py b/spring_amd/_lib.py
--- a/spring_amd/_lib.py
+++ b/spring_amd/_lib.py
@@ -112,7 +112,8 @@
                 ("table_mode", C.c_int32), ("plan0", C.c_int32 * 6), ("plan1", C.c_int32 * 6), ("long_min", C.c_int32),
                 ("long_blocks", C.c_int32), ("debug", C.c_int32), ("long_split", C.c_int32), ("entry_flags", C.c_int32),
                 ("out_writers", C.c_int32), ("alternatives", C.c_int32), ("phases", C.c_int32), ("known_absent", C.c_int32),
-                ("sort_prefix_bits", C.c_int32), ("dict_build_mode", C.c_int32), ("strand_filter", C.c_int32)]
+                ("sort_prefix_bits", C.c_int32), ("dict_build_mode", C.c_int32), ("strand_filter", C.c_int32),
+                ("sort_digit_bits", C.c_int32), ("presence_overlap", C.c_int32)]
 
 
 class Info(C.Structure):
@@ -211,7 +212,8 @@
                    ("sort_prefix_bits", C.c_uint64), ("sort_repaired_runs", C.c_uint64), ("sort_full_sorts", C.c_uint64),
                    ("sort_long_runs", C.c_uint64), ("sort_list_overflows", C.c_uint64), ("dict_build_path", C.c_uint64),
                    ("strand_filter", C.c_uint64), ("strand_filter_dropped", C.c_uint64),
-                   ("strand_filter_build", C.c_uint64)])
+                   ("strand_filter_build", C.c_uint64), ("presence_overlap", C.c_uint64),
+                   ("presence_plain_rounds", C.c_uint64), ("sort_digit_bits", C.c_uint64)])
 
 
 NOT_INT = {"spring_reorder_last_error": C.c_char_p, "spring_synth_dna_bytes": C.c_size_t,
diff --git a/spring_amd/csrc/dict_build.h b/spring_amd/csrc/dict_build.h
--- a/spring_amd/csrc/dict_build.h
+++ b/spring_amd/csrc/dict_build.h
@@ -8,6 +8,15 @@
 bool launch_unpack_keys(hipStream_t st, const uint8_t *dna, uint32_t n, int L, int W, int S, uint32_t rec_fixed,
                         uint64_t *reads, uint16_t *lens, uint32_t *bad_len, int dstart0, int dend0, int dstart1, int dend1,
                         uint64_t *keys0, uint32_t *vals0, uint64_t *keys1, uint32_t *vals1);
+
+constexpr uint32_t UNIQ_TILE = 2048;
+inline uint32_t uniq_tiles(uint64_t m) { return (uint32_t)((m + UNIQ_TILE - 1) / UNIQ_TILE); }
+void launch_unique_count(hipStream_t st, const uint64_t *h, uint32_t m, uint32_t *tcnt, uint32_t *tfirst, uint32_t *numkeys);
+void launch_unique_write(hipStream_t st, const uint64_t *h, uint32_t m, const uint32_t *tcnt, const uint32_t *tfirst,
+                         uint64_t *uhash, uint32_t *ustart, uint32_t *ucount);
+
+hipError_t sort_pairs_wide(hipStream_t st, void *tmp, size_t &tmp_bytes, const uint64_t *kin, uint64_t *kout,
+                           const uint32_t *vin, uint32_t *vout, size_t n, unsigned end_bit, unsigned begin_bit);
 
 constexpr int TAB_WRITE_LG = 10;
 inline int tab_write_lg(int bshift) { return 64 - bshift < TAB_WRITE_LG ? 64 - bshift : TAB_WRITE_LG; }
diff --git a/spring_amd/csrc/dict_build.hip b/spring_amd/csrc/dict_build.hip
--- a/spring_amd/csrc/dict_build.hip
+++ b/spring_amd/csrc/dict_build.hip
@@ -1,4 +1,6 @@
+#include <cstring>
 #include <hip/hip_runtime.h>
+#include <rocprim/rocprim.hpp>
 
 #include "dict_build.h"
 #include "strand_filter.h"
@@ -100,6 +102,142 @@
                      rec_fixed, reads, lens, bad_len, dstart0, dend0 - dstart0 + 1, dstart1, dend1 - dstart1 + 1, keys0, vals0,
                      keys1, vals1);
   return true;
+}
+
+constexpr uint32_t UNIQ_THREADS = 256, UNIQ_ROWS = 8, UNIQ_WAVES = UNIQ_THREADS / 64;
+static_assert(UNIQ_THREADS * UNIQ_ROWS == UNIQ_TILE, "a tile is 8 rows of 64 per wavefront");
+constexpr uint32_t UNIQ_NONE = 0xffffffffu;
+
+__device__ __forceinline__ void uniq_rows(const uint64_t *__restrict__ h, uint64_t m, uint64_t base, uint32_t lane,
+                                          unsigned long long (&v)[UNIQ_ROWS], unsigned long long (&mask)[UNIQ_ROWS]) {
+  unsigned long long before = (base && base <= m) ? h[base - 1] : 0ull;
+#pragma unroll
+  for (uint32_t k = 0; k < UNIQ_ROWS; k++) {
+    const uint64_t i = base + 64u * k + lane;
+    const bool valid = i < m;
+    const unsigned long long x = valid ? h[i] : 0ull;
+    unsigned long long p = __shfl_up(x, 1);
+    if (lane == 0u) p = before;
+    mask[k] = __ballot(valid && (i == 0u || x != p));
+    before = __shfl(x, 63);
+    v[k] = x;
+  }
+}
+
+__global__ __launch_bounds__(UNIQ_THREADS) void k_uniq_count(const uint64_t *__restrict__ h, uint32_t m,
+                                                             uint32_t *__restrict__ tcnt, uint32_t *__restrict__ tfirst) {
+  __shared__ uint32_t s_cnt[UNIQ_WAVES], s_first[UNIQ_WAVES];
+  const uint32_t lane = threadIdx.x & 63u, w = threadIdx.x >> 6;
+  const uint64_t base = (uint64_t)blockIdx.x * UNIQ_TILE + (uint64_t)w * (64u * UNIQ_ROWS);
+  unsigned long long v[UNIQ_ROWS], mask[UNIQ_ROWS];
+  uniq_rows(h, m, base, lane, v, mask);
+  uint32_t cnt = 0, first = UNIQ_NONE;
+#pragma unroll
+  for (uint32_t k = 0; k < UNIQ_ROWS; k++) {
+    if (first == UNIQ_NONE && mask[k]) first = (uint32_t)(base + 64u * k) + (uint32_t)(__ffsll(mask[k]) - 1);
+    cnt += (uint32_t)__popcll(mask[k]);
+  }
+  if (lane == 0u) { s_cnt[w] = cnt; s_first[w] = first; }
+  __syncthreads();
+  if (threadIdx.x == 0u) {
+    uint32_t c = 0, f = UNIQ_NONE;
+    for (uint32_t j = 0; j < UNIQ_WAVES; j++) {
+      c += s_cnt[j];
+      if (f == UNIQ_NONE) f = s_first[j];
+    }
+    tcnt[blockIdx.x] = c;
+    tfirst[blockIdx.x] = f;
+  }
+}
+
+constexpr uint32_t UNIQ_SCAN_THREADS = 1024;
+__global__ __launch_bounds__(UNIQ_SCAN_THREADS) void k_uniq_scan(uint32_t *__restrict__ tcnt, uint32_t *__restrict__ tfirst,
+                                                                 uint32_t ntiles, uint32_t m, uint32_t *__restrict__ numkeys) {
+  __shared__ uint32_t s_sum[UNIQ_SCAN_THREADS], s_min[UNIQ_SCAN_THREADS];
+  const uint32_t t = threadIdx.x, per = (ntiles + UNIQ_SCAN_THREADS - 1) / UNIQ_SCAN_THREADS;
+  const uint32_t lo = min(t * per, ntiles), hi = min(lo + per, ntiles);
+  uint32_t sum = 0, mn = UNIQ_NONE;
+#pragma unroll 8
+  for (uint32_t j = lo; j < hi; j++) { sum += tcnt[j]; mn = min(mn, tfirst[j]); }
+  s_sum[t] = sum; s_min[t] = mn;
+  __syncthreads();
+  for (uint32_t d = 1; d < UNIQ_SCAN_THREADS; d <<= 1) {
+    const uint32_t a = t >= d ? s_sum[t - d] : 0u, b = t + d < UNIQ_SCAN_THREADS ? s_min[t + d] : UNIQ_NONE;
+    __syncthreads();
+    s_sum[t] += a; s_min[t] = min(s_min[t], b);
+    __syncthreads();
+  }
+  uint32_t run = s_sum[t] - sum;
+  uint32_t nxt = min(t + 1 < UNIQ_SCAN_THREADS ? s_min[t + 1] : UNIQ_NONE, m);
+#pragma unroll 8
+  for (uint32_t j = lo; j < hi; j++) { const uint32_t c = tcnt[j]; tcnt[j] = run; run += c; }
+#pragma unroll 8
+  for (uint32_t j = hi; j > lo; j--) { nxt = min(nxt, tfirst[j - 1]); tfirst[j - 1] = nxt; }
+  if (t == UNIQ_SCAN_THREADS - 1) { *numkeys = s_sum[t]; tfirst[ntiles] = m; }
+}
+
+__global__ __launch_bounds__(UNIQ_THREADS) void k_uniq_write(const uint64_t *__restrict__ h, uint32_t m,
+                                                             const uint32_t *__restrict__ toff, const uint32_t *__restrict__ tnext,
+                                                             uint64_t *__restrict__ uhash, uint32_t *__restrict__ ustart,
+                                                             uint32_t *__restrict__ ucount) {
+  __shared__ uint32_t s_cnt[UNIQ_WAVES], s_first[UNIQ_WAVES];
+  const uint32_t lane = threadIdx.x & 63u, w = threadIdx.x >> 6;
+  const uint64_t base = (uint64_t)blockIdx.x * UNIQ_TILE + (uint64_t)w * (64u * UNIQ_ROWS);
+  unsigned long long v[UNIQ_ROWS], mask[UNIQ_ROWS];
+  uniq_rows(h, m, base, lane, v, mask);
+  uint32_t cnt = 0, first = UNIQ_NONE;
+#pragma unroll
+  for (uint32_t k = 0; k < UNIQ_ROWS; k++) {
+    if (first == UNIQ_NONE && mask[k]) first = (uint32_t)(base + 64u * k) + (uint32_t)(__ffsll(mask[k]) - 1);
+    cnt += (uint32_t)__popcll(mask[k]);
+  }
+  if (lane == 0u) { s_cnt[w] = cnt; s_first[w] = first; }
+  __syncthreads();
+  if (!cnt) return;
+  uint32_t rank = toff[blockIdx.x];
+  for (uint32_t j = 0; j < w; j++) rank += s_cnt[j];
+  uint32_t after = UNIQ_NONE;
+  for (uint32_t j = w + 1; j < UNIQ_WAVES; j++)
+    if (after == UNIQ_NONE) after = s_first[j];
+  if (after == UNIQ_NONE) after = tnext[blockIdx.x + 1];
+  uint32_t rownext[UNIQ_ROWS];
+#pragma unroll
+  for (int k = UNIQ_ROWS - 1; k >= 0; k--) {
+    rownext[k] = after;
+    if (mask[k]) after = (uint32_t)(base + 64u * k) + (uint32_t)(__ffsll(mask[k]) - 1);
+  }
+#pragma unroll
+  for (uint32_t k = 0; k < UNIQ_ROWS; k++) {
+    const unsigned long long mk = mask[k];
+    if ((mk >> lane) & 1ull) {
+      const uint32_t i = (uint32_t)(base + 64u * k) + lane;
+      const uint32_t r = rank + (uint32_t)__popcll(mk & ((1ull << lane) - 1ull));
+      const unsigned long long rest = (mk >> lane) >> 1;
+      const uint32_t nx = rest ? i + (uint32_t)__ffsll(rest) : rownext[k];
+      uhash[r] = v[k];
+      ustart[r] = i;
+      ucount[r] = nx - i;
+    }
+    rank += (uint32_t)__popcll(mk);
+  }
+}
+
+void launch_unique_count(hipStream_t st, const uint64_t *h, uint32_t m, uint32_t *tcnt, uint32_t *tfirst, uint32_t *numkeys) {
+  const uint32_t ntiles = uniq_tiles(m);
+  hipLaunchKernelGGL(k_uniq_count, dim3(ntiles), dim3(UNIQ_THREADS), 0, st, h, m, tcnt, tfirst);
+  hipLaunchKernelGGL(k_uniq_scan, dim3(1), dim3(UNIQ_SCAN_THREADS), 0, st, tcnt, tfirst, ntiles, m, numkeys);
+}
+void launch_unique_write(hipStream_t st, const uint64_t *h, uint32_t m, const uint32_t *tcnt, const uint32_t *tfirst,
+                         uint64_t *uhash, uint32_t *ustart, uint32_t *ucount) {
+  hipLaunchKernelGGL(k_uniq_write, dim3(uniq_tiles(m)), dim3(UNIQ_THREADS), 0, st, h, m, tcnt, tfirst, uhash, ustart, ucount);
+}
+
+hipError_t sort_pairs_wide(hipStream_t st, void *tmp, size_t &tmp_bytes, const uint64_t *kin, uint64_t *kout,
+                           const uint32_t *vin, uint32_t *vout, size_t n, unsigned end_bit, unsigned begin_bit) {
+  using onesweep = rocprim::radix_sort_onesweep_config<rocprim::kernel_config<1024, 8>, rocprim::kernel_config<1024, 6>, 10,
+                                                       rocprim::block_radix_rank_algorithm::match>;
+  return rocprim::radix_sort_pairs<rocprim::radix_sort_config<rocprim::default_config, rocprim::default_config, onesweep, 0>>(
+      tmp, tmp_bytes, kin, kout, vin, vout, n, begin_bit, end_bit, st);
 }
 
 __global__ void k_tab_partition(const uint64_t *__restrict__ h0, uint32_t nk0, const uint64_t *__restrict__ h1, uint32_t nk1,
diff --git a/spring_amd/csrc/reorder_pipeline.cpp b/spring_amd/csrc/reorder_pipeline.cpp
--- a/spring_amd/csrc/reorder_pipeline.cpp
+++ b/spring_amd/csrc/reorder_pipeline.cpp
@@ -128,6 +128,13 @@
   uint32_t marked_lines = 0;
   uint4 *pres = nullptr;
   int pres_lgb = 0;
+  struct PresSide {
+    bool pending = false;
+    hipEvent_t done = nullptr;
+    uint64_t *uhash[2] = {nullptr, nullptr};
+    uint32_t *d_drops = nullptr, *d_part = nullptr, *h_drops = nullptr;
+    uint64_t nm = 0;
+  } side;
   bool user_plan0 = false;
   DevParams P;
   uint32_t K = 0;
@@ -344,6 +351,10 @@
     return fail(SPRING_REORDER_E_ARG, "dict_build_mode: 0 (library's choice) or 1 (key pass, memset, merge and insert passes)");
   if (o.strand_filter < -1 || o.strand_filter > 32)
     return fail(SPRING_REORDER_E_ARG, "strand_filter: 0 (library's choice), -1 (off) or 1 .. 32 (on, at most 2^n buckets)");
+  if (o.sort_digit_bits != 0 && o.sort_digit_bits != 8 && o.sort_digit_bits != 10)
+    return fail(SPRING_REORDER_E_ARG, "sort_digit_bits: 0 (library's choice), 8 or 10 bits per pass of the prefix sort");
+  if (o.presence_overlap < -1 || o.presence_overlap > 0)
+    return fail(SPRING_REORDER_E_ARG, "presence_overlap: 0 (library's choice) or -1 (presence table inside build_dict, sweep from round 0)");
   int ndev = 0;
   HIPCHK(hipGetDeviceCount(&ndev));
   if (ndev <= 0) return fail(SPRING_REORDER_E_HIP, "no HIP device");
@@ -363,9 +374,14 @@
   return 0;
 }
 
+static int presence_join(spring_reorder_ctx *ctx);
+
 void spring_reorder_destroy(spring_reorder_ctx *ctx) {
   if (!ctx) return;
   (void)hipSetDevice(ctx->dev);
+  (void)presence_join(ctx);
+  if (ctx->side.done) (void)hipEventDestroy(ctx->side.done);
+  if (ctx->side.h_drops) (void)hipHostFree(ctx->side.h_drops);
   if (ctx->st) (void)hipStreamSynchronize(ctx->st);
   if (ctx->st2) (void)hipStreamSynchronize(ctx->st2);
   if (ctx->st3) (void)hipStreamSynchronize(ctx->st3);
@@ -1013,6 +1029,7 @@
 }
 
 static unsigned sort_prefix_auto(uint64_t m) { return m <= (1ull << 29) ? 40u : 48u; }
+constexpr int SORT_DIGIT_BITS = 10;
 
 static bool strand_filter_wanted(const spring_reorder_ctx *ctx);
 
@@ -1028,6 +1045,53 @@
   }
   return lgb;
 }
+static bool two_groups_expected(const spring_reorder_ctx *ctx);
+static bool presence_beside_rounds(const spring_reorder_ctx *ctx) {
+  const spring_reorder_opts &o = ctx->o;
+  return o.presence_overlap == 0 && o.strand_filter == 0 && !o.time_search && o.num_devices < 2 && two_groups_expected(ctx);
+}
+static int presence_side_build(spring_reorder_ctx *ctx, uint64_t *const uhash[2], int lgb) {
+  auto &s = ctx->side;
+  hipStream_t st = ctx->st;
+  const uint32_t nk0 = ctx->dict[0].numkeys, nk1 = ctx->dict[1].numkeys;
+  const int wl = ctx->dict[0].end - ctx->dict[0].start + 1;
+  if (!ctx->st3) HIPCHK(hipStreamCreateWithFlags(&ctx->st3, hipStreamNonBlocking));
+  if (!s.done) HIPCHK(hipEventCreateWithFlags(&s.done, hipEventDisableTiming | hipEventDisableSystemFence));
+  if (!s.h_drops) HIPCHK(hipHostMalloc((void **)&s.h_drops, PRES_DROP_CTRS * 4, hipHostMallocDefault));
+  DMALLOC(s.d_drops, PRES_DROP_CTRS * 4);
+  DMALLOC(s.d_part, 2 * ((size_t)pres_write_blocks(lgb) + 1) * 4);
+  s.uhash[0] = uhash[0]; s.uhash[1] = uhash[1];
+  s.nm = (uint64_t)nk0 + nk1;
+  ctx->pres_lgb = lgb;
+  ctx->stats.strand_filter_build = 2;
+  ctx->stats.presence_overlap = 1;
+  HIPCHK(hipEventRecord(ctx->ev[3], st));
+  HIPCHK(hipStreamWaitEvent(ctx->st3, ctx->ev[3], 0));
+  s.pending = true;
+  HIPCHK(hipMemsetAsync(s.d_drops, 0, PRES_DROP_CTRS * 4, ctx->st3));
+  launch_pres_write(ctx->st3, uhash[0], nk0, uhash[1], nk1, wl, ctx->pres, lgb, s.d_part, s.d_drops);
+  launch_pres_insert(ctx->st3, uhash[0], nk0, uhash[1], nk1, wl, reinterpret_cast<uint32_t *>(ctx->pres), lgb, s.d_drops, true);
+  HIPCHK(hipGetLastError());
+  HIPCHK(hipMemcpyAsync(s.h_drops, s.d_drops, PRES_DROP_CTRS * 4, hipMemcpyDeviceToHost, ctx->st3));
+  HIPCHK(hipEventRecord(s.done, ctx->st3));
+  return 0;
+}
+static int presence_join(spring_reorder_ctx *ctx) {
+  auto &s = ctx->side;
+  if (!s.pending) return 0;
+  s.pending = false;
+  (void)hipSetDevice(ctx->dev);
+  const hipError_t e = hipStreamSynchronize(ctx->st3);
+  if (e == hipSuccess)
+    for (uint32_t i = 0; i < PRES_DROP_CTRS; i++) ctx->stats.strand_filter_dropped += s.h_drops[i];
+  ctx->dfree(s.uhash[0]); ctx->dfree(s.uhash[1]); ctx->dfree(s.d_drops); ctx->dfree(s.d_part);
+  s.uhash[0] = s.uhash[1] = nullptr; s.d_drops = s.d_part = nullptr;
+  HIPCHK(e);
+  if (ctx->o.debug) fprintf(stderr, "[dict] presence table: 2^%d buckets written once on the side stream, %llu of %llu keys dropped\n",
+                            ctx->pres_lgb, (unsigned long long)ctx->stats.strand_filter_dropped, (unsigned long long)s.nm);
+  return 0;
+}
+
 int spring_reorder_build_dict(spring_reorder_ctx *ctx) {
   double t_last = now_ms();
   if (!ctx) return fail(SPRING_REORDER_E_ARG, "ctx is NULL");
@@ -1038,6 +1102,7 @@
   const uint32_t n = ctx->n;
   HIPCHK(hipEventRecord(ctx->ev[2], st));
   ctx->pres = nullptr; ctx->pres_lgb = 0;
+  ctx->stats.presence_plain_rounds = 0;
   ctx->stats.strand_filter = 0; ctx->stats.strand_filter_dropped = 0; ctx->stats.strand_filter_build = 0;
   uint64_t *uhash[2] = {nullptr, nullptr};
   uint32_t *ustart[2] = {nullptr, nullptr}, *ucount[2] = {nullptr, nullptr};
@@ -1123,9 +1188,12 @@
       DMALLOC(d_runs, (size_t)cap * 8);
       HIPCHK(hipMemsetAsync(d_ctr, 0, 16, st));
       tmp_bytes = 0;
-      HIPCHK(sort_pairs(st, nullptr, tmp_bytes, k_in, k_out, v_in, d.ids, m, 64, 64 - T));
+      const int digit = ctx->o.sort_digit_bits ? ctx->o.sort_digit_bits : ctx->o.dict_build_mode == 1 ? 8 : SORT_DIGIT_BITS;
+      const auto prefix_sort = digit == 10 ? sort_pairs_wide : sort_pairs;
+      ctx->stats.sort_digit_bits = (uint64_t)digit;
+      HIPCHK(prefix_sort(st, nullptr, tmp_bytes, k_in, k_out, v_in, d.ids, m, 64, 64 - T));
       DMALLOC(d_tmp, tmp_bytes);
-      HIPCHK(sort_pairs(st, d_tmp, tmp_bytes, k_in, k_out, v_in, d.ids, m, 64, 64 - T));
+      HIPCHK(prefix_sort(st, d_tmp, tmp_bytes, k_in, k_out, v_in, d.ids, m, 64, 64 - T));
       DBG_T("prefix sort");
       launch_sort_repair(st, k_out, d.ids, m, T, d_list, cap, d_ctr, d_runs);
       HIPCHK(hipGetLastError());
@@ -1152,8 +1220,34 @@
     }
     ctx->dfree(d_tmp); d_tmp = nullptr;
     ctx->dfree(v_in);
+    DMALLOC(d_nruns, 16);
+    if (ctx->o.dict_build_mode != 1) {
+      uint32_t *d_tcnt = nullptr, *d_tfirst = nullptr, numkeys = 0;
+      const size_t ntiles = uniq_tiles(m);
+      DMALLOC(d_tcnt, ntiles * 4);
+      DMALLOC(d_tfirst, (ntiles + 1) * 4);
+      launch_unique_count(st, k_out, m, d_tcnt, d_tfirst, d_nruns);
+      HIPCHK(hipGetLastError());
+      HIPCHK(hipMemcpyAsync(&numkeys, d_nruns, 4, hipMemcpyDeviceToHost, st));
+      HIPCHK(hipStreamSynchronize(st));
+      d.numkeys = numkeys;
+      DBG_T("unique count");
+      DMALLOC(cnt, (size_t)numkeys * 4);
+      DMALLOC(ustart[l], (size_t)numkeys * 4);
+      launch_unique_write(st, k_out, m, d_tcnt, d_tfirst, k_in, ustart[l], cnt);
+      HIPCHK(hipGetLastError());
+      uhash[l] = k_in;
+      ucount[l] = cnt;
+      DMALLOC(d.urec, (size_t)numkeys * 16);
+      DMALLOC(d.deep, ((size_t)m / DEEP_BIN + 1) * 4);
+      DMALLOC(d.d_ndeep, 16);
+      HIPCHK(hipMemsetAsync(d.d_ndeep, 0, 12, st));
+      ctx->dfree(k_out); ctx->dfree(d_nruns); ctx->dfree(d_tcnt); ctx->dfree(d_tfirst);
+      DBG_T("unique write");
+      if (d_flag) { ctx->dfree(d_flag); ctx->dfree(d_slot); }
+      continue;
+    }
     DMALLOC(cnt, (size_t)m * 4);
-    DMALLOC(d_nruns, 16);
     tmp_bytes = 0;
     HIPCHK(rle(st, nullptr, tmp_bytes, k_out, m, k_in, cnt, d_nruns));
     DMALLOC(d_tmp, tmp_bytes);
@@ -1308,6 +1402,15 @@
   }
   int lgb = 0;
   if (presence_wanted(ctx, nm)) lgb = presence_alloc(ctx, nm, dbg);
+  ctx->stats.presence_overlap = 0;
+  if (ctx->pres && one_pass && presence_beside_rounds(ctx)) {
+    ctx->dfree(ustart[0]); ctx->dfree(ustart[1]); ctx->dfree(ucount[0]); ctx->dfree(ucount[1]);
+    DBG_T("free temps");
+    int rs = presence_side_build(ctx, uhash, lgb);
+    if (rs) return rs;
+    ctx->stage = ST_DICT;
+    return 0;
+  }
   if (ctx->pres) {
     const int wl = ctx->dict[0].end - ctx->dict[0].start + 1;
     uint32_t *d_drops = nullptr, *d_part = nullptr;
@@ -1381,6 +1484,7 @@
 int spring_reorder_presence_table(spring_reorder_ctx *ctx, void *out, size_t cap, int32_t *lgb) {
   if (!ctx || ctx->stage < ST_DICT) return fail(SPRING_REORDER_E_STATE, "presence_table: build_dict first");
   if (!ctx->pres) return fail(SPRING_REORDER_E_STATE, "presence_table: this build made no presence table");
+  { int rj = presence_join(ctx); if (rj) return rj; }
   const size_t nb = (size_t)16 << ctx->pres_lgb;
   if (lgb) *lgb = ctx->pres_lgb;
   if (!out) return 0;
@@ -1452,6 +1556,11 @@
   const uint32_t K = o.num_chains ? o.num_chains : auto_chains(ctx->n, dict_is_deep(ctx), dict_is_very_deep(ctx), dict_has_heavy_tail(ctx));
   const int phases = (groups_wanted(o, K, two_groups_pay_shallow(K)) == 2 && two_groups_fit(ctx->n, K)) ? 2 : 1;
   return mc_kernel_chosen(ctx, K, phases, true);
+}
+static bool two_groups_expected(const spring_reorder_ctx *ctx) {
+  const spring_reorder_opts &o = ctx->o;
+  const uint32_t K = o.num_chains ? o.num_chains : auto_chains(ctx->n, dict_is_deep(ctx), dict_is_very_deep(ctx), dict_has_heavy_tail(ctx));
+  return groups_wanted(o, K, two_groups_pay_shallow(K)) == 2 && two_groups_fit(ctx->n, K);
 }
 static void fill_params(spring_reorder_ctx *ctx, DevParams &P) {
   const spring_reorder_opts &o = ctx->o;
@@ -1817,6 +1926,13 @@
 }
 }
 
+constexpr double PRES_SIDE_NS_PER_KEY = 0.050, PLAIN_ROUND_NS_PER_CHAIN = 2.4;
+static int presence_plain_batches(const spring_reorder_ctx *ctx, int R) {
+  const double build_us = (double)ctx->side.nm * PRES_SIDE_NS_PER_KEY * 1e-3;
+  const double batch_us = std::max(1.0, (double)ctx->P.Ktot * PLAIN_ROUND_NS_PER_CHAIN * 1e-3 * R);
+  return (int)std::min(16.0, std::max(1.0, std::ceil(build_us / batch_us)));
+}
+
 static int run_chains_phased(spring_reorder_ctx *ctx, int R, bool timed) {
   DevParams &P = ctx->P;
   const bool stats = ctx->o.collect_stats != 0;
@@ -1824,7 +1940,12 @@
   if (!ctx->st3) HIPCHK(hipStreamCreateWithFlags(&ctx->st3, hipStreamNonBlocking));
   hipStream_t sg[2] = {ctx->st, ctx->st2}, sc = ctx->st3;
   uint64_t round_no[2] = {0, 0};
+  const bool beside = ctx->side.pending && P.sf && !timed && !stats;
+  if (!beside) { int rj = presence_join(ctx); if (rj) return rj; }
+  const int plain = beside ? presence_plain_batches(ctx, R) : 0;
+  ctx->stats.presence_plain_rounds = (uint64_t)plain * (uint64_t)R;
   RunOwned own;
+  struct JoinOnExit { spring_reorder_ctx *c; ~JoinOnExit() { (void)presence_join(c); } } join_guard{ctx};
   SyncOnError sync_guard{{ctx->st2, ctx->st3, ctx->st}};
   constexpr unsigned ORDER_ONLY = hipEventDisableTiming | hipEventDisableSystemFence;
   hipEvent_t ev[2], cev[2], ev0, evt;
@@ -1845,10 +1966,16 @@
   bool have_b = false;
   uint64_t rounds = 0, launches = 0;
   double ms_search = 0;
+  int batches = 0;
   auto enqueue_batch = [&]() -> int {
+    const bool sweep_off = batches < plain;
+    if (beside && batches == plain)
+      for (int g = 0; g < 2; g++) HIPCHK(hipStreamWaitEvent(sg[g], ctx->side.done, 0));
+    batches++;
     for (int r = 0; r < R; r++) {
       for (int g = 0; g < 2; g++) {
-        const DevParams Q = group_params(ctx, g, round_no[g]);
+        DevParams Q = group_params(ctx, g, round_no[g]);
+        if (sweep_off) { Q.sf = 0; Q.pres = nullptr; Q.pres_lgb = 0; }
         if (timed) HIPCHK(hipEventRecord(tev[4 * r + 2 * g], sg[g]));
         launch_round(sg[g], Q, stats, false);
         if (timed) HIPCHK(hipEventRecord(tev[4 * r + 2 * g + 1], sg[g]));
@@ -1890,12 +2017,15 @@
     launches += 2 * (uint64_t)R;
     return 0;
   };
+  for (int b = 0; b < plain; b++)
+    if ((rr = enqueue_batch())) return rr;
   if ((rr = run_round_loop(ctx, look, rounds, !timed, " (two groups)", enqueue_batch, count_batch, collect_times))) return rr;
   HIPCHK(hipStreamWaitEvent(sg[0], ev[1], 0));
   HIPCHK(hipEventRecord(ctx->ev[5], sg[0]));
   HIPCHK(hipStreamSynchronize(sg[1]));
   HIPCHK(hipStreamSynchronize(sc));
   HIPCHK(hipStreamSynchronize(sg[0]));
+  if ((rr = presence_join(ctx))) return rr;
   ctx->round_no = round_no[0];
   ctx->stats.rounds = rounds;
   ctx->stats.ms_search_kernel = ms_search;
@@ -1931,6 +2061,7 @@
   if (r0) return r0;
   DevParams &P = ctx->P;
   int R = ctx->o.rounds_per_sync > 0 ? ctx->o.rounds_per_sync : (K >= 256 ? 16 : 256);
+  if (P.phases != 2) { int rj = presence_join(ctx); if (rj) return rj; }
   if (P.phases == 2) {
     int rp = run_chains_phased(ctx, R, timed);
     if (rp) return rp;
@@ -2016,6 +2147,7 @@
     return fail(SPRING_REORDER_E_ARG, "mg_begin: total_chains (%u) must be a positive multiple of world (%u)", total_chains, world);
   if (ctx->o.force_literal_update) return fail(SPRING_REORDER_E_ARG, "mg_begin: the literal consensus path only exists in the two-kernel round");
   HIPCHK(hipSetDevice(ctx->dev));
+  { int rj = presence_join(ctx); if (rj) return rj; }
   const uint32_t K = total_chains / world;
   ctx->stats.chains = total_chains;
   ctx->stats.deep_pool = (dict_is_deep(ctx) ? 1 : 0) | (dict_has_heavy_tail(ctx) ? 2 : 0);
@@ -2406,6 +2538,7 @@
   if (!ctx) return fail(SPRING_REORDER_E_ARG, "ctx is NULL");
   if (ctx->stage != ST_CHAINS) return fail(SPRING_REORDER_E_STATE, "finalize: run_chains first");
   HIPCHK(hipSetDevice(ctx->dev));
+  { int rj = presence_join(ctx); if (rj) return rj; }
   hipStream_t st = ctx->st;
   DevParams &P = ctx->P;
   const uint32_t K = ctx->K;
@@ -2541,6 +2674,7 @@
 int spring_reorder_get_stats(spring_reorder_ctx *ctx, spring_reorder_stats *out) {
   if (!ctx || !out) return fail(SPRING_REORDER_E_ARG, "NULL argument");
   HIPCHK(hipSetDevice(ctx->dev));
+  { int rj = presence_join(ctx); if (rj) return rj; }
   HIPCHK(hipStreamSynchronize(ctx->st));
   spring_reorder_stats &s = ctx->stats;
   auto el = [&](int a, int b) {
diff --git a/spring_amd/reorder.py b/spring_amd/reorder.py
--- a/spring_amd/reorder.py
+++ b/spring_amd/reorder.py
@@ -42,6 +42,8 @@
     sort_prefix_bits: int = 0
     dict_build_mode: int = 0
     strand_filter: int = 0
+    sort_digit_bits: int = 0
+    presence_overlap: int = 0
 
     def to_c(self):
         o = _lib.Opts()
@@ -69,6 +71,8 @@
         o.sort_prefix_bits = self.sort_prefix_bits
         o.dict_build_mode = self.dict_build_mode
         o.strand_filter = self.strand_filter
+        o.sort_digit_bits = self.sort_digit_bits
+        o.presence_overlap = self.presence_overlap
         o.num_devices = len(self.devices)
         for i, d in enumerate(self.devices):
             o.devices[i] = d
```

Result: no change. 375.8 Mreads/s (-0.5%).
